# NumericalEarth/Breeze.jl

Measured on AMD Instinct MI355X. Metric: grid-cells advanced/sec (tendency+Poisson step), 512^3 anelastic, higher is better.
Workload: dtype f64

## Files before the change

breeze.jl_amd/csrc/bz_acoustic_kernels.h:

```cpp
#pragma once
#include "bz_compressible_internal.h"

__device__ __forceinline__ void ac_wall_faces(const DevGrid &g, const AcParams &P, int i, int j, double &up0, double &up1, double &vp0, double &vp1)
{
    if (g.bounded_x) {
        if (i == 0 && P.wall_w) up0 = 0.0;
        if (i == g.Nx - 1) up1 = 0.0;
    }
    if (g.bounded_y) {
        if (j == 0 && P.wall_s) vp0 = 0.0;
        if (j == g.Ny - 1) vp1 = 0.0;
    }
}
__device__ __forceinline__ bool ac_accumulate(const AcParams &P)
{
    return !(P.skip_avg_if_dry && __builtin_amdgcn_readfirstlane(*P.skip_avg_if_dry) == 1);
}

#ifndef AC_PENCIL
#define AC_PENCIL 1
#endif
__device__ __forceinline__ void ac_pencil_block(int &bx, int &j, int &k)
{
    bx = blockIdx.x; j = blockIdx.y; k = blockIdx.z;
    const unsigned gx = gridDim.x, gy = gridDim.y, gz = gridDim.z;
    if (AC_PENCIL && (gy & 63u) == 0) {
        const unsigned w = bx + gx * (j + gy * k), c = w & 7u;
        unsigned r = w >> 3;
        bx = (int)(r % gx); r /= gx;
        const unsigned jj = r & 7u; r >>= 3;
        k = (int)(r % gz); r /= gz;
        j = (int)(((r * 8 + c) * 8) + jj);
    }
    bx = __builtin_amdgcn_readfirstlane(bx); j = __builtin_amdgcn_readfirstlane(j); k = __builtin_amdgcn_readfirstlane(k);
}

template <bool ZERO, bool STORE0, bool PF, bool NOPERT, class ST>
__global__ __launch_bounds__(256) void k_ac_stage_init(DevGrid g, AcFieldsT<ST> F)
{
    int bx, j, k;
    ac_pencil_block(bx, j, k);
    const int i = bx * 256 + threadIdx.x;
    if (i >= g.Nx) return;
    const long long sz = g.Sxy;
    const long long n = g.idx(i, j, k);
    if (j >= g.Ny) {
        if (PF) F.Gp_rv[n] = F.G_rv[n] - (F.p[n] - F.p[n - g.Sx]) * g.rdy;
        return;
    }
    if (PF) {
        const WrapIdx W = wrap_of(g, i, j);
        const double p0 = F.p[n];
        F.Gp_ru[n] = F.G_ru[n] - (p0 - F.p[n + W.im]) * g.rdx;
        F.Gp_rv[n] = F.G_rv[n] - (p0 - F.p[n + W.jm]) * g.rdy;
    }
    if (STORE0) {
        ((double *)F.U0_rho_d)[n] = F.rho_d[n];
        ((double *)F.U0_rth)[n] = F.rth[n];
        ((double *)F.U0_ru)[n] = F.ru[n];
        ((double *)F.U0_rv)[n] = F.rv[n];
        ((double *)F.U0_rw)[n] = F.rw[n];
        ((double *)F.U0_rq)[n] = F.rq[n];
        if (!NOPERT) { F.rp[n] = 0.0; F.rthp_out[n] = 0.0; F.rup[n] = 0.0; F.rvp[n] = 0.0; F.rwp[n] = 0.0; }
    } else if (!NOPERT) {
    F.rp[n] = F.U0_rho_d[n] - F.rho_d[n];
    F.rthp_out[n] = F.U0_rth[n] - F.rth[n];
    F.rup[n] = F.U0_ru[n] - F.ru[n];
    F.rvp[n] = F.U0_rv[n] - F.rv[n];
    F.rwp[n] = F.U0_rw[n] - F.rw[n];
    }
    if (ZERO) {
    F.au[n] = 0.0;
    F.av[n] = 0.0;
    F.aw[n] = 0.0;
    }
    if (k == 0) {
        F.Gs[n] = 0.0;
    } else {
        const long long m = n - sz;
        const double dp = ((F.p[n] - g.p_r[k]) - (F.p[m] - g.p_r[k - 1])) * g.rdzf[k];
        const double rf = ((F.rho[n] - g.rho[k]) + (F.rho[m] - g.rho[k - 1])) / 2.0;
        F.Gs[n] = F.G_rw[n] - dp - g.g * rf;
    }
    if (k == g.Nz - 1) {
        if (STORE0) { ((double *)F.U0_rw)[n + sz] = F.rw[n + sz]; if (!NOPERT) F.rwp[n + sz] = 0.0; }
        else if (!NOPERT) F.rwp[n + sz] = F.U0_rw[n + sz] - F.rw[n + sz];
        F.Gs[n + sz] = 0.0;
    }
}

template <bool DAMP, bool STEP, class ST>
__global__ __launch_bounds__(256) void k_ac_horizontal(DevGrid g, AcFieldsT<ST> F, AcParams P)
{
    const int i = blockIdx.x * 256 + threadIdx.x, j = blockIdx.y, k = blockIdx.z;
    if (i >= g.Nx) return;
    const WrapIdx W = wrap_of(g, i, j);
    const long long n = g.idx(i, j, k), mx = n + W.im, my = n + W.jm;
    double up = F.rup[n], vp = F.rvp[n];
    const double rt = F.rthp[n], rtx = F.rthp[mx], rty = F.rthp[my];
    if (DAMP) {
        const double d0 = rt - F.rth_old[n];
        const double ddx = (d0 - (rtx - F.rth_old[mx])) * g.rdx;
        const double ddy = (d0 - (rty - F.rth_old[my])) * g.rdy;
        const double th = F.thL[n];
        up -= P.kdamp * ddx / ((th + F.thL[mx]) / 2.0);
        vp -= P.kdamp * ddy / ((th + F.thL[my]) / 2.0);
    }
    if (STEP) {
        const double p0 = F.p[n];
        double dpx = (p0 - F.p[mx]) * g.rdx;
        double dpy = (p0 - F.p[my]) * g.rdy;
        if (P.gate != 0.0) {
            const double c0 = F.Clin[n] * rt;
            dpx = dpx + P.gate * ((c0 - F.Clin[mx] * rtx) * g.rdx);
            dpy = dpy + P.gate * ((c0 - F.Clin[my] * rty) * g.rdy);
        }
        up += P.dtau * (F.G_ru[n] - dpx);
        vp += P.dtau * (F.G_rv[n] - dpy);
        if (g.bounded_x && i == 0 && P.wall_w) up = 0.0;
        if (g.bounded_y && j == 0 && P.wall_s) vp = 0.0;
        F.au[n] += up;
        F.av[n] += vp;
    }
    if (g.bounded_x && i == 0 && P.wall_w) up = 0.0;
    if (g.bounded_y && j == 0 && P.wall_s) vp = 0.0;
    F.rup[n] = up;
    F.rvp[n] = vp;
}

__device__ __forceinline__ double ibz(double fp, double fm, bool p_per, bool m_per)
{
    fp = p_per ? fm : fp;
    fm = m_per ? fp : fm;
    return (fp + fm) / 2.0;
}

template <bool DAMP>
__device__ __forceinline__ double ac_face_update(double up, double G, double rt_b, double rt_a, double rto_b, double rto_a,
                                                 double th_b, double th_a, double C_b, double C_a, double p_b, double p_a,
                                                 double rd, const AcParams &P)
{
    if (DAMP) {
        const double dd = ((rt_b - rto_b) - (rt_a - rto_a)) * rd;
        up -= P.kdamp * dd / ((th_b + th_a) / 2.0);
    }
    double dp = (p_b - p_a) * rd;
    if (P.gate != 0.0) dp = dp + P.gate * ((C_b * rt_b - C_a * rt_a) * rd);
    return up + P.dtau * (G - dp);
}

#ifndef ACX
#define ACX 64
#endif
#ifndef ACY
#define ACY 4
#endif
#ifndef ABX
#define ABX 256
#endif
#ifndef ABY
#define ABY 1
#endif
#ifndef AC_MINW
#define AC_MINW 1
#endif
template <bool FIRST, bool FUSED, bool DAMP, class ST>
__global__ __launch_bounds__(ACX * ACY, AC_MINW) void k_ac_column_forward(DevGrid g, AcFieldsT<ST> F, AcParams P)
{
    int bx = blockIdx.x, by = blockIdx.y;
    if (P.xcd) {
        const unsigned w = blockIdx.y * gridDim.x + blockIdx.x, c = w & 7u, r = w >> 3;
        bx = (int)(r % gridDim.x);
        by = (int)(c * (gridDim.y >> 3) + r / gridDim.x);
    }
    const int i = bx * ACX + threadIdx.x, j = by * ACY + threadIdx.y;
    if (i >= g.Nx || j >= g.Ny) return;
    const WrapIdx W = wrap_of(g, i, j);
    const long long sz = g.Sxy;
    const int Nz = g.Nz;
    long long n = g.idx(i, j, 0);
    const double dtn2 = P.dtn * P.dtn;

    double th_0 = F.thL[n], th_p = F.thL[n + sz];
    double C_m = 0.0, C_0 = F.Clin[n];
#ifndef AC_FX
#define AC_FX 1
#endif
    const bool FX = AC_FX && FUSED && (ACX == 64) && sizeof(ST) == 8;
    const int lane = threadIdx.x;
    double thy_m0 = 0.0, thy_p0 = 0.0, thy_m1 = 0.0, thy_p1 = 0.0;
    double cy_m0 = 0.0, cy_p0 = 0.0;
    if (FX) {
        thy_m0 = F.thL[n + W.jm]; thy_p0 = F.thL[n + W.jp];
        thy_m1 = F.thL[n + sz + W.jm]; thy_p1 = F.thL[n + sz + W.jp];
        cy_m0 = F.Clin[n + W.jm]; cy_p0 = F.Clin[n + W.jp];
    }
    double w_m = 0.0, w_0 = F.rwp[n], w_p = F.rwp[n + sz];
    double rs_m = 0.0, rths_m = 0.0, rp_m = 0.0, rthp_m = 0.0;
    double beta = 1.0, phi_m = 0.0, c_m = 0.0;
    double thf_0 = th_0, thf_m = th_0;

    for (int k = 0; k < Nz; ++k, n += sz) {
        const double rdc = g.rdzc[k];
        const double Ax = g.Ax[k], Ay = g.Ay[k], Vinv = g.Vinv_c[k];
        const double rp = F.rp[n], rthp = F.rthp[n];
        double thxm, thxp, thym, thyp;
        if (FX) {
            const double e_m = (lane == 0) ? F.thL[n + W.im] : 0.0, e_p = (lane == ACX - 1 || i == g.Nx - 1) ? F.thL[n + W.ip] : 0.0;
            thxm = __shfl_up(th_0, 1); thxp = __shfl_down(th_0, 1);
            if (lane == 0) thxm = e_m;
            if (lane == ACX - 1 || i == g.Nx - 1) thxp = e_p;
            thym = thy_m0; thyp = thy_p0;
        } else {
            thxm = F.thL[n + W.im]; thxp = F.thL[n + W.ip]; thym = F.thL[n + W.jm]; thyp = F.thL[n + W.jp];
        }
        double up0, up1, vp0, vp1;
        if (FUSED) {
            const long long nxm = n + W.im, nxp = n + W.ip, nym = n + W.jm, nyp = n + W.jp;
            const double rt_xm = F.rthp[nxm], rt_xp = F.rthp[nxp], rt_ym = F.rthp[nym], rt_yp = F.rthp[nyp];
            double o0 = 0.0, o_xm = 0.0, o_xp = 0.0, o_ym = 0.0, o_yp = 0.0;
            if (DAMP) { o0 = F.rth_old[n]; o_xm = F.rth_old[nxm]; o_xp = F.rth_old[nxp]; o_ym = F.rth_old[nym]; o_yp = F.rth_old[nyp]; }
            double c_xm = 0.0, c_xp = 0.0, c_ym = 0.0, c_yp = 0.0;
            if (FX) {
                const double e_m = (lane == 0) ? F.Clin[nxm] : 0.0, e_p = (lane == ACX - 1 || i == g.Nx - 1) ? F.Clin[nxp] : 0.0;
                c_xm = __shfl_up(C_0, 1); c_xp = __shfl_down(C_0, 1);
                if (lane == 0) c_xm = e_m;
                if (lane == ACX - 1 || i == g.Nx - 1) c_xp = e_p;
                c_ym = cy_m0; c_yp = cy_p0;
            } else if (P.gate != 0.0) { c_xm = F.Clin[nxm]; c_xp = F.Clin[nxp]; c_ym = F.Clin[nym]; c_yp = F.Clin[nyp]; }
            const double p0 = F.p[n], p_xm = F.p[nxm], p_xp = F.p[nxp], p_ym = F.p[nym], p_yp = F.p[nyp];
            up0 = ac_face_update<DAMP>(F.rup_in[n], F.G_ru[n], rthp, rt_xm, o0, o_xm, th_0, thxm, C_0, c_xm, p0, p_xm, g.rdx, P);
            up1 = ac_face_update<DAMP>(F.rup_in[nxp], F.G_ru[nxp], rt_xp, rthp, o_xp, o0, thxp, th_0, c_xp, C_0, p_xp, p0, g.rdx, P);
            vp0 = ac_face_update<DAMP>(F.rvp_in[n], F.G_rv[n], rthp, rt_ym, o0, o_ym, th_0, thym, C_0, c_ym, p0, p_ym, g.rdy, P);
            vp1 = ac_face_update<DAMP>(F.rvp_in[nyp], F.G_rv[nyp], rt_yp, rthp, o_yp, o0, thyp, th_0, c_yp, C_0, p_yp, p0, g.rdy, P);
            ac_wall_faces(g, P, i, j, up0, up1, vp0, vp1);
            F.rup[n] = up0;
            F.rvp[n] = vp0;
            if (FIRST) { F.au[n] = 0.0 + up0; F.av[n] = 0.0 + vp0; }
            else { F.au[n] += up0; F.av[n] += vp0; }
        } else {
            up0 = F.rup[n]; up1 = F.rup[n + W.ip]; vp0 = F.rvp[n]; vp1 = F.rvp[n + W.jp];
            ac_wall_faces(g, P, i, j, up0, up1, vp0, vp1);
            F.rth_old[n] = rthp;
        }
        const double thf_p = (k + 1 < Nz) ? (th_p + th_0) / 2.0 : th_0;

        const double dxM = Ax * up1 - Ax * up0;
        const double dxT = Ax * ((thxp + th_0) / 2.0) * up1 - Ax * ((th_0 + thxm) / 2.0) * up0;
        const double dyM = Ay * vp1 - Ay * vp0;
        const double dyT = Ay * ((thyp + th_0) / 2.0) * vp1 - Ay * ((th_0 + thym) / 2.0) * vp0;
        const double divM = Vinv * (dxM + dyM);
        const double divT = Vinv * (dxT + dyT);
        const double dzW = (w_p - w_0) * rdc;
        const double dzT = (thf_p * w_p - thf_0 * w_0) * rdc;
        const double rs = rp + P.dtau * (F.G_rho_d[n] - divM) - P.dto * dzW;
        const double rths = rthp + P.dtau * (P.f_theta * F.G_rth[n] - divT) - P.dto * dzT;
        F.rs[n] = rs;
        F.rths[n] = rths;

        double phi = 0.0;
        if (k > 0) {
            const double rdf = g.rdzf[k], rdm = g.rdzc[k - 1];
            const double dps = (C_0 * rths - C_m * rths_m) * rdf;
            const double dpo = (C_0 * rthp - C_m * rthp_m) * rdf;
            const double Gp = P.dto * dpo + P.dtn * dps;
            const double Gb = g.g * (P.dto * ((rp + rp_m) / 2.0) + P.dtn * ((rs + rs_m) / 2.0));
            const double d2 = ((w_p - w_0) * rdc - (w_0 - w_m) * rdm) * rdf;
            const double Gd = -P.d_old * d2;
            const double sp = F.sponge[k];
            const double f = w_0 + P.dtau * P.f_w * F.Gs[n] - Gp - Gb - Gd - fabs(P.dto) * sp * w_0;
            const double a = -dtn2 * C_m * thf_m * rdm * rdf + dtn2 * g.g * rdm / 2.0 + (-P.d_new * rdm * rdf);
            const double b = 1.0 + (dtn2 * thf_0 * (C_0 * rdc + C_m * rdm) * rdf + dtn2 * g.g * (rdc - rdm) / 2.0 +
                                    P.d_new * (rdc + rdm) * rdf + fabs(P.dtn) * sp);
            const double t = c_m / beta;
            beta = b - a * t;
            phi = (f - a * phi_m) / beta;
            if (FIRST) F.tfac[n] = t;
            c_m = -dtn2 * C_0 * thf_p * rdc * rdf + (-dtn2 * g.g * rdc / 2.0) + (-P.d_new * rdc * rdf);
        } else if (FIRST) {
            F.tfac[n] = 0.0;
        }
        F.phi[n] = phi;
        phi_m = phi;

        rs_m = rs; rths_m = rths; rp_m = rp; rthp_m = rthp;
        C_m = C_0;
        th_0 = th_p; thf_m = thf_0; thf_0 = thf_p;
        w_m = w_0; w_0 = w_p;
        if (k + 1 < Nz) {
            C_0 = F.Clin[n + sz];
            th_p = (k + 2 < Nz) ? F.thL[n + 2 * sz] : th_0;
            w_p = F.rwp[n + 2 * sz];
            if (FX) {
                cy_m0 = F.Clin[n + sz + W.jm]; cy_p0 = F.Clin[n + sz + W.jp];
                thy_m0 = thy_m1; thy_p0 = thy_p1;
                if (k + 2 < Nz) { thy_m1 = F.thL[n + 2 * sz + W.jm]; thy_p1 = F.thL[n + 2 * sz + W.jp]; }
            }
        }
    }
}

template <class T>
__device__ __forceinline__ T ac_ld(const T *base, unsigned e)
{
    return *(const T *)((const char *)base + (size_t)(e * (unsigned)sizeof(T)));
}
template <class T, class V>
__device__ __forceinline__ void ac_st(T *base, unsigned e, V v)
{
    *(T *)((char *)base + (size_t)(e * (unsigned)sizeof(T))) = (T)v;
}
#ifndef AC2_NT
#define AC2_NT 0
#endif
#ifndef AC2_BARRIER
#define AC2_BARRIER 0
#endif
template <class T>
__device__ __forceinline__ T ac_ld_nt(const T *base, unsigned e)
{
    if (AC2_NT & 1) return __builtin_nontemporal_load((const T *)((const char *)base + (size_t)(e * (unsigned)sizeof(T))));
    return ac_ld(base, e);
}
template <class T, class V>
__device__ __forceinline__ void ac_st_nt(T *base, unsigned e, V v)
{
    if (AC2_NT & 2) __builtin_nontemporal_store((T)v, (T *)((char *)base + (size_t)(e * (unsigned)sizeof(T))));
    else ac_st(base, e, v);
}

template <bool DAMP, bool PF>
__device__ __forceinline__ double ac_face_update2(double up, double G, double rt_b, double rt_a, double rto_b, double rto_a,
                                                  double th_b, double th_a, double C_b, double C_a, double p_b, double p_a,
                                                  double rd, const AcParams &P)
{
    if (DAMP) {
        const double dd = ((rt_b - rto_b) - (rt_a - rto_a)) * rd;
        up -= P.kdamp * dd / ((th_b + th_a) / 2.0);
    }
    if (PF) {
        if (P.gate != 0.0) G = G - P.gate * ((C_b * rt_b - C_a * rt_a) * rd);
        return up + P.dtau * G;
    }
    double dp = (p_b - p_a) * rd;
    if (P.gate != 0.0) dp = dp + P.gate * ((C_b * rt_b - C_a * rt_a) * rd);
    return up + P.dtau * (G - dp);
}

template <bool FIRST, bool DAMP, bool PF, int CFG, class ST, int INIT = 0>
__global__ __launch_bounds__((CFG & 1) ? 512 : 256, (CFG & 2) ? 3 : 2) void k_ac_forward2(DevGrid g, AcFieldsT<ST> F, AcParams P)
{
    static_assert(FIRST || INIT == 0, "initial perturbations belong to the first substep of a stage");
    int bx = blockIdx.x, by = blockIdx.y;
    if (P.xcd) {
        const unsigned w = blockIdx.y * gridDim.x + blockIdx.x, c = w & 7u, r = w >> 3;
        bx = (int)(r % gridDim.x);
        by = (int)(c * (gridDim.y >> 3) + r / gridDim.x);
    }
    const int i = bx * (int)blockDim.x + threadIdx.x, j = by * (int)blockDim.y + threadIdx.y;
    if (i >= g.Nx || j >= g.Ny) return;
    const WrapIdx W = wrap_of(g, i, j);
    const unsigned sz = (unsigned)g.Sxy;
    const unsigned dxp = (unsigned)(int)W.ip, dym = (unsigned)(int)W.jm, dyp = (unsigned)(int)W.jp;
    const int Nz = g.Nz;
    unsigned e = (unsigned)g.idx(i, j, 0);
    const double dtn2 = P.dtn * P.dtn;
    const int lane = threadIdx.x & 63;
    const bool edge_m = (lane == 0), edge_p = (lane == 63 || i == g.Nx - 1);
    const bool edge = edge_m || edge_p;
    const unsigned dedge = edge_m ? (unsigned)(int)W.im : dxp;
    const ColPtr::cptr sponge = (ColPtr::cptr)F.sponge;
    const double *Gu = PF ? F.Gp_ru : F.G_ru, *Gv = PF ? F.Gp_rv : F.G_rv;
    const bool acc = ac_accumulate(P);

    double th_0 = ac_ld(F.thL, e), th_p = ac_ld(F.thL, e + sz);
    double C_m = 0.0, C_0 = ac_ld(F.Clin, e);
    double thy_m0 = ac_ld(F.thL, e + dym), thy_p0 = ac_ld(F.thL, e + dyp);
    double thy_m1 = ac_ld(F.thL, e + sz + dym), thy_p1 = ac_ld(F.thL, e + sz + dyp);
    double cy_m0 = ac_ld(F.Clin, e + dym), cy_p0 = ac_ld(F.Clin, e + dyp);
    auto pert = [&](const double *U0, const double *U, unsigned ee) { return (double)(ST)(ac_ld(U0, ee) - ac_ld(U, ee)); };
    auto pert_w = [&](unsigned ee) { return ac_ld(F.U0_rw, ee) - ac_ld((const double *)F.rw, ee); };
    double w_m = 0.0, w_0, w_p;
    if (INIT == 2) { w_0 = 0.0; w_p = 0.0; }
    else if (INIT == 1) { w_0 = pert_w(e); w_p = pert_w(e + sz); }
    else { w_0 = ac_ld(F.rwp, e); w_p = ac_ld(F.rwp, e + sz); }
    double rs_m = 0.0, rths_m = 0.0, rp_m = 0.0, rthp_m = 0.0;
    double beta = 1.0, phi_m = 0.0, c_m = 0.0;
    double thf_0 = th_0, thf_m = th_0;

    struct AcLevel {
        double rp, rthp, rt_ym, rt_yp, o0, o_ym, o_yp, ru0, ru1, rv0, rv1, Gu0, Gu1, Gv0, Gv1, p0, p_xm, p_xp, p_ym, p_yp, au_o, av_o, Grho, Grth, Gs_k;
        double e_th, e_C, e_rt, e_o;
        double C_n, cy_mn, cy_pn, th_n, thy_mn, thy_pn, w_n;
    };
    auto level = [&](const unsigned e, const int k) {
        AcLevel L;
        const unsigned exp_ = e + dxp, eym = e + dym, eyp = e + dyp;
        if (INIT == 2) { L.rp = 0.0; L.rthp = 0.0; L.rt_ym = 0.0; L.rt_yp = 0.0; }
        else if (INIT == 1) {
            L.rp = pert(F.U0_rho_d, F.rho_d, e); L.rthp = pert(F.U0_rth, F.rth, e);
            L.rt_ym = pert(F.U0_rth, F.rth, eym); L.rt_yp = pert(F.U0_rth, F.rth, eyp);
        } else {
        L.rp = ac_ld_nt(F.rp, e); L.rthp = ac_ld(F.rthp, e);
        L.rt_ym = ac_ld(F.rthp, eym); L.rt_yp = ac_ld(F.rthp, eyp);
        }
        L.o0 = 0.0; L.o_ym = 0.0; L.o_yp = 0.0;
        if (DAMP) { L.o0 = ac_ld(F.rth_old, e); L.o_ym = ac_ld(F.rth_old, eym); L.o_yp = ac_ld(F.rth_old, eyp); }
        if (INIT == 2) { L.ru0 = 0.0; L.ru1 = 0.0; L.rv0 = 0.0; L.rv1 = 0.0; }
        else if (INIT == 1) {
            L.ru0 = pert(F.U0_ru, F.ru, e); L.ru1 = pert(F.U0_ru, F.ru, exp_); L.rv0 = pert(F.U0_rv, F.rv, e); L.rv1 = pert(F.U0_rv, F.rv, eyp);
        } else {
        L.ru0 = ac_ld(F.rup_in, e); L.ru1 = ac_ld(F.rup_in, exp_); L.rv0 = ac_ld(F.rvp_in, e); L.rv1 = ac_ld(F.rvp_in, eyp);
        }
        L.Gu0 = ac_ld(Gu, e); L.Gu1 = ac_ld(Gu, exp_); L.Gv0 = ac_ld(Gv, e); L.Gv1 = ac_ld(Gv, eyp);
        L.p0 = 0.0; L.p_xm = 0.0; L.p_xp = 0.0; L.p_ym = 0.0; L.p_yp = 0.0;
        if (!PF) {
            L.p0 = ac_ld(F.p, e); L.p_xm = ac_ld(F.p, e + (unsigned)(int)W.im); L.p_xp = ac_ld(F.p, exp_);
            L.p_ym = ac_ld(F.p, eym); L.p_yp = ac_ld(F.p, eyp);
        }
        L.au_o = 0.0; L.av_o = 0.0;
        if (!FIRST && acc && P.acc_mode != 1) { L.au_o = ac_ld_nt(F.au, e); L.av_o = ac_ld_nt(F.av, e); }
        L.Grho = ac_ld_nt(F.G_rho_d, e); L.Grth = ac_ld_nt(F.G_rth, e); L.Gs_k = ac_ld_nt(F.Gs, e);
        L.e_th = 0.0; L.e_C = 0.0; L.e_rt = 0.0; L.e_o = 0.0;
        if (edge) {
            const unsigned ee = e + dedge;
            L.e_th = ac_ld(F.thL, ee); L.e_C = ac_ld(F.Clin, ee);
            L.e_rt = INIT == 2 ? 0.0 : INIT == 1 ? pert(F.U0_rth, F.rth, ee) : ac_ld(F.rthp, ee);
            if (DAMP) L.e_o = ac_ld(F.rth_old, ee);
        }
        const unsigned e1 = (k + 1 < Nz) ? e + sz : e, e2 = (k + 2 < Nz) ? e1 + sz : e1;
        L.C_n = ac_ld(F.Clin, e1); L.cy_mn = ac_ld(F.Clin, e1 + dym); L.cy_pn = ac_ld(F.Clin, e1 + dyp);
        L.th_n = ac_ld(F.thL, e2); L.thy_mn = ac_ld(F.thL, e2 + dym); L.thy_pn = ac_ld(F.thL, e2 + dyp);
        L.w_n = INIT == 2 ? 0.0 : INIT == 1 ? pert_w(e1 + sz) : ac_ld_nt(F.rwp, e1 + sz);
        return L;
    };
    constexpr bool PIPE = (CFG & 8) != 0;
    auto work = [&](const AcLevel &L, const int k, const unsigned e) {
        const double rdc = g.rdzc[k];
        const double Ax = g.Ax[k], Ay = g.Ay[k], Vinv = g.Vinv_c[k];
        const double rp = L.rp, rthp = L.rthp, rt_ym = L.rt_ym, rt_yp = L.rt_yp, o0 = L.o0, o_ym = L.o_ym, o_yp = L.o_yp;
        const double ru0 = L.ru0, ru1 = L.ru1, rv0 = L.rv0, rv1 = L.rv1, Gu0 = L.Gu0, Gu1 = L.Gu1, Gv0 = L.Gv0, Gv1 = L.Gv1;
        const double p0 = L.p0, p_xm = L.p_xm, p_xp = L.p_xp, p_ym = L.p_ym, p_yp = L.p_yp, au_o = L.au_o, av_o = L.av_o;
        const double Grho = L.Grho, Grth = L.Grth, Gs_k = L.Gs_k, e_th = L.e_th, e_C = L.e_C, e_rt = L.e_rt, e_o = L.e_o;
        const double C_n = L.C_n, cy_mn = L.cy_mn, cy_pn = L.cy_pn, th_n = L.th_n, thy_mn = L.thy_mn, thy_pn = L.thy_pn, w_n = L.w_n;
        const double sp = sponge[k];

        constexpr bool DPP = (CFG & 16) != 0;
        double thxm = ac_lane_up<DPP>(th_0), thxp = ac_lane_down<DPP>(th_0);
        double c_xm = ac_lane_up<DPP>(C_0), c_xp = ac_lane_down<DPP>(C_0);
        double rt_xm = ac_lane_up<DPP>(rthp), rt_xp = ac_lane_down<DPP>(rthp);
        double o_xm = 0.0, o_xp = 0.0;
        if (DAMP) { o_xm = ac_lane_up<DPP>(o0); o_xp = ac_lane_down<DPP>(o0); }
        if (edge_m) { thxm = e_th; c_xm = e_C; rt_xm = e_rt; o_xm = e_o; }
        if (edge_p) { thxp = e_th; c_xp = e_C; rt_xp = e_rt; o_xp = e_o; }
        const double thym = thy_m0, thyp = thy_p0, c_ym = cy_m0, c_yp = cy_p0;

        const double up0 = ac_face_update2<DAMP, PF>(ru0, Gu0, rthp, rt_xm, o0, o_xm, th_0, thxm, C_0, c_xm, p0, p_xm, g.rdx, P);
        const double up1 = ac_face_update2<DAMP, PF>(ru1, Gu1, rt_xp, rthp, o_xp, o0, thxp, th_0, c_xp, C_0, p_xp, p0, g.rdx, P);
        const double vp0 = ac_face_update2<DAMP, PF>(rv0, Gv0, rthp, rt_ym, o0, o_ym, th_0, thym, C_0, c_ym, p0, p_ym, g.rdy, P);
        const double vp1 = ac_face_update2<DAMP, PF>(rv1, Gv1, rt_yp, rthp, o_yp, o0, thyp, th_0, c_yp, C_0, p_yp, p0, g.rdy, P);
        const double au_n = FIRST ? 0.0 + up0 : (P.acc_mode == 2) ? au_o + (ru0 + up0) : au_o + up0;
        const double av_n = FIRST ? 0.0 + vp0 : (P.acc_mode == 2) ? av_o + (rv0 + vp0) : av_o + vp0;
        const double thf_p = (k + 1 < Nz) ? (th_p + th_0) / 2.0 : th_0;

        const double dxM = Ax * up1 - Ax * up0;
        const double dxT = Ax * ((thxp + th_0) / 2.0) * up1 - Ax * ((th_0 + thxm) / 2.0) * up0;
        const double dyM = Ay * vp1 - Ay * vp0;
        const double dyT = Ay * ((thyp + th_0) / 2.0) * vp1 - Ay * ((th_0 + thym) / 2.0) * vp0;
        const double divM = Vinv * (dxM + dyM);
        const double divT = Vinv * (dxT + dyT);
        const double dzW = (w_p - w_0) * rdc;
        const double dzT = (thf_p * w_p - thf_0 * w_0) * rdc;
        const double rs = rp + P.dtau * (Grho - divM) - P.dto * dzW;
        const double rths = rthp + P.dtau * (P.f_theta * Grth - divT) - P.dto * dzT;

        double phi = 0.0, t = 0.0;
        if (k > 0) {
            const double rdf = g.rdzf[k], rdm = g.rdzc[k - 1];
            const double dps = (C_0 * rths - C_m * rths_m) * rdf;
            const double dpo = (C_0 * rthp - C_m * rthp_m) * rdf;
            const double Gp = P.dto * dpo + P.dtn * dps;
            const double Gb = g.g * (P.dto * ((rp + rp_m) / 2.0) + P.dtn * ((rs + rs_m) / 2.0));
            const double d2 = ((w_p - w_0) * rdc - (w_0 - w_m) * rdm) * rdf;
            const double Gd = -P.d_old * d2;
            const double f = w_0 + P.dtau * P.f_w * Gs_k - Gp - Gb - Gd - fabs(P.dto) * sp * w_0;
            const double a = -dtn2 * C_m * thf_m * rdm * rdf + dtn2 * g.g * rdm / 2.0 + (-P.d_new * rdm * rdf);
            const double b = 1.0 + (dtn2 * thf_0 * (C_0 * rdc + C_m * rdm) * rdf + dtn2 * g.g * (rdc - rdm) / 2.0 +
                                    P.d_new * (rdc + rdm) * rdf + fabs(P.dtn) * sp);
            t = c_m / beta;
            beta = b - a * t;
            phi = (f - a * phi_m) / beta;
            c_m = -dtn2 * C_0 * thf_p * rdc * rdf + (-dtn2 * g.g * rdc / 2.0) + (-P.d_new * rdc * rdf);
        }
        if (INIT) ac_st(F.rthp, e, rthp);
        if (INIT && !g.wrap_y) {
            if (j == 0) ac_st(F.rthp, e + dym, rt_ym);
            if (j == g.Ny - 1) ac_st(F.rthp, e + dyp, rt_yp);
        }
        ac_st_nt(F.rup, e, up0);
        ac_st_nt(F.rvp, e, vp0);
        if (acc && (FIRST || P.acc_mode != 1)) {
            ac_st_nt(F.au, e, au_n);
            ac_st_nt(F.av, e, av_n);
        }
        ac_st_nt(F.rs, e, rs);
        ac_st_nt(F.rths, e, rths);
        if (FIRST) ac_st_nt(F.tfac, e, t);
        ac_st_nt(F.phi, e, phi);
        phi_m = phi;
        if (AC2_BARRIER || (CFG & 4)) __builtin_amdgcn_s_barrier();

        rs_m = rs; rths_m = rths; rp_m = rp; rthp_m = rthp;
        C_m = C_0; C_0 = C_n;
        thf_m = thf_0; thf_0 = thf_p;
        th_0 = th_p; th_p = th_n;
        w_m = w_0; w_0 = w_p; w_p = w_n;
        cy_m0 = cy_mn; cy_p0 = cy_pn;
        thy_m0 = thy_m1; thy_p0 = thy_p1; thy_m1 = thy_mn; thy_p1 = thy_pn;
    };
    if (!PIPE) {
        for (int k = 0; k < Nz; ++k, e += sz) work(level(e, k), k, e);
    } else {
        AcLevel LA = level(e, 0), LB;
#pragma unroll 1
        for (int k = 0; k < Nz; k += 2, e += 2 * sz) {
            const int k1 = (k + 1 < Nz) ? k + 1 : k;
            LB = level(e + (unsigned)(k1 - k) * sz, k1);
            work(LA, k, e);
            if (k + 1 < Nz) {
                const int k2 = (k + 2 < Nz) ? k + 2 : k + 1;
                LA = level(e + (unsigned)(k2 - k) * sz, k2);
                work(LB, k + 1, e + sz);
            }
        }
    }
}

template <bool FIRST, class ST, int INIT = 0>
__global__ __launch_bounds__(ABX * ABY) void k_ac_column_backward(DevGrid g, AcFieldsT<ST> F, AcParams P)
{
    const int i = blockIdx.x * ABX + threadIdx.x, j = blockIdx.y * ABY + threadIdx.y;
    if (i >= g.Nx || j >= g.Ny) return;
    const long long sz = g.Sxy;
    const int Nz = g.Nz;
    const bool acc = ac_accumulate(P);
    long long n = g.idx(i, j, Nz - 1);
    double w_hi = F.rwp[n + sz];
    if (INIT) {
        w_hi = (INIT == 2) ? 0.0 : F.U0_rw[n + sz] - F.rw[n + sz];
        F.rwp[n + sz] = w_hi;
    }
    double th_0 = F.thL[n];
    double thf_hi = th_0;
    double t_hi = 0.0;
    for (int k = Nz - 1; k >= 0; --k, n -= sz) {
        const double th_m = (k > 0) ? F.thL[n - sz] : th_0;
        const double thf_lo = (k > 0) ? (th_0 + th_m) / 2.0 : th_0;
        double w_lo = F.phi[n];
        if (k < Nz - 1) w_lo -= t_hi * w_hi;
        const double rdc = g.rdzc[k];
        const double dzW = (w_hi - w_lo) * rdc;
        const double dzT = (thf_hi * w_hi - thf_lo * w_lo) * rdc;
        F.rp[n] = F.rs[n] - P.dtn * dzW;
        F.rthp_out[n] = F.rths[n] - P.dtn * dzT;
        const double w_old = (!FIRST && acc && P.acc_mode == 2) ? F.rwp[n] : 0.0;
        F.rwp[n] = w_lo;
        if (acc) {
            if (FIRST) F.aw[n] = 0.0 + w_lo;
            else if (P.acc_mode == 2) F.aw[n] += (w_old + w_lo);
            else if (P.acc_mode == 0) F.aw[n] += w_lo;
        }
        t_hi = F.tfac[n];
        w_hi = w_lo;
        thf_hi = thf_lo;
        th_0 = th_m;
    }
}

template <bool DAMP, class ST>
__global__ __launch_bounds__(256) void k_ac_finalize(DevGrid g, AcFieldsT<ST> F, AcParams P)
{
    const int i = blockIdx.x * 256 + threadIdx.x, j = blockIdx.y, k = blockIdx.z;
    if (i >= g.Nx) return;
    const WrapIdx W = wrap_of(g, i, j);
    const long long sz = g.Sxy;
    const long long n = g.idx(i, j, k), mx = n + W.im, my = n + W.jm;
    if (DAMP) {
        const double d0 = F.rthp[n] - F.rth_old[n];
        const double ddx = (d0 - (F.rthp[mx] - F.rth_old[mx])) * g.rdx;
        const double ddy = (d0 - (F.rthp[my] - F.rth_old[my])) * g.rdy;
        const double th = F.thL[n];
        double up = F.rup[n] - P.kdamp * ddx / ((th + F.thL[mx]) / 2.0);
        double vp = F.rvp[n] - P.kdamp * ddy / ((th + F.thL[my]) / 2.0);
        if (g.bounded_x && i == 0 && P.wall_w) up = 0.0;
        if (g.bounded_y && j == 0 && P.wall_s) vp = 0.0;
        F.rup[n] = up;
        F.rvp[n] = vp;
    }
    const double r0 = F.rho_d[n];
    double rx = (r0 + F.rho_d[mx]) / 2.0, ry = (r0 + F.rho_d[my]) / 2.0;
    rx = (rx == 0.0) ? 1.0 : rx;
    ry = (ry == 0.0) ? 1.0 : ry;
    const double ua = (F.ru[n] + F.au[n] * P.inv_N) / rx;
    const double va = (F.rv[n] + F.av[n] * P.inv_N) / ry;
    st_img(F.au, n, ua, W.ox, W.oy);
    st_img(F.av, n, va, W.ox, W.oy);
    double wa = 0.0;
    if (k > 0) {
        double rz = (r0 + F.rho_d[n - sz]) / 2.0;
        rz = (rz == 0.0) ? 1.0 : rz;
        wa = (F.rw[n] + F.aw[n] * P.inv_N) / rz;
    }
    st_img(F.aw, n, wa, W.ox, W.oy);
// ... 271 lines not shown
```

breeze.jl_amd/csrc/bz_internal.h:

```cpp
#pragma once
#include <hip/hip_runtime.h>
#include <hipfft/hipfft.h>

#include <cstdint>
#include <cstdio>
#include <string>
#include <vector>

#include "../../include/breeze_hip.h"

struct ColPtr {
    const double *p = nullptr;
    ColPtr() = default;
    __host__ __device__ ColPtr(const double *q) : p(q) {}
    __host__ __device__ operator const double *() const { return p; }
#ifdef __HIPCC__
    typedef const double __attribute__((address_space(4))) *cptr;
    __device__ __forceinline__ double operator[](int k) const { return ((cptr)p)[k]; }
    __device__ __forceinline__ double operator[](long long k) const { return ((cptr)p)[k]; }
#endif
};

struct DevGrid {
    int Nx, Ny, Nz;
    int Hx, Hy, Hz;
    int Sx, Sy;
    long long Sxy;
    double dx, dy, rdx, rdy, Az;
    ColPtr dzc, dzf, rdzf;
    ColPtr rdzc;
    ColPtr zc;
    ColPtr Ax, Ay;
    ColPtr Vinv_c, Vinv_f;
    ColPtr rho, rho_f;
    ColPtr rrho, rrho_f;
    ColPtr p_r, T_r;
    ColPtr pi_dry, lnpi;
    double kap_num;
    double g, Rd, Rv, cpd, cpv, pst;
    int formulation;
    int microphysics;
    int sa_maxiter;
    double sa_Ll, sa_cl, sa_dc, sa_L0, sa_Ttr, sa_ptr, sa_abstol;
    double *qv_field, *ql_field;
    double *rqcl_field, *rqr_field, *qcl_field, *qr_field;
    int wrap_y;
    int flat_y;
    int bounded_x;
    int bounded_y;

    __host__ __device__ inline long long idx(int i, int j, int k) const {
        return (long long)(i + Hx) + (long long)Sx * ((long long)(j + Hy)) + Sxy * (long long)(k + Hz);
    }
};

struct RKEpilogue {
    int mode = 0;
    double dt = 0.0, alpha = 0.0, oma = 0.0;
    const double *u0 = nullptr;
    double *u0_out = nullptr;
    const double *u0b = nullptr;
    double *u0b_out = nullptr;
};
#ifdef __HIPCC__
__device__ __forceinline__ void st_img(double *__restrict__ f, long long n, double v, long long ox, long long oy)
{
    f[n] = v;
    if (ox) f[n + ox] = v;
    if (oy) {
        f[n + oy] = v;
        if (ox) f[n + ox + oy] = v;
    }
}
__device__ __forceinline__ void st_img_only(double *__restrict__ f, long long n, double v, long long ox, long long oy)
{
    if (ox) f[n + ox] = v;
    if (oy) {
        f[n + oy] = v;
        if (ox) f[n + ox + oy] = v;
    }
}
__device__ __forceinline__ double bz_cdiv(double a, double b, double rb)
{
    const double q0 = a * rb;
    return fma(fma(-q0, b, a), rb, q0);
}
__device__ __forceinline__ double bz_rk_apply(int mode, double dt, double alpha, double oma, const double *u0,
                                              double *u0_out, double G, double uold, long long n)
{
    if (mode == 0) return G;
    double u0v;
    if (mode == 1) { u0_out[n] = uold; u0v = uold; }
    else u0v = u0[n];
    return oma * u0v + alpha * (uold + dt * G);
}
__device__ __forceinline__ double bz_rk_apply_pre(int mode, double dt, double alpha, double oma, double u0v, double *u0_out, double G,
                                                  double uold, long long n)
{
    if (mode == 1) { u0_out[n] = uold; u0v = uold; }
    else if (mode == 3) u0v = uold;
    return oma * u0v + alpha * (uold + dt * G);
}
#endif

#ifdef __HIPCC__
__device__ __forceinline__ double bz_sconst(double c)
{
    asm volatile("" : "+s"(c));
    return c;
}
__device__ __forceinline__ double bz_exp_small(double a)
{
    int s = 0;
    while (fabs(a) > 0.0625 && s < 64) { a *= 0.5; ++s; }
    double p = bz_sconst(1.0 / 362880.0);
    p = fma(p, a, bz_sconst(1.0 / 40320.0));
    p = fma(p, a, bz_sconst(1.0 / 5040.0));
    p = fma(p, a, bz_sconst(1.0 / 720.0));
    p = fma(p, a, bz_sconst(1.0 / 120.0));
    p = fma(p, a, bz_sconst(1.0 / 24.0));
    p = fma(p, a, bz_sconst(1.0 / 6.0));
    p = fma(p, a, 0.5);
    p = fma(p, a, 1.0);
    p = fma(p, a, 1.0);
    for (; s > 0; --s) p *= p;
    return p;
}
__device__ __forceinline__ double bz_exner_factor(const DevGrid &g, int k, double q, double cpm)
{
    return g.pi_dry[k] * bz_exp_small(((q * g.kap_num) / (cpm * g.cpd)) * g.lnpi[k]);
}
__device__ __forceinline__ double bz_buoyancy(const DevGrid &g, const double *__restrict__ T, const double *__restrict__ q,
                                              long long n, int k)
{
    double qv, ql = 0.0;
    if (g.microphysics == 1) { qv = g.qv_field[n]; ql = g.ql_field[n]; }
    else if (g.microphysics == 2) { qv = q[n]; ql = g.qcl_field[n] + g.qr_field[n]; }
    else qv = q[n];
    const double Rm = (1.0 - (qv + ql)) * g.Rd + qv * g.Rv;
    const double rhop = g.rho[k] * (g.Rd * g.T_r[k] / (Rm * T[n]) - 1.0);
    return -g.g * rhop;
}
__device__ __forceinline__ double bz_kessler_T(const DevGrid &g, double th, double qv, double ql, double pr)
{
    const double qd = 1.0 - (qv + ql);
    const double cpm = qd * g.cpd + qv * g.cpv + ql * g.sa_cl;
    return pow(pr / g.pst, (qd * g.Rd + qv * g.Rv) / cpm) * th + (g.sa_Ll * ql) / cpm;
}
__device__ __forceinline__ double bz_sa_psat(const DevGrid &g, double T)
{
    return g.sa_ptr * pow(T / g.sa_Ttr, g.sa_dc / g.Rv) * exp((1.0 / g.sa_Ttr - 1.0 / T) * g.sa_L0 / g.Rv);
}
__device__ __forceinline__ double bz_sa_T(const DevGrid &g, double th, double qv, double ql, double pr)
{
    const double qd = 1.0 - (qv + ql);
    const double cpm = qd * g.cpd + qv * g.cpv + ql * g.sa_cl;
    return pow(pr / g.pst, (qd * g.Rd + qv * g.Rv) / cpm) * th + (g.sa_Ll * ql) / cpm;
}
__device__ __forceinline__ void bz_sa_adjust(const DevGrid &g, double T, double qt, double pr, double &qv, double &ql)
{
    const double ps = bz_sa_psat(g, T);
    const double qs = (g.Rd / g.Rv) * (1.0 - qt) * ps / (pr - ps);
    ql = fmax(0.0, qt - qs);
    qv = qt - ql;
}
__device__ __forceinline__ double bz_sa_residual(const DevGrid &g, double T, double th, double qt, double pr)
{
    double qv, ql;
    bz_sa_adjust(g, T, qt, pr, qv, ql);
    return T - bz_sa_T(g, th, qv, ql, pr);
}
__device__ __forceinline__ double bz_sa_diagnose(const DevGrid &g, double th, double qt, double pr, double &qv, double &ql)
{
    qv = qt; ql = 0.0;
    const double T1 = bz_sa_T(g, th, qt, 0.0, pr);
    if (th == 0.0) return T1;
    const double rho1 = pr / (((1.0 - qt) * g.Rd + qt * g.Rv) * T1);
    if (qt <= bz_sa_psat(g, T1) / (rho1 * g.Rv * T1)) return T1;
    double qv1, ql1;
    bz_sa_adjust(g, T1, qt, pr, qv1, ql1);
    const double dT = (g.sa_Ll * ql1) / ((1.0 - (qv1 + ql1)) * g.cpd + qv1 * g.cpv + ql1 * g.sa_cl);
    double x1 = T1, x2 = T1 + fmax(0.01, dT / 2.0);
    double r1 = bz_sa_residual(g, x1, th, qt, pr), r2 = bz_sa_residual(g, x2, th, qt, pr);
    for (int it = 0; it < g.sa_maxiter && fabs(r2) > g.sa_abstol; ++it) {
        double s = (x2 - x1) / (r2 - r1);
        const bool valid = isfinite(s);
        s = valid ? s : 0.0;
        x1 = x2; r1 = r2;
        x2 -= r2 * s;
        r2 = valid ? bz_sa_residual(g, x2, th, qt, pr) : 0.0;
    }
    bz_sa_adjust(g, x2, qt, pr, qv, ql);
    return bz_sa_T(g, th, qv, ql, pr);
}
__device__ __forceinline__ double bz_ds_temperature(const DevGrid &g, double th, double qv, double ql, double rho, double abstol,
                                                    int maxiter)
{
    const double qd = 1.0 - (qv + ql);
    const double Rm = qd * g.Rd + qv * g.Rv;
    const double cpm = qd * g.cpd + qv * g.cpv + ql * g.sa_cl;
    const double kap = Rm / cpm, gam = cpm / (cpm - Rm);
    const double L = (g.sa_Ll * ql) / cpm;
    double T = pow(th, gam) * pow(rho * Rm / g.pst, gam - 1.0) + L;
    double dT = T;
    for (int it = 0; it < maxiter && fabs(dT) > abstol; ++it) {
        const double Phi = pow(rho * Rm * T / g.pst, kap) * th;
        dT = -(T - Phi - L) / (1.0 - kap * Phi / T);
        T += dT;
    }
    return T;
}
__device__ __forceinline__ double bz_ds_residual(const DevGrid &g, double T, double th0, double rho, double qt, double &qv, double &ql)
{
    const double qs = bz_sa_psat(g, T) / (rho * g.Rv * T);
    ql = fmax(0.0, qt - qs);
    qv = qt - ql;
    const double qd = 1.0 - (qv + ql);
    const double Rm = qd * g.Rd + qv * g.Rv;
    const double cpm = qd * g.cpd + qv * g.cpv + ql * g.sa_cl;
    const double L = (g.sa_Ll * ql) / cpm;
    const double p = rho * Rm * T;
    return (T - L) * pow(g.pst / p, Rm / cpm) - th0;
}
__device__ __forceinline__ double bz_ds_adjust(const DevGrid &g, double th, double qt, double rho, double nabstol, int nmaxiter,
                                               double &qv, double &ql)
{
    qv = qt; ql = 0.0;
    if (th == 0.0) return 0.0;
    const double T1 = bz_ds_temperature(g, th, qt, 0.0, rho, nabstol, nmaxiter);
    if (qt <= bz_sa_psat(g, T1) / (rho * g.Rv * T1)) return T1;
    double qv1, ql1;
    bz_ds_residual(g, T1, th, rho, qt, qv1, ql1);
    const double dT = (g.sa_Ll * ql1) / ((1.0 - (qv1 + ql1)) * g.cpd + qv1 * g.cpv + ql1 * g.sa_cl);
    double x1 = T1, x2 = T1 + fmax(0.01, dT / 2.0);
    double a, b;
    double r1 = bz_ds_residual(g, x1, th, rho, qt, a, b), r2 = bz_ds_residual(g, x2, th, rho, qt, a, b);
    for (int it = 0; it < g.sa_maxiter && fabs(r2) > g.sa_abstol; ++it) {
        double s = (x2 - x1) / (r2 - r1);
        const bool valid = isfinite(s);
        s = valid ? s : 0.0;
        x1 = x2; r1 = r2;
        x2 -= r2 * s;
        r2 = valid ? bz_ds_residual(g, x2, th, rho, qt, a, b) : 0.0;
    }
    bz_ds_residual(g, x2, th, rho, qt, qv, ql);
    return bz_ds_temperature(g, th, qv, ql, rho, nabstol, nmaxiter);
}
#endif

struct BzComm;
struct ProfileSlot {
    const char *name;
    double total_ms = 0.0;
    int64_t launches = 0;
    std::vector<std::pair<hipEvent_t, hipEvent_t>> pending;
};

struct bz_tuning {
    bool no_fused = false;
    bool no_fuse_rk = false;
    bool no_lean = false;
    bool no_xcd = false;
    bool no_closure_march = false;
    bool no_k6_stored = false;
    bool no_dry_shortcut = false;
    bool side_scalar = false;
    int side_cus = 0;
    int side_cu_layout = 0;
    bool no_fuse_forcing = false;
    bool no_fold_forcing = false;
    int ac_xcd = 1;
    int ac_forward2 = 1;
    int ac_rotate = 1;
    int ac_pair_avg = 1;
    int ac_init_fold = 1;
    int ac_pfold = 1;
    int ac_bx = 128;
    int ac_cfg = 29;
    bool no_fuse_level_sums = false;
    bool no_tridiag_coop = false;
    bool no_xfft = false;
    int poisson_kxmajor = 1;
    int poisson_kx_chunk_mb = 0;
    int poisson_kx_chunk_kb = 0;
    int poisson_kx_pad = 1;
    int poisson_chunk = 0;
    int xf_kchunk_f = 0, xf_kchunk_i = 0;
    int scalar_lds = 1;
    bool no_rho3d_exchange = false;
    bool no_generic_march = false;
    bool generic_onepass = false;
    bool no_ac_fuse = false;
    bool no_ac_end_fuse = false;
    bool comm_no_overlap = false;
    bool comm_self_messages = false;
    bool comm_no_side_scalar = false;
    int graph = -1;
    bool graph_debug = false;
};
void bzi_read_tuning(bz_tuning &t);
#define BZ_REJECT_BOUNDED_Y(ctx, enabling, what)                                                                             \
    do {                                                                                                                     \
        if ((ctx) && (ctx)->dg.bounded_y && (enabling)) {                                                                                \
            (ctx)->last_error = what ": not implemented on a Bounded y (topology (Periodic, Bounded, Bounded))";            \
            return BZ_ERR_UNSUPPORTED;                                                                                       \
        }                                                                                                                    \
    } while (0)
#define BZ_REJECT_KINEMATIC(ctx, who)                                                                                        \
    do {                                                                                                                     \
        if ((ctx) && (ctx)->kinematic) {                                                                                     \
            (ctx)->last_error = who ": the context has PrescribedDynamics (no momentum, no pressure solve); use bz_time_steps_kinematic"; \
            return BZ_ERR_UNSUPPORTED;                                                                                       \
        }                                                                                                                    \
    } while (0)
#define BZ_HALO_XFACE 8
#define BZ_HALO_YFACE 4
struct bz_ctx;
bool bzi_lean_forcings_ok(const bz_ctx *ctx);

struct bz_ctx {
    bz_tuning tune;
    bz_grid grid;
    bz_constants constants;
    DevGrid dg;
    hipStream_t stream = nullptr;
    bool walls_lean_ok = false;
    int num_cus = 256;
    std::string last_error;

    double *d_columns = nullptr;
    int NXH = 0;
    hipfftHandle plan_fwd = 0, plan_inv = 0;
    hipfftDoubleComplex *d_dctx = nullptr;
    bool plans_ok = false;
    hipfftHandle plan_fwd_c = 0, plan_inv_c = 0;
    int pchunk = 0;
    int kr0 = 0, krn = 0;
    bool xf = false;
    bool xf_slab = false;
    void *d_wtab = nullptr;
    hipfftHandle plan_y = 0;
    bool kxmajor = false;
    int kx_cw = 0, kx_nch = 0, kx_pad = 0;
    hipfftHandle plan_yc = 0, plan_yc_last = 0;
    int profile_mute = 0;
    hipfftHandle slab_plan_x_fwd = 0, slab_plan_x_inv = 0, slab_plan_y = 0;
    bool slab_plans_ok = false;
    int slab_inv_ld = 0;
    double *d_rhs = nullptr;
    hipfftDoubleComplex *d_hat = nullptr;
    double *d_ibeta = nullptr;
    double *d_tfac = nullptr;
    double *d_lower = nullptr;
    double *d_scalar = nullptr;
    double *d_havg = nullptr;
    double *d_moments = nullptr;
    struct AzPlan *az = nullptr;
    int y_nranks = 1, y_rank = 0, nkx = 0, kx0 = 0, Ny_global = 0;
    bool slab_mode = false;
    bool tiled_tendencies = true;
    bool fuse_rk = true;
    bool G_is_predictor = false;
    bool fused_ok = true;
    int q_host = 0;
    int *h_qstate = nullptr;
    hipEvent_t ev_q = nullptr;
    bool q_pending = false;
    int *d_qstate = nullptr;
    bool diagnostics_stale = false;
    bool lean_step_last = false;
    bool lean = true;
    bool lean_xcd = true;
    hipStream_t side_stream = nullptr;
    hipEvent_t ev_fork = nullptr, ev_join = nullptr;
    bool side_scalar = false;
    void *d_lev_rows = nullptr;
    double *d_pi_dry = nullptr;
    bool compressible = false;
    bool has_reference = false;
    bz_split_explicit se;
    int weno_R = 3;
    int scalar_R = 3;
    double *d_gflux = nullptr;
    double dz_min = 0.0;
    double *d_sponge = nullptr;
    double *d_Clin = nullptr;
    double *d_tfac_ac = nullptr;
    double *d_up2 = nullptr, *d_vp2 = nullptr;
    double *d_Gp_ru = nullptr, *d_Gp_rv = nullptr;
    double *d_thL2 = nullptr;
    double *d_balance = nullptr;
    bool thL_alt = false;
    bool substep_f32 = false;
    bool ac_whole_step = false;
    bool ac_rotate = false;
    bool ac_skip_avg = false;
    bool ac_fused = true;
    int ac_open[4] = {0, 0, 0, 0};
    double ac_open_relax = 0.5;
    bz_kessler_microphysics kessler_params;
    bz_kessler_model_fields kessler;
    double kessler_pst = 1e5;
    bool has_instant_precip = false;
    double *ip_precipitation_rate = nullptr;
    bool has_relaxation = false;
    double *d_relax = nullptr;
    int relax_mask = 0, relax_specific = 0;
    const double *field_forcing = nullptr;
    int field_forcing_specific = 0;
    bool has_forcings = false;
    double *d_forcing = nullptr;
    int forcing_static_mask = 0, forcing_subsidence_mask = 0;
    double *d_lsum_rows = nullptr;
    long long lsum_P = 0;
    bool lsum_fresh = false;
    bool lsum_step_last = false;
    bool fold_momentum_forcing = false;
    double forcing_f = 0.0, forcing_flux_theta = 0.0, forcing_flux_q = 0.0, forcing_drag = 0.0, forcing_drag_eps = 0.0, forcing_flux_energy = 0.0;
    bool has_bulk = false;
    bz_bulk_surface_fluxes bulk;
    bool bulk_const_on = false;
    bool sl_on = false;
    bz_surface_layer sl;
    double *d_sl = nullptr;
    bool sl_initialized = false;
    int n_tracers = 0;
    bz_tracer_fields tracers[BZ_MAX_TRACERS];
    bool has_closure = false;
    bz_smagorinsky_lilly closure;
    double *closure_nu = nullptr;
    double *d_closure_ipi = nullptr;
    bool has_diffusivity = false;
    bz_scalar_diffusivity diffusivity;
    double *diff_nu = nullptr, *diff_kappa = nullptr;
    double *d_diff_table = nullptr;
    double *d_diff_scratch = nullptr;
    int diff_scratch_fields = 0;
    double *up2_user = nullptr, *vp2_user = nullptr;
    alignas(8) unsigned char ac_stage_storage[160] = {0};
    int bounded_mask = 0;
    double bounded_lo = 0.0, bounded_hi = 1.0;
    bool kinematic = false;
    bool kin_correction = false;
    double *d_kin_div = nullptr;
    uint64_t velocity_epoch = 0;
    uint64_t kin_div_epoch = 0;
    const double *kin_div_u = nullptr, *kin_div_v = nullptr, *kin_div_w = nullptr;
    struct BzComm *comm = nullptr;
    bool profiling = false;
    std::vector<ProfileSlot> slots;
    int graph_mode = 0;
    bool graph_capturing = false;
    uint64_t config_epoch = 0;
    struct GraphSlot {
        uint64_t key = 0;
        int seen = 0;
        hipGraph_t graph = nullptr;
        hipGraphExec_t exec = nullptr;
        bool g_is_predictor = false, lean_step_last = false, lsum_step_last = false;
    } graph_slots[2];
    int graph_next = 0;
    hipStream_t graph_stream = nullptr, graph_user_stream = nullptr;
    long long graph_replays = 0, graph_captures = 0;
};

uint64_t bzi_graph_key(const bz_ctx *ctx, int kind, double dt, const void *a, size_t na, const void *b, size_t nb, const void *c, size_t nc,
                       const void *d, size_t nd);
int bzi_graph_begin(bz_ctx *ctx, uint64_t key, bool *capture);
int bzi_graph_end(bz_ctx *ctx, uint64_t key, int body_rc);
void bzi_graph_destroy(bz_ctx *ctx);
void bzi_graph_configure(bz_ctx *ctx);
int bzi_apply_stream(bz_ctx *ctx, hipStream_t stream);

#define BZ_HIP(expr)                                                                        \
    do {                                                                                    \
        hipError_t _e = (expr);                                                             \
        if (_e != hipSuccess) {                                                             \
            ctx->last_error = std::string(#expr) + ": " + hipGetErrorString(_e);            \
            return -(int)_e;                                                                \
        }                                                                                   \
    } while (0)

#define BZ_FFT(expr)                                                                        \
    do {                                                                                    \
        hipfftResult _r = (expr);                                                           \
        if (_r != HIPFFT_SUCCESS) {                                                         \
            ctx->last_error = std::string(#expr) + ": hipfft status " + std::to_string((int)_r); \
            return -1000 - (int)_r;                                                         \
        }                                                                                   \
    } while (0)

#define BZ_LAUNCH_CHECK()                                                                   \
    do {                                                                                    \
        hipError_t _e = hipGetLastError();                                                  \
        if (_e != hipSuccess) {                                                             \
            ctx->last_error = std::string("kernel launch: ") + hipGetErrorString(_e);       \
            return -(int)_e;                                                                \
        }                                                                                   \
    } while (0)

typedef unsigned long long bz_bits_t;
__device__ __forceinline__ bz_bits_t bz_real_bits(double d) { return (bz_bits_t)__double_as_longlong(d); }
__device__ __forceinline__ double bz_real_inf() { return __longlong_as_double(0x7ff0000000000000LL); }

struct ProfileScope {
    bz_ctx *ctx;
    int slot = -1;
    hipEvent_t e0 = nullptr, e1 = nullptr;
    ProfileScope(bz_ctx *c, const char *name);
    ~ProfileScope();
};

int bzi_fill_halo(bz_ctx *ctx, double *f, int kind);
int bzi_apply_forcings(bz_ctx *ctx, const bz_state *s, double *Gu, double *Gv, double *Gth, double *Gq, double scale, bool momentum_done = false);
int bzi_compute_forcings(bz_ctx *ctx, const bz_state *s);
double *bzi_level_sum_rows(bz_ctx *ctx, long long *P);
bool bzi_level_sums_ride(const bz_ctx *ctx);
int bzi_flux_bc(bz_ctx *ctx, const bz_state *s, double *Gu, double *Gv, double *Gth, double *Gq, double scale);
int bzi_surface_layer_stage(bz_ctx *ctx, const bz_state *s, int stage, double dt);
void bzi_forcing_teardown(bz_ctx *ctx);
void bzi_diagnostics_teardown(bz_ctx *ctx);
void bzi_azimuthal_teardown(bz_ctx *ctx);
void bzi_moments_teardown(bz_ctx *ctx);
int bzi_tracer_specific(bz_ctx *ctx);
int bzi_tracer_rk3(bz_ctx *ctx, double dt, double alpha, bool first);
int bzi_tracer_store_initial_state(bz_ctx *ctx);
int bzi_tracer_tendencies(bz_ctx *ctx, const bz_state *s, bool one_record = true);
int bzi_momentum_advection_gen1(bz_ctx *ctx, const bz_state *s, const bz_prognostic *G);
int bzi_momentum_advection_generic(bz_ctx *ctx, const bz_state *s, const bz_prognostic *G);
int bzi_generic_tendencies_fused_rk(bz_ctx *ctx, const bz_state *s, const bz_prognostic *U0, const bz_prognostic *G, double dt, double alpha,
                                    bool first);
int bzi_scalar_tendency_generic(bz_ctx *ctx, double *Gc, const double *u, const double *v, const double *w, const double *c);
int bzi_scalar_rho3d_generic(bz_ctx *ctx, double *Gc, double *Grho, const double *rho, const double *u, const double *v, const double *w,
                             const double *c, const double *ru, const double *rv, const double *rw);
void bzi_closure_teardown(bz_ctx *ctx);
int bzi_apply_closure(bz_ctx *ctx, const bz_state *s, double *Gu, double *Gv, double *Gw, double *Gth, double *Gq, double scale);
void bzi_diffusivity_teardown(bz_ctx *ctx);
int bzi_diffusivity_halos(bz_ctx *ctx);
int bzi_apply_diffusivity(bz_ctx *ctx, const bz_state *s, double *Gu, double *Gv, double *Gw, double *Gth, double *Gq, double scale);
int bzi_cmp_closure_fields(bz_ctx *ctx, const bz_compressible_state *s);
int bzi_cmp_closure_slow(bz_ctx *ctx, const bz_compressible_state *s, const bz_compressible_prognostic *G);
int bzi_cmp_diffusivity_slow(bz_ctx *ctx, const bz_compressible_state *s, const bz_compressible_prognostic *G);
int bzi_cmp_water_closure(bz_ctx *ctx, const bz_compressible_state *s, const bz_compressible_prognostic *G, const int *skip_if_dry);
int bzi_implicit_step(bz_ctx *ctx, double *ru, double *rv, double *rw, double *rth, double *rq, double dtau);
int bzi_kessler_rk3(bz_ctx *ctx, double dt, double alpha, bool first);
int bzi_kessler_columns(bz_ctx *ctx, double *theta, double *rho_theta, double *rho_q, const double *density, const double *pressure, double dt);
int bzi_kessler_update(bz_ctx *ctx, const bz_state *s, const bz_prognostic *G, double dt);
int bzi_fill_halos_multi(bz_ctx *ctx, double *const *fields, const int *kinds, int n);
int bzi_poisson_setup(bz_ctx *ctx, const double *h_rho_halo );
int bzi_bounded_tendencies(bz_ctx *ctx, const bz_state *s, const bz_prognostic *G);
int bzi_compute_tendencies_generic(bz_ctx *ctx, const bz_state *s, const bz_prognostic *G);
int bzi_momentum_tendencies_generic(bz_ctx *ctx, const bz_state *s, const bz_prognostic *G);
int bzi_apply_relaxation(bz_ctx *ctx, const bz_state *s, const bz_prognostic *G, const double *rho3d = nullptr);
int bzi_lean_setup(bz_ctx *ctx);
int bzi_dist_time_step(bz_ctx *ctx, const bz_state *s, const bz_prognostic *U0, const bz_prognostic *G, double dt, bool diagnose = true);
int bzi_pack_rows_geom(bz_ctx *ctx, double *const *fields, const int32_t *levels, int32_t n, int32_t row0, int32_t nrows, double *buffer,
                       int32_t unpack, int sx, long long sxy);
int bzi_comm_join_pending(bz_ctx *ctx);
int bzi_refresh_diagnostics(bz_ctx *ctx, const bz_state *s, const char *who);
int bzi_kinematic_update_state(bz_ctx *ctx, const bz_state *s, const bz_prognostic *G, int compute_tendencies);
void bzi_kinematic_teardown(bz_ctx *ctx);
enum bz_tier { BZ_TIER_LEAN, BZ_TIER_FUSED_RK, BZ_TIER_FUSED, BZ_TIER_OPERATORS };
bz_tier bzi_anelastic_tier(const bz_ctx *ctx);
inline constexpr double BZ_SSP_RK3_ALPHA[3] = {1.0, 1.0 / 4.0, 2.0 / 3.0};
int bzi_zero_wall_faces(bz_ctx *ctx, const bz_prognostic *G, const bz_prognostic *U0 = nullptr);
int bzi_fused_rk_physics(bz_ctx *ctx, const bz_state *s, const bz_prognostic *G, double dt, double alpha, bool first, bool fold);
void bzi_lean_step_done(bz_ctx *ctx, bool diagnosed);
int bzi_scan_moisture(bz_ctx *ctx, const bz_state *s);
int bzi_scan_moisture_field(bz_ctx *ctx, const double *rho_q);
const int *bzi_moisture_state(const bz_ctx *ctx);
void bzi_moisture_unknown(bz_ctx *ctx);
struct LeanStage;
void bzi_lean_stage(const bz_state *s, const bz_prognostic *U0, const bz_prognostic *G, int stage, LeanStage *L);
int bzi_dist_time_step_compressible(bz_ctx *ctx, const bz_compressible_state *s, const bz_compressible_prognostic *U0,
                                    const bz_compressible_prognostic *G, const bz_acoustic_substepper *sub, double dt);
int bzi_compressible_store_initial_state(bz_ctx *ctx, const bz_compressible_state *s, const bz_compressible_prognostic *U0);
void bzi_comm_teardown(bz_ctx *ctx);
int bzi_comm_allreduce_sum(bz_ctx *ctx, double *buf, int n);
void bzi_lean_teardown(bz_ctx *ctx);
void bzi_poisson_teardown(bz_ctx *ctx);
int bzi_poisson_solve(bz_ctx *ctx, const bz_state *s, double dt);
int bzi_poisson_spectral(bz_ctx *ctx);
int bzi_poisson_from_momentum(bz_ctx *ctx, const bz_state *s, double dt, const bz_prognostic *predictor);
int bzi_fft_chunk(bz_ctx *ctx, int k0, bool forward);
int bzi_xf_forward(bz_ctx *ctx, const bz_state *s, double dt, const bz_prognostic *predictor, const double *rhs = nullptr,
                   double *hat = nullptr, int blocks = 1, int klo = 0, int khi = 0);
int bzi_xf_inverse(bz_ctx *ctx, const double *hat = nullptr, double *phi = nullptr, int blocks = 1, int klo = 0, int khi = 0);
int bzi_xf_y(bz_ctx *ctx, bool forward);
int bzi_tridiag_launch(bz_ctx *ctx, double *hat, double scale, int Ny, int mean_column, int kx_lo = 0, int kx_hi = 0);
int bzi_xf_middle(bz_ctx *ctx);
int bzi_rk3_fused(bz_ctx *ctx, const bz_state *s, const bz_prognostic *U0, const bz_prognostic *G, double dt,
                  double alpha, bool first);
int bzi_poisson_source_fused(bz_ctx *ctx, const bz_state *s, double dt, double *rhs = nullptr,
                             const bz_prognostic *predictor = nullptr);
int bzi_project_diagnose(bz_ctx *ctx, const bz_state *s, double dt, const double *phi_c = nullptr,
                         const double *phi_below = nullptr, const bz_prognostic *predictor = nullptr, bool store_phi = true,
                         const double *rtheta_in = nullptr, const double *rq_in = nullptr, bool level_sums = false);
int bzi_project_lean(bz_ctx *ctx, const bz_state *s, double dt, const double *phi_c, const double *phi_below,
                     const bz_prognostic *predictor, double *sa, double *sb);
struct LeanStage {
    bz_state sin;
    bz_state sout;
    bz_prognostic u0;
    const double *pa, *pb;
    double *oa, *ob;
};
int bzi_tendencies_lean(bz_ctx *ctx, const bz_state *s, const bz_prognostic *U0, const bz_prognostic *G, const double *pa,
                        const double *pb, double *oa, double *ob, double dt, double alpha, bool first, int rows = 0, int which = 3);
static inline int bzi_lean_tendencies(bz_ctx *ctx, const LeanStage &L, const bz_prognostic *G, double dt, double alpha, bool first,
                                      int rows = 0, int which = 3)
{
    return bzi_tendencies_lean(ctx, &L.sin, &L.u0, G, L.pa, L.pb, L.oa, L.ob, dt, alpha, first, rows, which);
}
int bzi_scalar_pair_fork(bz_ctx *ctx, const LeanStage &L, const bz_prognostic *G, double dt, double alpha, bool first);
int bzi_scalar_pair_join(bz_ctx *ctx);
int bzi_tendencies_fused_rk(bz_ctx *ctx, const bz_state *s, const bz_prognostic *U0, const bz_prognostic *G, double dt,
                            double alpha, bool first);
int bzi_create(bz_ctx **out, const bz_grid *grid, const bz_constants *constants, const bz_reference_state *ref,
               int weno_order, int y_nranks, int y_rank, bool slab_mode, bool compressible = false);
void bzi_compressible_teardown(bz_ctx *ctx);
void bzi_balance_teardown(bz_ctx *ctx);
int bzi_refresh_reference_columns(bz_ctx *ctx, const double *density, const double *pressure);
bool bzi_k6_stored_ok(const bz_ctx *ctx);
int bzi_k6_stored(bz_ctx *ctx, int comp, const bz_state *s, const bz_prognostic *G, const bz_prognostic *U0, const RKEpilogue *Ein, int bm);
int bzi_scalar_pair_tendency(bz_ctx *ctx, const bz_state *s, const bz_prognostic *G, const bz_prognostic *U0 = nullptr,
                             const RKEpilogue *E = nullptr);
int bzi_u_tendency_lds(bz_ctx *ctx, const bz_state *s, const bz_prognostic *G, const bz_prognostic *U0 = nullptr,
                       const RKEpilogue *E = nullptr);
int bzi_v_tendency_lds(bz_ctx *ctx, const bz_state *s, const bz_prognostic *G, const bz_prognostic *U0 = nullptr,
                       const RKEpilogue *E = nullptr);
int bzi_w_tendency_lds(bz_ctx *ctx, const bz_state *s, const bz_prognostic *G, const bz_prognostic *U0 = nullptr,
                       const RKEpilogue *E = nullptr, int buoyancy_mode = 0);
```

breeze.jl_amd/csrc/bz_step.hip:

```cpp
#include <cstdlib>

#include "bz_internal.h"

extern "C" int bz_update_state(bz_ctx *ctx, const bz_state *s, const bz_prognostic *G, int compute_tendencies)
{
    if (!ctx || !s || (compute_tendencies && !G)) return BZ_ERR_INVALID;
    if (ctx->kinematic) return bzi_kinematic_update_state(ctx, s, G, compute_tendencies);
    int rc;
    if (ctx->comm && (rc = bzi_comm_join_pending(ctx))) return rc;
    ctx->diagnostics_stale = false;
    if (ctx->d_qstate) BZ_HIP(hipMemsetAsync(ctx->d_qstate, 0, sizeof(int), ctx->stream));
    bzi_moisture_unknown(ctx);
    double *sf[4] = {s->rho_theta, s->rho_q, ctx->dg.rqcl_field, ctx->dg.rqr_field};
    int sk[4] = {0, 0, 0, 0};
    if ((rc = bzi_fill_halos_multi(ctx, sf, sk, ctx->dg.microphysics == 2 ? 4 : 2))) return rc;
    if ((rc = bz_compute_velocities(ctx, s))) return rc;
    if ((rc = bz_compute_auxiliary_thermodynamic_variables(ctx, s))) return rc;
    if (compute_tendencies && (rc = bz_compute_tendencies(ctx, s, G))) return rc;
    return BZ_OK;
}

bz_tier bzi_anelastic_tier(const bz_ctx *ctx)
{
    const DevGrid &g = ctx->dg;
    const bool slab = ctx->slab_mode;
    const bool walls_lean = g.bounded_y && ctx->walls_lean_ok;
    const bool order5 = ctx->weno_R == 3 && ctx->scalar_R == 3;
    const bool theta_model = g.formulation == 0;
    const bool lean_switches = slab || (ctx->fuse_rk && ctx->lean);
    const bool lean_anelastic = slab || !ctx->compressible;
    const bool lean_forcings = !ctx->has_forcings || (!slab && bzi_lean_forcings_ok(ctx));
    const bool rk_orders = slab ? order5
                                : ctx->scalar_R == ctx->weno_R && (ctx->weno_R == 3 || ctx->n_tracers == 0);
    const bool rk_forcings = slab || !(ctx->has_forcings && ctx->tune.no_fuse_forcing);
    const bool fused_tier = !slab;
    if ((ctx->fused_ok || walls_lean) && lean_switches && order5 && lean_anelastic && theta_model && g.microphysics == 0 && lean_forcings &&
        !ctx->has_bulk && !ctx->has_closure && !ctx->has_diffusivity && !ctx->has_relaxation && ctx->n_tracers == 0 && !ctx->bounded_mask &&
        (long long)g.Sxy * (g.Nz + 2 * g.Hz + 1) < (1LL << 32))
        return BZ_TIER_LEAN;
    if ((ctx->fused_ok || (walls_lean && ctx->weno_R != 3)) && ctx->fuse_rk && rk_orders && theta_model && g.microphysics != 2 &&
        !ctx->bounded_mask && !ctx->has_relaxation && rk_forcings)
        return BZ_TIER_FUSED_RK;
    return ctx->fused_ok && fused_tier ? BZ_TIER_FUSED : BZ_TIER_OPERATORS;
}

int bzi_zero_wall_faces(bz_ctx *ctx, const bz_prognostic *G, const bz_prognostic *U0)
{
    const DevGrid &g = ctx->dg;
    for (const long long face : {g.Sxy * g.Hz, g.Sxy * (g.Hz + g.Nz)})
        BZ_HIP(hipMemsetAsync(G->rho_w + face, 0, g.Sxy * sizeof(double), ctx->stream));
    return U0 ? bzi_zero_wall_faces(ctx, U0, nullptr) : BZ_OK;
}

int bzi_scalar_pair_fork(bz_ctx *ctx, const LeanStage &L, const bz_prognostic *G, double dt, double alpha, bool first)
{
    BZ_HIP(hipEventRecord(ctx->ev_fork, ctx->stream));
    BZ_HIP(hipStreamWaitEvent(ctx->side_stream, ctx->ev_fork, 0));
    hipStream_t keep = ctx->stream;
    ctx->stream = ctx->side_stream;
    const int rc = bzi_lean_tendencies(ctx, L, G, dt, alpha, first, 0, 2);
    ctx->stream = keep;
    if (rc) return rc;
    BZ_HIP(hipEventRecord(ctx->ev_join, ctx->side_stream));
    return BZ_OK;
}

int bzi_scalar_pair_join(bz_ctx *ctx) { BZ_HIP(hipStreamWaitEvent(ctx->stream, ctx->ev_join, 0)); return BZ_OK; }

int bzi_fused_rk_physics(bz_ctx *ctx, const bz_state *s, const bz_prognostic *G, double dt, double alpha, bool first, bool fold)
{
    int rc;
    if (ctx->n_tracers) {
        if ((rc = bzi_tracer_tendencies(ctx, s))) return rc;
        if ((rc = bzi_tracer_rk3(ctx, dt, alpha, first))) return rc;
    }
    if (ctx->has_closure && (rc = bzi_apply_closure(ctx, s, G->rho_u, G->rho_v, G->rho_w, s->rho_theta, s->rho_q, alpha * dt))) return rc;
    if (ctx->has_diffusivity && (rc = bzi_apply_diffusivity(ctx, s, G->rho_u, G->rho_v, G->rho_w, s->rho_theta, s->rho_q, alpha * dt))) return rc;
    if (ctx->has_forcings && (rc = bzi_apply_forcings(ctx, s, G->rho_u, G->rho_v, s->rho_theta, s->rho_q, alpha * dt, fold))) return rc;
    if ((ctx->has_forcings || ctx->has_bulk) && (rc = bzi_flux_bc(ctx, s, G->rho_u, G->rho_v, s->rho_theta, s->rho_q, alpha * dt))) return rc;
    return BZ_OK;
}

void bzi_lean_step_done(bz_ctx *ctx, bool diagnosed)
{
    ctx->lean_step_last = true;
    ctx->G_is_predictor = true;
    ctx->diagnostics_stale = !diagnosed;
}

void bzi_lean_stage(const bz_state *s, const bz_prognostic *U0, const bz_prognostic *G, int stage, LeanStage *L)
{
    L->sin = *s; L->sout = *s;
    if (stage > 0) { L->sin.rho_u = U0->rho_u; L->sin.rho_v = U0->rho_v; L->sin.rho_w = U0->rho_w; }
    if (stage < 2) { L->sout.rho_u = U0->rho_u; L->sout.rho_v = U0->rho_v; L->sout.rho_w = U0->rho_w; }
    L->u0.rho_u = s->rho_u; L->u0.rho_v = s->rho_v; L->u0.rho_w = s->rho_w; L->u0.rho_theta = s->rho_theta; L->u0.rho_q = s->rho_q;
    L->pa = stage == 0 ? s->rho_theta : stage == 1 ? G->rho_theta : U0->rho_theta;
    L->pb = stage == 0 ? s->rho_q : stage == 1 ? G->rho_q : U0->rho_q;
    L->oa = stage == 0 ? G->rho_theta : stage == 1 ? U0->rho_theta : s->rho_theta;
    L->ob = stage == 0 ? G->rho_q : stage == 1 ? U0->rho_q : s->rho_q;
}

static int lean_project(bz_ctx *ctx, const bz_state *s, const LeanStage &L, const bz_prognostic *G, double adt, bool full)
{
    return full ? bzi_project_diagnose(ctx, s, adt, nullptr, nullptr, G, true, L.oa, L.ob) : bzi_project_lean(ctx, &L.sout, adt, nullptr, nullptr, G, L.oa, L.ob);
}

static int lean_solve_and_project(bz_ctx *ctx, const bz_state *s, const LeanStage &L, const bz_prognostic *G, double adt, bool full, bool forked)
{
    const DevGrid &g = ctx->dg;
    const int ch = ctx->pchunk;
    int rc = BZ_OK;
    if (ch) {
        {
            ProfileScope ps(ctx, "poisson_source_term+fft_forward");
            ctx->profile_mute++;
            for (int k0 = 0; k0 < g.Nz && !rc; k0 += ch) {
                ctx->kr0 = k0; ctx->krn = ch;
                rc = bzi_poisson_source_fused(ctx, s, adt, nullptr, G);
                if (!rc) rc = bzi_fft_chunk(ctx, k0, true);
            }
            ctx->krn = 0;
            ctx->profile_mute--;
        }
        if (rc) return rc;
        ProfileScope ps(ctx, "poisson_tridiagonal");
        if ((rc = bzi_tridiag_launch(ctx, (double *)ctx->d_hat, 1.0 / ((double)g.Nx * (double)g.Ny), g.Ny, 1))) return rc;
    } else if (ctx->xf) {
        {
            ProfileScope ps(ctx, "poisson_source_term+fft_x");
            if ((rc = bzi_xf_forward(ctx, s, adt, G))) return rc;
        }
        if ((rc = bzi_xf_middle(ctx))) return rc;
        ProfileScope ps(ctx, "poisson_fft_x_inverse");
        if ((rc = bzi_xf_inverse(ctx))) return rc;
    } else {
        if ((rc = bzi_poisson_source_fused(ctx, s, adt, nullptr, G))) return rc;
        if ((rc = bzi_poisson_spectral(ctx))) return rc;
    }
    if (forked && (rc = bzi_scalar_pair_join(ctx))) return rc;
    if (!ch) return lean_project(ctx, s, L, G, adt, full);
    ProfileScope ps(ctx, !full ? "poisson_fft_inverse+project_momentum" : "poisson_fft_inverse+project_and_diagnose");
    ctx->profile_mute++;
    for (int k0 = 0; k0 < g.Nz && !rc; k0 += ch) {
        if ((rc = bzi_fft_chunk(ctx, k0, false))) break;
        ctx->kr0 = k0; ctx->krn = ch;
        rc = lean_project(ctx, s, L, G, adt, full);
    }
    ctx->krn = 0;
    ctx->profile_mute--;
    return rc;
}

static int step_lean(bz_ctx *ctx, const bz_state *s, const bz_prognostic *U0, const bz_prognostic *G, double dt, bool diagnose)
{
    int rc;
    if ((rc = bzi_zero_wall_faces(ctx, G, U0))) return rc;
    const bool fork = ctx->side_scalar && !ctx->has_forcings;
    for (int stage = 0; stage < 3; ++stage) {
        const double alpha = BZ_SSP_RK3_ALPHA[stage];
        LeanStage L;
        bzi_lean_stage(s, U0, G, stage, &L);
        if ((rc = bzi_lean_tendencies(ctx, L, G, dt, alpha, stage == 0, 0, fork ? 1 : 3))) return rc;
        if (fork && (rc = bzi_scalar_pair_fork(ctx, L, G, dt, alpha, stage == 0))) return rc;
        if (ctx->has_forcings && (rc = bzi_flux_bc(ctx, &L.sin, G->rho_u, G->rho_v, L.oa, L.ob, alpha * dt))) return rc;
        if ((rc = lean_solve_and_project(ctx, s, L, G, alpha * dt, diagnose && stage == 2, fork))) return rc;
    }
    bzi_lean_step_done(ctx, diagnose);
    return BZ_OK;
}

static int step_fused_rk(bz_ctx *ctx, const bz_state *s, const bz_prognostic *U0, const bz_prognostic *G, double dt, bool lsum_in)
{
    int rc;
    if ((rc = bzi_zero_wall_faces(ctx, G))) return rc;
    const bool fold = ctx->has_forcings && ctx->weno_R == 3 && bzi_k6_stored_ok(ctx) && ctx->tiled_tendencies && !ctx->tune.no_fuse_forcing && !ctx->tune.no_fold_forcing;
    for (int stage = 0; stage < 3; ++stage) {
        const double alpha = BZ_SSP_RK3_ALPHA[stage];
        if (stage == 0) ctx->lsum_fresh = lsum_in;
        if (fold && (rc = bzi_compute_forcings(ctx, s))) return rc;
        ctx->fold_momentum_forcing = fold;
        rc = bzi_tendencies_fused_rk(ctx, s, U0, G, dt, alpha, stage == 0);
        ctx->fold_momentum_forcing = false;
        if (rc) return rc;
        if ((rc = bzi_fused_rk_physics(ctx, s, G, dt, alpha, stage == 0, fold))) return rc;
        if ((rc = bzi_implicit_step(ctx, G->rho_u, G->rho_v, G->rho_w, s->rho_theta, s->rho_q, alpha * dt))) return rc;
        if (ctx->dg.bounded_y && (rc = bzi_fill_halo(ctx, G->rho_v, BZ_HALO_YFACE))) return rc;
        if ((rc = bzi_poisson_from_momentum(ctx, s, alpha * dt, G))) return rc;
        const bool ride = bzi_level_sums_ride(ctx) && ctx->d_lsum_rows;
        if ((rc = bzi_project_diagnose(ctx, s, alpha * dt, nullptr, nullptr, G, stage == 2, nullptr, nullptr, ride))) return rc;
        ctx->lsum_fresh = ride;
        if ((rc = bzi_tracer_specific(ctx))) return rc;
        if ((rc = bzi_surface_layer_stage(ctx, s, stage, dt))) return rc;
    }
    ctx->lsum_step_last = ctx->lsum_fresh;
    ctx->G_is_predictor = true;
    return BZ_OK;
}

static int step_fused(bz_ctx *ctx, const bz_state *s, const bz_prognostic *U0, const bz_prognostic *G, double dt)
{
    int rc;
    if (ctx->G_is_predictor && (rc = bz_compute_tendencies(ctx, s, G))) return rc;
    for (int stage = 0; stage < 3; ++stage) {
        const double alpha = BZ_SSP_RK3_ALPHA[stage];
        if ((rc = bz_compute_flux_bc_tendencies(ctx, s, G))) return rc;
        if ((rc = bzi_rk3_fused(ctx, s, U0, G, dt, alpha, stage == 0))) return rc;
        if (ctx->dg.microphysics == 2 && (rc = bzi_kessler_rk3(ctx, dt, alpha, stage == 0))) return rc;
        if ((rc = bzi_tracer_rk3(ctx, dt, alpha, stage == 0))) return rc;
        if ((rc = bz_implicit_step(ctx, s, alpha * dt))) return rc;
        if ((rc = bzi_poisson_from_momentum(ctx, s, alpha * dt, nullptr))) return rc;
        if ((rc = bzi_project_diagnose(ctx, s, alpha * dt))) return rc;
        if ((rc = bzi_tracer_specific(ctx))) return rc;
        if ((rc = bzi_surface_layer_stage(ctx, s, stage, dt))) return rc;
        if ((rc = bz_compute_tendencies(ctx, s, G))) return rc;
    }
    if (ctx->dg.microphysics == 2 && (rc = bzi_kessler_update(ctx, s, G, dt))) return rc;
    return BZ_OK;
}

static int step_operators(bz_ctx *ctx, const bz_state *s, const bz_prognostic *U0, const bz_prognostic *G, double dt)
{
    int rc;
    if (ctx->G_is_predictor && (rc = bz_compute_tendencies(ctx, s, G))) return rc;
    if ((rc = bz_store_initial_state(ctx, s, U0))) return rc;
    for (int stage = 0; stage < 3; ++stage) {
        const double alpha = BZ_SSP_RK3_ALPHA[stage];
        if ((rc = bz_compute_flux_bc_tendencies(ctx, s, G))) return rc;
        if ((rc = bz_ssp_rk3_substep(ctx, s, U0, G, dt, alpha))) return rc;
        if ((rc = bz_implicit_step(ctx, s, alpha * dt))) return rc;
        if ((rc = bz_compute_pressure_correction(ctx, s, alpha * dt))) return rc;
        if ((rc = bz_make_pressure_correction(ctx, s, alpha * dt))) return rc;
        if ((rc = bz_update_state(ctx, s, G, 1))) return rc;
        if ((rc = bzi_surface_layer_stage(ctx, s, stage, dt))) return rc;
    }
    if (ctx->dg.microphysics == 2 && (rc = bzi_kessler_update(ctx, s, G, dt))) return rc;
    return BZ_OK;
}

static int anelastic_step_body(bz_ctx *ctx, bz_tier tier, const bz_state *s, const bz_prognostic *U0, const bz_prognostic *G, double dt, bool diagnose)
{
    ctx->lean_step_last = false;
    ctx->lsum_step_last = false;
    const bool lsum_in = ctx->lsum_fresh;
    ctx->lsum_fresh = false;
    if (tier == BZ_TIER_LEAN) return step_lean(ctx, s, U0, G, dt, diagnose);
    if (tier == BZ_TIER_FUSED_RK) return step_fused_rk(ctx, s, U0, G, dt, lsum_in);
    if (tier == BZ_TIER_FUSED) return step_fused(ctx, s, U0, G, dt);
    return step_operators(ctx, s, U0, G, dt);
}

static int one_anelastic_step(bz_ctx *ctx, const bz_state *s, const bz_prognostic *U0, const bz_prognostic *G, double dt, bool diagnose)
{
    if (ctx->slab_mode) {
        if (ctx->comm) return bzi_dist_time_step(ctx, s, U0, G, dt, diagnose);
        ctx->last_error = "bz_time_step_anelastic: a y-slab context needs a communicator (bz_comm_init_rccl / bz_comm_init_local) "
                          "or a host-side distributed driver";
        return BZ_ERR_UNSUPPORTED;
    }
    const bz_tier tier = bzi_anelastic_tier(ctx);
    if (ctx->diagnostics_stale && tier != BZ_TIER_LEAN) { const int rcs = bz_update_state(ctx, s, G, 0); if (rcs) return rcs; }
    const int kind = 1 + (diagnose ? 0 : 16) + 32 * ctx->q_host + (ctx->lsum_fresh ? 128 : 0);
    const uint64_t key = bzi_graph_key(ctx, kind, dt, s, sizeof(*s), U0, sizeof(*U0), G, sizeof(*G), nullptr, 0);
    bool capture = false;
    int rc;
    if (bzi_graph_begin(ctx, key, &capture) == 1) {
        if (ctx->lean_step_last) ctx->diagnostics_stale = !diagnose;
        ctx->lsum_fresh = ctx->lsum_step_last;
        return BZ_OK;
    }
    const bool lsum_in = ctx->lsum_fresh;
    if (capture) {
        rc = anelastic_step_body(ctx, tier, s, U0, G, dt, diagnose);
        if ((rc = bzi_graph_end(ctx, key, rc)) != -1) return rc;
        ctx->lsum_fresh = lsum_in;
    }
    return anelastic_step_body(ctx, tier, s, U0, G, dt, diagnose);
}

static void level_sums_open(bz_ctx *ctx)
{
    ctx->lsum_fresh = false;
    long long P;
    (void)bzi_level_sum_rows(ctx, &P);
}

static int surface_layer_first_step(bz_ctx *ctx, const bz_state *s)
{
    if (!ctx->sl_on || !ctx->sl.filtered || ctx->sl_initialized) return BZ_OK;
    return bz_surface_layer_initialize(ctx, s);
}

extern "C" int bz_time_step_anelastic(bz_ctx *ctx, const bz_state *s, const bz_prognostic *U0, const bz_prognostic *G, double dt)
{
    if (!ctx || !s || !U0 || !G) return BZ_ERR_INVALID;
    BZ_REJECT_KINEMATIC(ctx, "bz_time_step_anelastic");
    level_sums_open(ctx);
    int rc = bzi_scan_moisture(ctx, s);
    if (!rc) rc = surface_layer_first_step(ctx, s);
    if (!rc) rc = one_anelastic_step(ctx, s, U0, G, dt, true);
    ctx->lsum_fresh = false;
    return rc;
}

extern "C" int bz_time_steps_anelastic(bz_ctx *ctx, const bz_state *s, const bz_prognostic *U0, const bz_prognostic *G, double dt, int n,
                                       int diagnose_last)
{
    if (!ctx || !s || !U0 || !G || n < 0) return BZ_ERR_INVALID;
    BZ_REJECT_KINEMATIC(ctx, "bz_time_steps_anelastic");
    level_sums_open(ctx);
    if (n > 0) { const int rc = bzi_scan_moisture(ctx, s); if (rc) return rc; }
    if (n > 0) { const int rc = surface_layer_first_step(ctx, s); if (rc) return rc; }
    for (int it = 0; it < n; ++it) {
        const int rc = one_anelastic_step(ctx, s, U0, G, dt, it == n - 1 && diagnose_last);
        if (rc) { ctx->lsum_fresh = false; return rc; }
    }
    ctx->lsum_fresh = false;
    return BZ_OK;
}

int bzi_refresh_diagnostics(bz_ctx *ctx, const bz_state *s, const char *who)
{
    if (!ctx->diagnostics_stale) return BZ_OK;
    if (!s) {
        ctx->last_error = std::string(who) + ": the diagnostics are stale (bz_time_steps_anelastic ended without the last diagnosis); call bz_update_state first";
        return BZ_ERR_INVALID;
    }
    if (ctx->comm) return bz_comm_update_state_and_project(ctx, s, nullptr, 1.0, 0);
    return bz_update_state(ctx, s, nullptr, 0);
}

extern "C" int bz_diagnostics_stale(const bz_ctx *ctx) { return ctx ? (ctx->diagnostics_stale ? 1 : 0) : BZ_ERR_INVALID; }
```

breeze.jl_amd/csrc/bz_tendency5.hip:

```cpp
#include <cstdlib>

#include "bz_tendency5_kernels.h"

__global__ void k_pi_dry(DevGrid g, double *__restrict__ pi, int n)
{
    const int t = blockIdx.x * blockDim.x + threadIdx.x;
    if (t >= n) return;
    const int k = t - g.Hz;
    const double q = 0.0, qd = 1.0 - q;
    const double Rm = qd * g.Rd + q * g.Rv;
    const double cpm = qd * g.cpd + q * g.cpv;
    pi[t] = pow(g.p_r[k] / g.pst, Rm / cpm);
}

__global__ void k_lev_rows(DevGrid g, const double *__restrict__ pi, LevRow5 *__restrict__ rows, int n)
{
    const int t = blockIdx.x * blockDim.x + threadIdx.x;
    if (t >= n) return;
    const int k = t - g.Hz;
    LevRow5 r;
    r.rho = g.rho[k]; r.rrho = g.rrho[k]; r.rho_f = g.rho_f[k]; r.rrho_f = g.rrho_f[k];
    r.Ax = g.Ax[k]; r.Ay = g.Ay[k]; r.Vinv_c = g.Vinv_c[k]; r.pi = pi[t];
    r.Vinv_f = g.Vinv_f[k]; r.T_r = g.T_r[k];
    for (int q = 0; q < 6; ++q) r.pad[q] = 0.0;
    rows[t] = r;
}

int bzi_lean_setup(bz_ctx *ctx)
{
    const DevGrid &g = ctx->dg;
    const int n = g.Nz + 2 * g.Hz;
    BZ_HIP(hipMalloc(&ctx->d_pi_dry, n * sizeof(double)));
    hipLaunchKernelGGL(k_pi_dry, dim3((n + 63) / 64), dim3(64), 0, 0, g, ctx->d_pi_dry, n);
    ctx->dg.pi_dry = ColPtr(ctx->d_pi_dry + g.Hz);
    BZ_HIP(hipMalloc(&ctx->d_lev_rows, n * sizeof(LevRow5)));
    hipLaunchKernelGGL(k_lev_rows, dim3((n + 63) / 64), dim3(64), 0, 0, g, ctx->d_pi_dry, (LevRow5 *)ctx->d_lev_rows, n);
    BZ_HIP(hipGetLastError());
    BZ_HIP(hipDeviceSynchronize());
    if (ctx->tune.side_cus > 0 && ctx->tune.side_cus < ctx->num_cus) {
        uint32_t mask[32] = {0};
        const int total = ctx->num_cus, want = ctx->tune.side_cus;
        for (int b = 0; b < want; ++b) {
            const int bit = ctx->tune.side_cu_layout == 1 ? (int)((long long)b * total / want) : b;
            mask[bit >> 5] |= 1u << (bit & 31);
        }
        BZ_HIP(hipExtStreamCreateWithCUMask(&ctx->side_stream, (uint32_t)((total + 31) / 32), mask));
    } else
    BZ_HIP(hipStreamCreateWithFlags(&ctx->side_stream, hipStreamNonBlocking));
    BZ_HIP(hipEventCreateWithFlags(&ctx->ev_fork, hipEventDisableTiming));
    BZ_HIP(hipEventCreateWithFlags(&ctx->ev_join, hipEventDisableTiming));
    ctx->side_scalar = ctx->tune.side_scalar;
    ctx->lean = !ctx->tune.no_lean;
    ctx->lean_xcd = !ctx->tune.no_xcd;
    return BZ_OK;
}

void bzi_lean_teardown(bz_ctx *ctx)
{
    if (ctx->d_pi_dry) hipFree(ctx->d_pi_dry);
    ctx->d_pi_dry = nullptr;
    if (ctx->d_lev_rows) hipFree(ctx->d_lev_rows);
    ctx->d_lev_rows = nullptr;
    if (ctx->d_qstate) hipFree(ctx->d_qstate);
    ctx->d_qstate = nullptr;
    if (ctx->h_qstate) hipHostFree(ctx->h_qstate);
    ctx->h_qstate = nullptr;
    if (ctx->ev_q) hipEventDestroy(ctx->ev_q);
    ctx->ev_q = nullptr;
    if (ctx->side_stream) { hipStreamSynchronize(ctx->side_stream); hipStreamDestroy(ctx->side_stream); ctx->side_stream = nullptr; }
    if (ctx->ev_fork) hipEventDestroy(ctx->ev_fork);
    if (ctx->ev_join) hipEventDestroy(ctx->ev_join);
    ctx->ev_fork = ctx->ev_join = nullptr;
}

static int pick_chunk5(const DevGrid &g, int nlev, int rows_per_block, bool fine = false)
{
    long long tiles = (long long)((g.Nx + 63) / 64) * ((g.Ny + rows_per_block - 1) / rows_per_block);
    const int floor_levels = fine ? 64 : 128;
    long long want = ((fine ? 4096 : 1024) + tiles - 1) / tiles;
    long long maxchunks = nlev / floor_levels > 0 ? nlev / floor_levels : 1;
    if (want > maxchunks) want = maxchunks;
    if (want < 1) want = 1;
    if (tiles * want < 512) {
        long long fill = (512 + tiles - 1) / tiles;
        long long cap = nlev / 8 > 0 ? nlev / 8 : 1;
        if (tiles * cap < 256) cap = nlev / 2 > 0 ? nlev / 2 : 1;
        if (fill > cap) fill = cap;
        if (fill > want) want = fill;
    }
    return (int)((nlev + want - 1) / want);
}

template <int TY>
static int lean_launch(bz_ctx *ctx, const bz_state *s, const bz_prognostic *U0, const bz_prognostic *G, const double *pa,
                       const double *pb, double *oa, double *ob, double dt, double alpha, bool first, int rows, int which)
{
    const DevGrid &g = ctx->dg;
    RKEpilogue E;
    E.mode = first ? 3 : 2; E.dt = dt; E.alpha = alpha; E.oma = 1.0 - alpha;
    Lean5 L;
    L.ru = s->rho_u; L.rv = s->rho_v; L.rw = s->rho_w; L.pa = pa; L.pb = pb; L.oa = oa; L.ob = ob; L.out = nullptr;
    L.T = s->T;
    L.pi_dry = ColPtr(ctx->d_pi_dry + g.Hz);
    L.lev = (const LevRow5 *)ctx->d_lev_rows + g.Hz;
    L.qstate = bzi_moisture_state(ctx);
    const int qh = L.qstate ? ctx->q_host : 2;
    L.mforce = 0; L.cor_f = 0.0; L.Fu = ColPtr(nullptr); L.Fv = ColPtr(nullptr); L.Su = ColPtr(nullptr); L.Sv = ColPtr(nullptr);
    if (ctx->has_forcings && bzi_lean_forcings_ok(ctx)) {
        const int m = ctx->forcing_static_mask;
        L.cor_f = ctx->forcing_f;
        if (m & 1) L.Fu = ColPtr(ctx->d_forcing);
        if (m & 2) L.Fv = ColPtr(ctx->d_forcing + (size_t)g.Nz);
        L.mforce = (ctx->forcing_f != 0.0 ? 1 : 0) | ((m & 1) ? 2 : 0) | ((m & 2) ? 4 : 0);
    }
    const dim3 block(64, TY);
    const int tx = (g.Nx + 63) / 64, nty = (g.Ny + TY - 1) / TY;
    if (rows && nty < 3) return rows == 1 ? BZ_OK : lean_launch<TY>(ctx, s, U0, G, pa, pb, oa, ob, dt, alpha, first, 0, which);
    const int ty = rows == 1 ? nty - 2 : rows == 2 ? 2 : nty;
    L.by0 = rows == 1 ? 1 : 0;
    L.bys = rows == 2 ? nty - 1 : 1;
    auto shape = [&](int nlev, int &kc) {
        kc = pick_chunk5(g, nlev, TY, sizeof(double) == 8);
        dim3 grid(tx, ty, (nlev + kc - 1) / kc);
        L.xcd = (ctx->lean_xcd && ((long long)grid.x * grid.y * grid.z) % 8 == 0) ? 1 : 0;
        return grid;
    };
    int kc;
    if (which & 1) {
        ProfileScope ps(ctx, "x_momentum_tendency+rk3+velocity");
        E.u0 = U0->rho_u; E.u0_out = U0->rho_u;
        L.out = G->rho_u;
        const dim3 grid = shape(g.Nz, kc);
        if (g.bounded_y) {
            if (L.mforce) hipLaunchKernelGGL((k6_u<TY, true, true>), grid, block, 0, ctx->stream, g, L, kc, E);
            else hipLaunchKernelGGL((k6_u<TY, false, true>), grid, block, 0, ctx->stream, g, L, kc, E);
        } else if (L.mforce) hipLaunchKernelGGL((k6_u<TY, true>), grid, block, 0, ctx->stream, g, L, kc, E);
        else hipLaunchKernelGGL((k6_u<TY, false>), grid, block, 0, ctx->stream, g, L, kc, E);
    }
    if (which & 1) {
        ProfileScope ps(ctx, "y_momentum_tendency+rk3+velocity");
        E.u0 = U0->rho_v; E.u0_out = U0->rho_v;
        L.out = G->rho_v;
        if (sizeof(double) == 8 && TY == 8 && rows == 0 && !ctx->slab_mode && !g.bounded_y && g.Ny % 16 == 0 && g.Ny >= 64) {
            const int kc16 = pick_chunk5(g, g.Nz, 16);
            const dim3 grid16(tx, g.Ny / 16, (g.Nz + kc16 - 1) / kc16), block16(64, 16);
            L.xcd = (ctx->lean_xcd && ((long long)grid16.x * grid16.y * grid16.z) % 8 == 0) ? 1 : 0;
            if (L.mforce) hipLaunchKernelGGL((k6_v<16, true>), grid16, block16, 0, ctx->stream, g, L, kc16, E);
            else hipLaunchKernelGGL((k6_v<16, false>), grid16, block16, 0, ctx->stream, g, L, kc16, E);
        } else {
        const dim3 grid = shape(g.Nz, kc);
        if (g.bounded_y) {
            if (L.mforce) hipLaunchKernelGGL((k6_v<TY, true, true>), grid, block, 0, ctx->stream, g, L, kc, E);
            else hipLaunchKernelGGL((k6_v<TY, false, true>), grid, block, 0, ctx->stream, g, L, kc, E);
        } else if (L.mforce) hipLaunchKernelGGL((k6_v<TY, true>), grid, block, 0, ctx->stream, g, L, kc, E);
        else hipLaunchKernelGGL((k6_v<TY, false>), grid, block, 0, ctx->stream, g, L, kc, E);
        }
    }
    if (which & 1) {
        ProfileScope ps(ctx, "z_momentum_tendency+rk3+velocity");
        E.u0 = U0->rho_w; E.u0_out = U0->rho_w;
        L.out = G->rho_w;
        const dim3 grid = shape(g.Nz - 1, kc);
#define BZ_LAUNCH_DRY_GENERAL(KERNEL, WYV)                                                                                                  \
        do {                                                                                                                                \
            if (qh != 2) {                                                                                                                  \
                hipLaunchKernelGGL((KERNEL<TY, WYV, true, true>), grid, block, 0, ctx->stream, g, L, kc, E);                                \
                hipLaunchKernelGGL((KERNEL<TY, WYV, false, true>), grid, block, 0, ctx->stream, g, L, kc, E);                               \
            } else hipLaunchKernelGGL((KERNEL<TY, WYV, false, false>), grid, block, 0, ctx->stream, g, L, kc, E);                           \
        } while (0)
        if (g.bounded_y) BZ_LAUNCH_DRY_GENERAL(k6_w, true);
        else BZ_LAUNCH_DRY_GENERAL(k6_w, false);
    }
    if (which & 2) {
        ProfileScope ps(ctx, "scalar_tendencies+rk3+thermo");
        E.u0 = U0->rho_theta; E.u0_out = U0->rho_theta; E.u0b = U0->rho_q; E.u0b_out = U0->rho_q;
        L.out = nullptr;
        const dim3 grid = shape(g.Nz, kc);
        if (g.bounded_y) BZ_LAUNCH_DRY_GENERAL(k5_scalar_pair, true);
        else BZ_LAUNCH_DRY_GENERAL(k5_scalar_pair, false);
    }
    BZ_LAUNCH_CHECK();
    return BZ_OK;
}

bool bzi_k6_stored_ok(const bz_ctx *ctx)
{
    const DevGrid &g = ctx->dg;
    return !ctx->tune.no_k6_stored && !g.flat_y && !g.bounded_x && !g.bounded_y && g.Nz > 1 &&
           (long long)g.Sxy * (g.Nz + 2 * g.Hz + 1) < (1LL << 32);
}

int bzi_k6_stored(bz_ctx *ctx, int comp, const bz_state *s, const bz_prognostic *G, const bz_prognostic *U0, const RKEpilogue *Ein, int bm)
{
    constexpr int TY = 8;
    const DevGrid &g = ctx->dg;
    RKEpilogue E;
    if (Ein) E = *Ein;
    Lean5 L;
    L.ru = s->rho_u; L.rv = s->rho_v; L.rw = s->rho_w; L.pa = L.pb = nullptr; L.oa = L.ob = nullptr; L.T = nullptr;
    L.pi_dry = ColPtr(nullptr);
    L.lev = nullptr;
    L.qstate = nullptr;
    L.mforce = 0; L.cor_f = 0.0; L.Fu = ColPtr(nullptr); L.Fv = ColPtr(nullptr); L.Su = ColPtr(nullptr); L.Sv = ColPtr(nullptr);
    if (ctx->fold_momentum_forcing && Ein && comp < 2) {
        const int m = ctx->forcing_static_mask, sm = ctx->forcing_subsidence_mask;
        const double *sub = ctx->d_forcing + (size_t)5 * g.Nz + (g.Nz + 1) + (size_t)4 * g.Nz;
        L.cor_f = ctx->forcing_f;
        if (m & 1) L.Fu = ColPtr(ctx->d_forcing);
        if (m & 2) L.Fv = ColPtr(ctx->d_forcing + (size_t)g.Nz);
        if (sm) { L.Su = ColPtr(sub); L.Sv = ColPtr(sub + (size_t)g.Nz); }
        L.mforce = (ctx->forcing_f != 0.0 ? 1 : 0) | ((m & 1) ? 2 : 0) | ((m & 2) ? 4 : 0) | (sm ? 8 | 16 : 0);
    }
    L.bT = s->T; L.bq = s->q;
    L.by0 = 0; L.bys = 1;
    const dim3 block(64, TY);
    const int tx = (g.Nx + 63) / 64, nty = (g.Ny + TY - 1) / TY;
    const int nlev = comp == 2 ? g.Nz - 1 : g.Nz;
    const int kc = pick_chunk5(g, nlev, TY, sizeof(double) == 8);
    const dim3 grid(tx, nty, (nlev + kc - 1) / kc);
    L.xcd = (!ctx->tune.no_xcd && ((long long)grid.x * grid.y * grid.z) % 8 == 0) ? 1 : 0;
    if (comp == 0) {
        ProfileScope ps(ctx, Ein ? "x_momentum_tendency+rk3" : "x_momentum_tendency");
        if (Ein) { E.u0 = U0->rho_u; E.u0_out = U0->rho_u; }
        L.vel = s->u; L.out = G->rho_u;
        if (L.mforce) hipLaunchKernelGGL((k6_u<TY, true, false, true>), grid, block, 0, ctx->stream, g, L, kc, E);
        else hipLaunchKernelGGL((k6_u<TY, false, false, true>), grid, block, 0, ctx->stream, g, L, kc, E);
    } else if (comp == 1) {
        ProfileScope ps(ctx, Ein ? "y_momentum_tendency+rk3" : "y_momentum_tendency");
        if (Ein) { E.u0 = U0->rho_v; E.u0_out = U0->rho_v; }
        L.vel = s->v; L.out = G->rho_v;
        if (L.mforce) hipLaunchKernelGGL((k6_v<TY, true, false, true>), grid, block, 0, ctx->stream, g, L, kc, E);
        else hipLaunchKernelGGL((k6_v<TY, false, false, true>), grid, block, 0, ctx->stream, g, L, kc, E);
    } else {
        ProfileScope ps(ctx, Ein ? "z_momentum_tendency+rk3" : "z_momentum_tendency");
        if (Ein) { E.u0 = U0->rho_w; E.u0_out = U0->rho_w; }
        L.vel = s->w; L.out = G->rho_w;
        if (bm == 0) hipLaunchKernelGGL((k6_w<TY, false, false, false, 0>), grid, block, 0, ctx->stream, g, L, kc, E);
        else if (bm == 1) hipLaunchKernelGGL((k6_w<TY, false, false, false, 1>), grid, block, 0, ctx->stream, g, L, kc, E);
        else if (bm == 2) hipLaunchKernelGGL((k6_w<TY, false, false, false, 2>), grid, block, 0, ctx->stream, g, L, kc, E);
        else hipLaunchKernelGGL((k6_w<TY, false, false, false, 3>), grid, block, 0, ctx->stream, g, L, kc, E);
    }
    BZ_LAUNCH_CHECK();
    return BZ_OK;
}

int bzi_tendencies_lean(bz_ctx *ctx, const bz_state *s, const bz_prognostic *U0, const bz_prognostic *G, const double *pa,
                        const double *pb, double *oa, double *ob, double dt, double alpha, bool first, int rows, int which)
{
    return lean_launch<8>(ctx, s, U0, G, pa, pb, oa, ob, dt, alpha, first, rows, which);
}
```

breeze.jl_amd/csrc/bz_tendency5_kernels.h:

```cpp
#pragma once
#include "bz_internal.h"
#include "bz_weno.h"
#include "bz_tendency4_kernels.h"

#ifndef BZ_KO
#define BZ_KO 0
#endif
#ifndef BZ6_ROTATE_DUTY
#define BZ6_ROTATE_DUTY 0
#endif
#ifndef BZ6_UNROLL2
#define BZ6_UNROLL2 0
#endif
#ifndef BZ6_LDS_BARRIER
#define BZ6_LDS_BARRIER 0
#endif
__device__ __forceinline__ void bz6_barrier()
{
#if BZ6_LDS_BARRIER
    __builtin_amdgcn_fence(__ATOMIC_RELEASE, "workgroup", "local");
    __builtin_amdgcn_s_barrier();
    __builtin_amdgcn_fence(__ATOMIC_ACQUIRE, "workgroup", "local");
#else
    __syncthreads();
#endif
}
typedef long long ix_t;
typedef unsigned ix32_t;

struct LevRow5 {
    double rho, rrho;
    double rho_f, rrho_f;
    double Ax, Ay, Vinv_c;
    double pi;
    double Vinv_f, T_r;
    double pad[6];
};
struct Lev5 {
    const LevRow5 *p;
#ifdef __HIPCC__
    __device__ __forceinline__ double at(int k, int f) const { return ((ColPtr::cptr)(const double *)p)[(long long)k * 16 + f]; }
    __device__ __forceinline__ double rho(int k) const { return at(k, 0); }
    __device__ __forceinline__ double rrho(int k) const { return at(k, 1); }
    __device__ __forceinline__ double rho_f(int k) const { return at(k, 2); }
    __device__ __forceinline__ double rrho_f(int k) const { return at(k, 3); }
    __device__ __forceinline__ double Ax(int k) const { return at(k, 4); }
    __device__ __forceinline__ double Ay(int k) const { return at(k, 5); }
    __device__ __forceinline__ double Vinv_c(int k) const { return at(k, 6); }
    __device__ __forceinline__ double pi(int k) const { return at(k, 7); }
    __device__ __forceinline__ double Vinv_f(int k) const { return at(k, 8); }
    __device__ __forceinline__ double T_r(int k) const { return at(k, 9); }
#endif
};
static_assert(sizeof(LevRow5) == 16 * sizeof(double), "LevRow5 is sixteen reals");

#ifndef BZ_LEAN_WAVES
#define BZ_LEAN_WAVES (sizeof(double) == 8 ? 4 : 6)
#endif
#ifndef BZ5_ZERO_SHORTCUT
#define BZ5_ZERO_SHORTCUT 1
#endif
#ifndef BZ5_TOPS_AHEAD
#define BZ5_TOPS_AHEAD 1
#endif
#ifndef BZ6_W_WAVES
#define BZ6_W_WAVES 4
#endif
#ifndef BZ5_EB
#define BZ5_EB 64
#endif
#ifndef BZ5_RAW_LDS
#define BZ5_RAW_LDS 0
#endif
#ifndef BZ5_SCALAR_WAVES
#define BZ5_SCALAR_WAVES (sizeof(double) == 8 ? 4 : 6)
#endif

struct Lean5 {
    const double *ru, *rv, *rw;
    const double *pa, *pb;
    double *out;
    double *oa, *ob;
    double *T;
    ColPtr pi_dry;
    const LevRow5 *lev;
    int mforce;
    double cor_f;
    ColPtr Fu, Fv;
    ColPtr Su, Sv;
    const double *vel, *bT, *bq;
    const int *qstate;
    int xcd;
    int by0, bys;
};

__device__ __forceinline__ void bz_block5(const Lean5 &L, int &bx, int &by, int &bz)
{
    bx = blockIdx.x; by = blockIdx.y; bz = blockIdx.z;
    if (L.xcd) {
        const unsigned gx = gridDim.x, gy = gridDim.y;
        const unsigned W = gx * gy * gridDim.z;
        unsigned w = bx + gx * (by + gy * bz);
        w = (w & 7u) * (W >> 3) + (w >> 3);
        bx = (int)(w % gx);
        by = (int)((w / gx) % gy);
        bz = (int)(w / (gx * gy));
    }
    by = L.by0 + by * L.bys;
    bx = __builtin_amdgcn_readfirstlane(bx);
    by = __builtin_amdgcn_readfirstlane(by);
    bz = __builtin_amdgcn_readfirstlane(bz);
}

__device__ __forceinline__ void st_img5(double *__restrict__ f, long long n, double v, long long ox, long long oy)
{
    f[n] = v;
    if (ox) f[n + ox] = v;
    if (oy) {
        f[n + oy] = v;
        if (ox) f[n + ox + oy] = v;
    }
}


__device__ __forceinline__ double bz_temperature5(const DevGrid &g, double rth, double rq, int k, const ColPtr pi_dry)
{
    const double rho = g.rho[k], rrho = g.rrho[k];
    const double th = bz_cdiv(rth, rho, rrho), q = bz_cdiv(rq, rho, rrho);
    if (pi_dry.p && __all(q == 0.0)) return pi_dry[k] * th;
    const double qd = 1.0 - q;
    const double cpm = qd * g.cpd + q * g.cpv;
    return bz_exner_factor(g, k, q, cpm) * th;
}

__device__ __forceinline__ double bz_temperature5r(const DevGrid &g, double rth, double rq, int k, double rho, double rrho, double pi)
{
    const double th = bz_cdiv(rth, rho, rrho), q = bz_cdiv(rq, rho, rrho);
    if (__all(q == 0.0)) return pi * th;
    const double qd = 1.0 - q;
    const double cpm = qd * g.cpd + q * g.cpv;
    return bz_exner_factor(g, k, q, cpm) * th;
}

template <bool WY> __device__ __forceinline__ int by5_face(const DevGrid &g, int j) { return WY ? bz_buffer_face(j, g.Ny) : 3; }
template <bool WY> __device__ __forceinline__ int by5_center(const DevGrid &g, int j) { return WY ? bz_buffer_center(j, g.Ny) : 3; }
template <bool WY>
__device__ __forceinline__ double bz_up5y(double m3, double m2, double m1, double p0, double p1, double p2, bool left, int B)
{
    if constexpr (WY) return bz_upB(m3, m2, m1, p0, p1, p2, left, B);
    else return bz_up5(m3, m2, m1, p0, p1, p2, left);
}
template <bool WY>
__device__ __forceinline__ double bz_symm4y(double qm2, double qm1, double q0, double qp1, int B)
{
    if constexpr (WY) return (B == 3) ? bz_symm4(qm2, qm1, q0, qp1) : bz_symm2(qm1, q0);
    else return bz_symm4(qm2, qm1, q0, qp1);
}

template <int TY, bool WY, bool DRYQ>
__device__ __forceinline__ void k5_scalar_pair_body(const DevGrid &g, const Lean5 &F, int kchunk, const RKEpilogue &E, double *Tp, double *FYp, int *ZF, double *RAWp)
{
    constexpr bool Q = !DRYQ;
    constexpr int TR = TY + 6, TC = 72;
    constexpr int NHALO = TR * 70 - TY * 64;
    constexpr int NT = 64 * TY;
    constexpr int HPT = (NHALO + NT - 1) / NT;
    double(*T)[2][TR][TC] = (double(*)[2][TR][TC])Tp;
    double(*FY)[2][TY + 1][64] = (double(*)[2][TY + 1][64])FYp;
    double *__restrict__ RAW = RAWp;
    constexpr bool ZS = BZ5_ZERO_SHORTCUT && Q;

    int bx, by, bz;
    bz_block5(F, bx, by, bz);
    const int tx = threadIdx.x, ty = threadIdx.y, t = ty * 64 + tx;
    const int tyu = __builtin_amdgcn_readfirstlane(ty);
    const Lev5 LV{F.lev};
    const int i0 = bx * 64, j0 = by * TY;
    const int i = i0 + tx, j = j0 + ty;
    const int ic = min(i, g.Nx + 2), jc = min(j, g.Ny + 2);
    const int nact = min(64, g.Nx - i0);
    const int ie = i0 + nact, le = nact - 1;
    const int kbeg = bz * kchunk, kend = min(kbeg + kchunk, g.Nz);
    if (kbeg >= kend) return;
    const int Byj = by5_face<WY>(g, j0 + tyu), Byt = by5_face<WY>(g, j0 + TY);
    const unsigned sz = (unsigned)g.Sxy;
    const bool store = (i < g.Nx) && (j < g.Ny);
    const double *__restrict__ ru = F.ru, *__restrict__ rv = F.rv, *__restrict__ rw = F.rw;
    const double *__restrict__ pa = F.pa, *__restrict__ pb = F.pb;
    unsigned n = (unsigned)g.idx(ic, jc, kbeg);

    int hr[HPT], hc[HPT];
    unsigned hn[HPT];
    bool hok[HPT];
#pragma unroll
    for (int q = 0; q < HPT; ++q) {
        const int h = t + q * NT;
        hok[q] = h < NHALO;
        int r, c;
        if (h < 6 * 70) {
            const int rr = h / 70;
            c = h - rr * 70;
            r = (rr < 3) ? rr : TY + rr;
        } else {
            const int hh = h - 6 * 70;
            const int rr = hh / 6, cc = hh - rr * 6;
            r = 3 + rr;
            c = (cc < 3) ? cc : 64 + cc;
        }
        if (!hok[q]) { r = 0; c = 0; }
        hr[q] = r; hc[q] = c;
        const int gi = min(i0 - 3 + c, g.Nx + 2), gj = min(j0 - 3 + r, g.Ny + 2);
        hn[q] = (unsigned)g.idx(gi, gj, kbeg);
    }
    const unsigned ntop0 = (unsigned)g.idx(ic, min(j0 + TY, g.Ny), kbeg);

    double a[6], b[6];
    double araw[3] = {0.0, 0.0, 0.0};
#pragma unroll
    for (int s = 0; s < 6; ++s) {
        const double rh = g.rho[kbeg + s - 3], rr = g.rrho[kbeg + s - 3];
        const double raw = pa[n + s * sz - 3 * sz];
        a[s] = bz_cdiv(raw, rh, rr);
        if (DRYQ && s >= 3) araw[s - 3] = raw;
        if constexpr (Q) {
            const double rawb = pb[n + s * sz - 3 * sz];
            b[s] = bz_cdiv(rawb, rh, rr);
            if (BZ5_RAW_LDS && s >= 3) { RAW[((s - 3) * 2 + 0) * NT + t] = raw; RAW[((s - 3) * 2 + 1) * NT + t] = rawb; }
        } else b[s] = 0.0;
    }
    double fza, fzb = 0.0;
    {
        const double wt = bz_cdiv(rw[n], g.rho_f[kbeg], g.rrho_f[kbeg]);
        const bool left = wt > 0.0;
        const int B = bz_buffer_face(kbeg, g.Nz);
        const double cf = g.Az * wt, rf = g.rho_f[kbeg];
        fza = rf * (cf * bz_upB(a[0], a[1], a[2], a[3], a[4], a[5], left, B));
        if constexpr (Q) fzb = rf * (cf * bz_upB(b[0], b[1], b[2], b[3], b[4], b[5], left, B));
    }
    int zrun = 0;
    if constexpr (ZS) {
#pragma unroll
        for (int s = 0; s < 6; ++s) zrun = (b[s] == 0.0) ? zrun + 1 : 0;
        if (t < 3) ZF[t] = 1;
        __syncthreads();
    }
    T[0][0][ty + 3][tx + 3] = a[3];
    if constexpr (Q) T[0][1][ty + 3][tx + 3] = b[3];
    {
        const double rh = g.rho[kbeg], rr = g.rrho[kbeg];
        bool z0 = (b[3] == 0.0);
#pragma unroll
        for (int q = 0; q < HPT; ++q)
            if (hok[q]) {
                T[0][0][hr[q]][hc[q]] = bz_cdiv(pa[hn[q]], rh, rr);
                if constexpr (Q) {
                    const double hbv = bz_cdiv(pb[hn[q]], rh, rr);
                    T[0][1][hr[q]][hc[q]] = hbv;
                    z0 = z0 && (hbv == 0.0);
                }
            }
        if (ZS && !__all(z0) && tx == 0) ZF[0] = 0;
    }
    __syncthreads();

    double ea = 0.0, eb = 0.0;
    int buf = 0;
    double ru_n = ru[n], rv_n = rv[n], rw_n = rw[n + sz];
    double rvtop_n = (tyu == 0 || (Q && tyu == TY / 2)) ? rv[ntop0] : 0.0;
    double ta_nx = 0.0, tb_nx = 0.0;
    if constexpr (BZ5_TOPS_AHEAD) { ta_nx = pa[n + 3 * sz]; if constexpr (Q) tb_nx = pb[n + 3 * sz]; }
    for (int k = kbeg; k < kend; ++k, n += sz) {
        double ha[HPT], hb[HPT];
        const unsigned lev = (unsigned)(k + 1 - kbeg) * sz;
        double ta_raw, tb_raw = 0.0;
        if constexpr (BZ5_TOPS_AHEAD) {
            ta_raw = ta_nx; tb_raw = tb_nx;
            const unsigned up = (k + 4 <= g.Nz + g.Hz - 1) ? 4 * sz : 3 * sz;
            ta_nx = pa[n + up];
            if constexpr (Q) tb_nx = pb[n + up];
        } else { ta_raw = pa[n + 3 * sz]; if constexpr (Q) tb_raw = pb[n + 3 * sz]; }
        const int lv3 = (ZS || (Q && BZ5_RAW_LDS)) ? (k - kbeg) % 3 : 0;
        bool zxy = false;
        if constexpr (ZS) {
            if (t == 0) ZF[(lv3 + 2) % 3] = 1;
            zxy = __builtin_amdgcn_readfirstlane(ZF[lv3]) != 0;
        }
#pragma unroll
        for (int q = 0; q < HPT; ++q) {
            if (BZ_KO & 2) { ha[q] = ta_raw; hb[q] = tb_raw; }
            else { ha[q] = hok[q] ? pa[hn[q] + lev] : 0.0; hb[q] = (Q && hok[q]) ? pb[hn[q] + lev] : 0.0; }
        }
        const double u0a = (BZ_KO & 16) ? ta_raw : (E.mode == 2) ? E.u0[n] : 0.0, u0b = (BZ_KO & 16) ? tb_raw : (Q && E.mode == 2) ? E.u0b[n] : 0.0;
        const double ru_t = ru_n, rv_t = rv_n, rw_t = rw_n, rvtop = rvtop_n;
        const int turn = (k - kbeg) & (TY - 1);
        const bool duty_a = tyu == turn, duty_b = Q && tyu == ((turn + TY / 2) & (TY - 1));
        if (BZ_KO & 32) { ru_n = ta_raw * 1e-3; rv_n = tb_raw; rw_n = ta_raw * 1e-4; } else {
        ru_n = ru[n + sz]; rv_n = rv[n + sz]; rw_n = rw[n + 2 * sz]; }
        {
            const int turn_n = (turn + 1) & (TY - 1);
            const bool duty_n = tyu == turn_n || (Q && tyu == ((turn_n + TY / 2) & (TY - 1)));
            rvtop_n = duty_n ? rv[ntop0 + lev] : 0.0;
        }
        const double rho = LV.rho(k), rrho = LV.rrho(k), Ax_k = LV.Ax(k), Ay_k = LV.Ay(k), Vi_k = LV.Vinv_c(k);
        const double rho1 = LV.rho(k + 1), rrho1 = LV.rrho(k + 1), rhof1 = LV.rho_f(k + 1), rrhof1 = LV.rrho_f(k + 1);
        const double rho3 = LV.rho(k + 3), rrho3 = LV.rrho(k + 3);
        if (((k - kbeg) & (BZ5_EB - 1)) == 0) {
            const int kk = min(k + (tx & (BZ5_EB - 1)), kend - 1);
            const long long ne = g.idx(ie, jc, kk);
            const double rhk = g.rho[kk], rrk = g.rrho[kk];
            const double ue = bz_cdiv(ru[ne], rhk, rrk);
            const bool le_ = ue > 0.0;
            const double cf = g.Ax[kk] * ue;
            ea = rhk * (cf * bz_up5(bz_cdiv(pa[ne - 3], rhk, rrk), bz_cdiv(pa[ne - 2], rhk, rrk), bz_cdiv(pa[ne - 1], rhk, rrk),
                                    bz_cdiv(pa[ne], rhk, rrk), bz_cdiv(pa[ne + 1], rhk, rrk), bz_cdiv(pa[ne + 2], rhk, rrk), le_));
            if constexpr (Q)
            eb = rhk * (cf * bz_up5(bz_cdiv(pb[ne - 3], rhk, rrk), bz_cdiv(pb[ne - 2], rhk, rrk), bz_cdiv(pb[ne - 1], rhk, rrk),
                                    bz_cdiv(pb[ne], rhk, rrk), bz_cdiv(pb[ne + 1], rhk, rrk), bz_cdiv(pb[ne + 2], rhk, rrk), le_));
        }
        const int src = (k - kbeg) & (BZ5_EB - 1);
        const double ut = bz_cdiv(ru_t, rho, rrho), vt = bz_cdiv(rv_t, rho, rrho);
        const double wt = bz_cdiv(rw_t, rhof1, rrhof1);
        const double cfx = Ax_k * ut, cfy = Ay_k * vt, cfz = g.Az * wt, rf = rhof1;
        const bool lx = ut > 0.0, ly = vt > 0.0, lz = wt > 0.0;
        const int Bz = bz_buffer_face(k + 1, g.Nz);
        double cfy2 = 0.0;
        bool ly2 = false;
        if (duty_a || duty_b) {
            const double vtop = bz_cdiv(rvtop, rho, rrho);
            ly2 = vtop > 0.0;
            cfy2 = Ay_k * vtop;
        }
        const int c = tx + 3;
        double fxa, fya, fza_hi, fxb, fyb, fzb_hi;
        const double ta = bz_cdiv(ta_raw, rho3, rrho3);
        {
            const double(*Tk)[TC] = T[buf][0];
            const double *rr_ = Tk[ty + 3] + tx;
            fxa = rho * (cfx * bz_up5(rr_[0], rr_[1], rr_[2], a[3], rr_[4], rr_[5], lx));
            fya = rho * (cfy * bz_up5y<WY>(Tk[ty][c], Tk[ty + 1][c], Tk[ty + 2][c], a[3], Tk[ty + 4][c], Tk[ty + 5][c], ly, Byj));
            FY[buf][0][ty][tx] = fya;
            if (duty_a)
                FY[buf][0][TY][tx] = rho * (cfy2 * bz_up5y<WY>(Tk[TY][c], Tk[TY + 1][c], Tk[TY + 2][c], Tk[TY + 3][c], Tk[TY + 4][c], Tk[TY + 5][c], ly2, Byt));
            fza_hi = rf * (cfz * bz_upB(a[1], a[2], a[3], a[4], a[5], ta, lz, Bz));
        }
        double tb = 0.0;
        fxb = 0.0; fyb = 0.0; fzb_hi = 0.0;
        if constexpr (Q) {
        tb = bz_cdiv(tb_raw, rho3, rrho3);
        bool zz = false;
        if constexpr (ZS) {
            zrun = (tb == 0.0) ? min(zrun + 1, 6) : 0;
            zz = __all(zrun >= 6);
        }
        if (zxy) {
            fxb = 0.0; fyb = 0.0;
            FY[buf][1][ty][tx] = 0.0;
            if (duty_b) FY[buf][1][TY][tx] = 0.0;
        } else {
            const double(*Tk)[TC] = T[buf][1];
            const double *rr_ = Tk[ty + 3] + tx;
            if (BZ_KO & 128) { fxb = rho * (cfx * b[3]); fyb = rho * (cfy * b[3]); } else {
            fxb = rho * (cfx * bz_up5(rr_[0], rr_[1], rr_[2], b[3], rr_[4], rr_[5], lx));
            fyb = rho * (cfy * bz_up5y<WY>(Tk[ty][c], Tk[ty + 1][c], Tk[ty + 2][c], b[3], Tk[ty + 4][c], Tk[ty + 5][c], ly, Byj)); }
            FY[buf][1][ty][tx] = fyb;
            if (duty_b)
                FY[buf][1][TY][tx] = rho * (cfy2 * bz_up5y<WY>(Tk[TY][c], Tk[TY + 1][c], Tk[TY + 2][c], Tk[TY + 3][c], Tk[TY + 4][c], Tk[TY + 5][c], ly2, Byt));
        }
        if (zz) fzb_hi = 0.0;
        else fzb_hi = (BZ_KO & 128) ? rf * (cfz * b[3]) : rf * (cfz * bz_upB(b[1], b[2], b[3], b[4], b[5], tb, lz, Bz));
        }
        double pa_n, pb_n;
        if constexpr (DRYQ) { pa_n = araw[0]; pb_n = b[3]; araw[0] = araw[1]; araw[1] = araw[2]; araw[2] = ta_raw; }
        else if (BZ_KO & 4) { pa_n = a[3]; pb_n = b[3]; }
        else if constexpr (BZ5_RAW_LDS) {
            double *ra = RAW + (lv3 * 2 + 0) * NT + t, *rb = ra + NT;
            pa_n = *ra; pb_n = *rb;
            *ra = ta_raw; *rb = tb_raw;
        } else { pa_n = pa[n]; pb_n = pb[n]; }
        T[buf ^ 1][0][ty + 3][tx + 3] = a[4];
        if constexpr (Q) T[buf ^ 1][1][ty + 3][tx + 3] = b[4];
        {
            const double rh = rho1, rr = rrho1;
            bool z1 = (b[4] == 0.0);
#pragma unroll
            for (int q = 0; q < HPT; ++q)
                if (hok[q]) {
                    T[buf ^ 1][0][hr[q]][hc[q]] = bz_cdiv(ha[q], rh, rr);
                    if constexpr (Q) {
                        const double hbv = bz_cdiv(hb[q], rh, rr);
                        T[buf ^ 1][1][hr[q]][hc[q]] = hbv;
                        z1 = z1 && (hbv == 0.0);
                    }
                }
            if (ZS && !__all(z1) && tx == 0) ZF[(lv3 + 1) % 3] = 0;
        }
        if (!(BZ_KO & 64)) __syncthreads();
        {
            double na = __shfl_down(fxa, 1);
            const double xa = __shfl(ea, src);
            if (tx == le) na = xa;
            const double dya = FY[buf][0][ty + 1][tx] - fya;
            const double Vi = Vi_k;
            const double ga = -(Vi * ((na - fxa) + dya + (fza_hi - fza)));
            double gb = 0.0;
            if constexpr (Q) {
                double nb = __shfl_down(fxb, 1);
                const double xb = __shfl(eb, src);
                if (tx == le) nb = xb;
                const double dyb = FY[buf][1][ty + 1][tx] - fyb;
                gb = -(Vi * ((nb - fxb) + dyb + (fzb_hi - fzb)));
            }
            if (store) {
                const double rth = bz_rk_apply_pre(E.mode, E.dt, E.alpha, E.oma, u0a, E.u0_out, ga, pa_n, n);
                F.oa[n] = rth;
                if constexpr (Q) {
                    const double rq = bz_rk_apply_pre(E.mode, E.dt, E.alpha, E.oma, u0b, E.u0b_out, gb, pb_n, n);
                    F.ob[n] = rq;
                }
            }
        }
        fza = fza_hi; fzb = fzb_hi;
#pragma unroll
        for (int s = 0; s < 5; ++s) { a[s] = a[s + 1]; b[s] = b[s + 1]; }
        a[5] = ta; b[5] = tb;
        buf ^= 1;
    }
}


template <bool DRYQ, bool GUARD>
__device__ __forceinline__ bool bz_lean_skip(const Lean5 &F)
{
    if constexpr (!GUARD) return false;
    const bool dry = F.qstate != nullptr && __builtin_amdgcn_readfirstlane(*F.qstate) == 1;
    return dry != DRYQ;
}
template <int TY, bool WY = false, bool DRYQ = false, bool GUARD = true>
__global__ __launch_bounds__(64 * TY) __attribute__((amdgpu_waves_per_eu(BZ5_SCALAR_WAVES, BZ5_SCALAR_WAVES))) void k5_scalar_pair(DevGrid g, Lean5 F, int kchunk, RKEpilogue E)
{
    constexpr int TR = TY + 6, TC = 72;
    __shared__ double T[2 * 2 * TR * TC];
    __shared__ double FY[2 * 2 * (TY + 1) * 64];
    __shared__ int ZF[3];
    __shared__ double RAW[(!DRYQ && BZ5_RAW_LDS) ? 3 * 2 * 64 * TY : 1];
    if (bz_lean_skip<DRYQ, GUARD>(F)) return;
    k5_scalar_pair_body<TY, WY, DRYQ>(g, F, kchunk, E, T, FY, ZF, RAW);
}

template <int KIND>
__device__ __forceinline__ double flux_x_lean(const DevGrid &g, const Tend3Fields &F, const double *__restrict__ m, int i, int j, int k, int By = 3)
{
    const long long n = g.idx(i, j, k);
    const double a = (KIND == T3_V && By != 3) ? bz_symm2(g.Ax[k] * F.ru[n - g.Sx], g.Ax[k] * F.ru[n]) : adv_x<KIND>(g, F, n, k);
    const double rh = (KIND == T3_W) ? g.rho_f[k] : g.rho[k], rr = (KIND == T3_W) ? g.rrho_f[k] : g.rrho[k];
    if constexpr (KIND == T3_U)
        return a * bz_up5(bz_cdiv(m[n - 2], rh, rr), bz_cdiv(m[n - 1], rh, rr), bz_cdiv(m[n], rh, rr), bz_cdiv(m[n + 1], rh, rr),
                          bz_cdiv(m[n + 2], rh, rr), bz_cdiv(m[n + 3], rh, rr), a > 0.0);
    else
        return a * bz_up5(bz_cdiv(m[n - 3], rh, rr), bz_cdiv(m[n - 2], rh, rr), bz_cdiv(m[n - 1], rh, rr), bz_cdiv(m[n], rh, rr),
                          bz_cdiv(m[n + 1], rh, rr), bz_cdiv(m[n + 2], rh, rr), a > 0.0);
}


template <int TY, bool MF = false, bool WY = false, bool ST = false>
__global__ __launch_bounds__(64 * TY, BZ_LEAN_WAVES) void k6_u(DevGrid g, Lean5 L, int kchunk, RKEpilogue E)
{
    static_assert(!(ST && WY), "stored-velocity instantiations: periodic / slab rows");
    constexpr int TR = TY + 6, TC = 72, NT = 64 * TY;
    constexpr int NH1 = TR * 70 - TY * 64;
    constexpr int NH2 = 3 * (TY + 1) + 64 + 3 * TY;
    static_assert(NH1 <= NT && NH2 <= NT, "one frame cell of each kind per thread");
    __shared__ double U[2][TR][TC];
    __shared__ double RU[2][TY][TC];
    __shared__ double RV[2][TY + 1][TC];
    __shared__ double RW[2][TY][TC];
    __shared__ double FY[2][TY + 1][64];
    int bx, by, bz;
    bz_block5(L, bx, by, bz);
    const int tx = threadIdx.x, ty = threadIdx.y, t = ty * 64 + tx, tc = tx + 3;
    const int i0 = bx * 64, j0 = by * TY;
    const int i = i0 + tx, j = j0 + ty;
    const int ic = min(i, g.Nx + 2), jc = min(j, g.Ny + 2);
    const int ie = i0 - 1, le = 0;
    const int kbeg = bz * kchunk, kend = min(kbeg + kchunk, g.Nz);
    if (kbeg >= kend) return;
    const ix_t sz = (ix_t)g.Sxy;
    const bool store = (i < g.Nx) && (j < g.Ny);
    const double *__restrict__ ru = L.ru, *__restrict__ rv = L.rv, *__restrict__ rw = L.rw;
    const double *__restrict__ vel = ST ? L.vel : L.ru;
    Tend3Fields F;
    F.ru = L.ru; F.rv = L.rv; F.rw = L.rw; F.u = F.v = F.w = F.T = F.q = nullptr; F.c = ST ? L.vel : nullptr; F.G = L.out;
    ix_t n = (ix_t)g.idx(ic, jc, kbeg);
    const bool h1ok = !(BZ_KO & 32768) && t < NH1;
    int h1r = 0, h1c = 0;
    {
        const int h = h1ok ? t : 0;
        if (h < 6 * 70) { const int rr = h / 70; h1c = h - rr * 70; h1r = (rr < 3) ? rr : TY + rr; }
        else { const int hh = h - 6 * 70, rr = hh / 6, cc = hh - rr * 6; h1r = 3 + rr; h1c = (cc < 3) ? cc : 64 + cc; }
    }
    const ix_t h1n = (ix_t)g.idx(min(i0 - 3 + h1c, g.Nx + 2), min(j0 - 3 + h1r, g.Ny + 2), kbeg);
    const bool h1raw = h1ok && h1r >= 3 && h1r < TY + 3 && (h1c == 2 || h1c == 67 || h1c == 68);
    const bool h2ok = !(BZ_KO & 32768) && t < NH2;
    int h2sel = 0, h2r = 0, h2c = 0;
    {
        const int id = h2ok ? t : 0;
        if (id < 3 * (TY + 1)) { h2r = id / 3; const int cc = id - 3 * h2r; h2c = (cc < 2) ? 1 + cc : 67; }
        else if (id < 3 * (TY + 1) + 64) { h2r = TY; h2c = 3 + (id - 3 * (TY + 1)); }
        else { h2sel = 1; const int m = id - 3 * (TY + 1) - 64; h2r = m / 3; const int cc = m - 3 * h2r; h2c = (cc < 2) ? 1 + cc : 67; }
    }
    const double *__restrict__ h2src = h2sel ? rw : rv;
    const ix_t h2n = (ix_t)g.idx(min(i0 - 3 + h2c, g.Nx + 2), min(j0 + h2r, g.Ny + 2), kbeg) + (h2sel ? sz : (ix_t)0);

    double r[6];
#pragma unroll
    for (int s = 0; s < 6; ++s) r[s] = ST ? vel[n + s * sz - 3 * sz] : bz_cdiv(ru[n + s * sz - 3 * sz], g.rho[kbeg + s - 3], g.rrho[kbeg + s - 3]);
    double fz_lo = vflux<T3_U>(g, F, n, kbeg, r[0], r[1], r[2], r[3], r[4], r[5]);
    double q0 = ru[n], q1 = ru[n + sz], q2 = ru[n + 2 * sz];
    U[0][ty + 3][tc] = r[3];
    RU[0][ty][tc] = q0;
    RV[0][ty][tc] = rv[n];
    RW[0][ty][tc] = rw[n + sz];
    if (h1ok) {
        const double raw = (ST && !h1raw) ? 0.0 : ru[h1n];
        U[0][h1r][h1c] = ST ? vel[h1n] : bz_cdiv(raw, g.rho[kbeg], g.rrho[kbeg]);
        if (h1raw) RU[0][h1r - 3][h1c] = raw;
    }
    if (h2ok) { if (h2sel) RW[0][h2r][h2c] = h2src[h2n]; else RV[0][h2r][h2c] = h2src[h2n]; }
    double tcur_raw = ru[n + 3 * sz];
    double tcur_v = ST ? vel[n + 3 * sz] : 0.0;
    double u0cur = (E.mode == 2) ? E.u0[n] : 0.0;
    __syncthreads();

    double edge = 0.0;
    int buf = 0;
#if BZ6_UNROLL2
#pragma unroll 2
#endif
    for (int k = kbeg; k < kend; ++k, n += sz) {
        const ix_t lev1 = (ix_t)(k + 1 - kbeg) * sz;
        const double p_top = ST ? ru[n + sz] : ru[n + ((k + 4 <= g.Nz + g.Hz - 1) ? 4 * sz : 3 * sz)];
        const double p_topv = ST ? vel[n + ((k + 4 <= g.Nz + g.Hz - 1) ? 4 * sz : 3 * sz)] : 0.0;
        const double p_h1 = (BZ_KO & 256) ? p_top : h1ok ? (ST ? vel : ru)[h1n + lev1] : 0.0;
        const double p_h1raw = (ST && h1raw) ? ru[h1n + lev1] : 0.0;
        const double p_h2 = (BZ_KO & 512) ? p_top : h2ok ? h2src[h2n + lev1] : 0.0;
        const double p_rv = (BZ_KO & 1024) ? p_top * 0.5 : rv[n + sz], p_rw = (BZ_KO & 1024) ? p_top * 0.25 : rw[n + 2 * sz];
        const double p_u0 = (BZ_KO & 2048) ? p_top : (E.mode == 2) ? E.u0[n + sz] : 0.0;
        if (((k - kbeg) & (BZ5_EB - 1)) == 0) {
            const int kk = min(k + (tx & (BZ5_EB - 1)), kend - 1);
            edge = ST ? flux_x_at<T3_U>(g, F, ie, jc, kk) : flux_x_lean<T3_U>(g, F, ru, ie, jc, kk);
        }
        const int src = (k - kbeg) & (BZ5_EB - 1);
        const double Ax = g.Ax[k], Ay = g.Ay[k], Az = g.Az;
        const double c0 = r[3];
        const double(*Uk)[TC] = U[buf];
        const double *rur = RU[buf][ty] + tc, *ur = Uk[ty + 3] + tc;
        const double ax = bz_symm4(Ax * rur[-1], Ax * q0, Ax * rur[1], Ax * rur[2]);
        const double fx = ax * bz_up5(ur[-2], ur[-1], c0, ur[1], ur[2], ur[3], ax > 0.0);
        const double *rvr = RV[buf][ty] + tc;
        const double ay = bz_symm4(Ay * rvr[-2], Ay * rvr[-1], Ay * rvr[0], Ay * rvr[1]);
        const double fy = ay * bz_up5y<WY>(Uk[ty][tc], Uk[ty + 1][tc], Uk[ty + 2][tc], c0, Uk[ty + 4][tc], Uk[ty + 5][tc], ay > 0.0, by5_face<WY>(g, __builtin_amdgcn_readfirstlane(j)));
        FY[buf][ty][tx] = fy;
        if (ty == (BZ6_ROTATE_DUTY ? ((k - kbeg) & (TY - 1)) : 0) && !(BZ_KO & 4096)) {
            const double *rvt = RV[buf][TY] + tc;
            const double at = bz_symm4(Ay * rvt[-2], Ay * rvt[-1], Ay * rvt[0], Ay * rvt[1]);
            FY[buf][TY][tx] = at * bz_up5y<WY>(Uk[TY][tc], Uk[TY + 1][tc], Uk[TY + 2][tc], Uk[TY + 3][tc], Uk[TY + 4][tc], Uk[TY + 5][tc], at > 0.0,
                                               by5_face<WY>(g, j0 + TY));
        }
        const double tnew = ST ? tcur_v : bz_cdiv(tcur_raw, g.rho[k + 3], g.rrho[k + 3]);
        const double *rwr = RW[buf][ty] + tc;
        const double wt = bz_symm4(Az * rwr[-2], Az * rwr[-1], Az * rwr[0], Az * rwr[1]);
        const double fz_hi = wt * bz_upB(r[1], r[2], r[3], r[4], r[5], tnew, wt > 0.0, bz_buffer_face(k + 1, g.Nz));
        U[buf ^ 1][ty + 3][tc] = r[4];
        RU[buf ^ 1][ty][tc] = ST ? p_top : q1;
        RV[buf ^ 1][ty][tc] = p_rv;
        RW[buf ^ 1][ty][tc] = p_rw;
        if (h1ok) {
            U[buf ^ 1][h1r][h1c] = ST ? p_h1 : bz_cdiv(p_h1, g.rho[k + 1], g.rrho[k + 1]);
            if (h1raw) RU[buf ^ 1][h1r - 3][h1c] = ST ? p_h1raw : p_h1;
        }
        if (h2ok) { if (h2sel) RW[buf ^ 1][h2r][h2c] = p_h2; else RV[buf ^ 1][h2r][h2c] = p_h2; }
        if (!(BZ_KO & 16384) && (!(BZ_KO & 8192) || ((k - kbeg) & 1))) bz6_barrier();
        {
            double nb = __shfl_up(fx, 1);
            const double e = __shfl(edge, src);
            if (tx == le) nb = e;
            const double dx = fx - nb;
            const double dy = (BZ_KO & 16384) ? 0.5 * fy : FY[buf][ty + 1][tx] - fy;
            double Gu = -(g.Vinv_c[k] * (dx + dy + (fz_hi - fz_lo)));
            if constexpr (MF) {
                if (L.mforce & 1) {
                    const double *rv0 = RV[buf][ty] + tc, *rv1 = RV[buf][ty + 1] + tc;
                    const double a = (rv0[-1] + rv1[-1]) / 2, b = (rv0[0] + rv1[0]) / 2;
                    Gu -= -L.cor_f * ((a + b) / 2);
                }
                if (L.mforce & (2 | 8)) {
                    const double rho = g.rho[k];
                    double tot = (L.mforce & 8) ? rho * L.Su[k] : 0.0;
                    if (L.mforce & 2) tot = (L.mforce & 8) ? tot + rho * L.Fu[k] : rho * L.Fu[k];
                    Gu += tot;
                }
            }
            if (store) L.out[n] = (ST && E.mode == 0) ? Gu : bz_rk_apply_pre(E.mode, E.dt, E.alpha, E.oma, u0cur, E.u0_out, Gu, q0, n);
        }
        fz_lo = fz_hi;
#pragma unroll
        for (int s = 0; s < 5; ++s) r[s] = r[s + 1];
        r[5] = tnew;
        if (ST) q0 = p_top;
        else { q0 = q1; q1 = q2; q2 = tcur_raw; tcur_raw = p_top; }
        u0cur = p_u0;
        if (ST) tcur_v = p_topv;
        buf ^= 1;
    }
}


template <int TY, bool MF = false, bool WY = false, bool ST = false>
__global__ __launch_bounds__(64 * TY, ((MF && WY) ? 4 : BZ_LEAN_WAVES)) void k6_v(DevGrid g, Lean5 L, int kchunk, RKEpilogue E)
{
    static_assert(!(ST && WY), "stored-velocity instantiations: periodic / slab rows");
    constexpr int RV = TY + 6, RM = TY + 4;
    constexpr int TC = 72;
    __shared__ double Tv[2][RV][TC];
    __shared__ double Tm[2][3][RM][64];
    __shared__ double FY[2][TY + 1][64];
    constexpr int NT = 64 * TY, NFR = 16 * 64, HPT = (NFR + NT - 1) / NT;
    int bx, by, bz;
    bz_block5(L, bx, by, bz);
    const int tx = threadIdx.x, ty = threadIdx.y, t = ty * 64 + tx, tc = tx + 3;
    const int i0 = bx * 64, j0 = by * TY;
    const int i = i0 + tx, j = j0 + ty;
    const int ic = min(i, g.Nx + 2), jc = min(j, g.Ny + 2);
    const int nact = min(64, g.Nx - i0);
    const int ie = i0 + nact, le = nact - 1;
    const int kbeg = bz * kchunk, kend = min(kbeg + kchunk, g.Nz);
    if (kbeg >= kend) return;
    const ix_t sz = (ix_t)g.Sxy;
    const bool store = (i < g.Nx) && (j < g.Ny) && !(WY && j == 0);
    const int ju = __builtin_amdgcn_readfirstlane(j);
    const int Bf = by5_face<WY>(g, ju), Bc = by5_center<WY>(g, ju), Bc0 = by5_center<WY>(g, j0 - 1);
    const double *__restrict__ ru = L.ru, *__restrict__ rv = L.rv, *__restrict__ rw = L.rw;
    const double *__restrict__ vel = ST ? L.vel : L.rv;
    Tend3Fields F;
    F.ru = L.ru; F.rv = L.rv; F.rw = L.rw; F.u = F.v = F.w = F.T = F.q = nullptr; F.c = ST ? L.vel : nullptr; F.G = L.out;
    const double Az = g.Az;
    ix_t n = (ix_t)g.idx(ic, jc, kbeg);

    bool hok[HPT];
    int hsel[HPT], hrow[HPT];
    ix_t hn[HPT];
    const double *hsrc[HPT];
#pragma unroll
    for (int q = 0; q < HPT; ++q) {
        const int h = t + q * NT;
        hok[q] = h < NFR;
        const int id = __builtin_amdgcn_readfirstlane(hok[q] ? (h >> 6) : 0);
        int sel, row, grow;
        if (id < 6) { sel = 0; row = (id < 3) ? id : TY + id; grow = j0 - 3 + row; }
        else if (id < 9) { sel = 1; const int m = id - 6; row = (m < 2) ? m : TY + 2; grow = j0 - 2 + row; }
        else if (id < 13) { sel = 2; const int m = id - 9; row = (m < 2) ? m : TY + m; grow = j0 - 2 + row; }
        else { sel = 3; const int m = id - 13; row = (m < 2) ? m : TY + 2; grow = j0 - 2 + row; }
        hsel[q] = sel; hrow[q] = row;
        hsrc[q] = (sel == 1) ? ru : (sel == 3) ? rw : (ST && sel == 0) ? vel : rv;
        hn[q] = (ix_t)g.idx(min(i0 + tx, g.Nx + 2), min(grow, g.Ny + 2), kbeg) + (sel == 3 ? sz : (ix_t)0);
    }
    auto frame_load = [&](int q, ix_t lev) -> double { return hsrc[q][hn[q] + lev]; };
    auto frame_store = [&](int b, int q, double raw, int klev) {
        if (hsel[q] == 0) Tv[b][hrow[q]][tc] = ST ? raw : bz_cdiv(raw, g.rho[klev], g.rrho[klev]);
        else Tm[b][hsel[q] - 1][hrow[q]][tx] = ((hsel[q] == 1) ? g.Ax[klev] : (hsel[q] == 2) ? g.Ay[klev] : Az) * raw;
    };

    const bool sok = t < 5 * TY;
    const int srow = sok ? t / 5 : 0, scc = sok ? t % 5 : 0, scol = (scc < 3) ? scc : 64 + scc;
    const ix_t sn = (ix_t)g.idx(min(i0 - 3 + scol, g.Nx + 2), min(j0 + srow, g.Ny + 2), kbeg);

    double r[6];
#pragma unroll
    for (int s = 0; s < 6; ++s) r[s] = ST ? vel[n + s * sz - 3 * sz] : bz_cdiv(rv[n + s * sz - 3 * sz], g.rho[kbeg + s - 3], g.rrho[kbeg + s - 3]);
    double fz_lo;
    if (WY && Bf != 3) {
        const double wt0 = bz_symm2(Az * rw[n - (ix_t)g.Sx], Az * rw[n]);
        fz_lo = wt0 * bz_upB(r[0], r[1], r[2], r[3], r[4], r[5], wt0 > 0.0, bz_buffer_face(kbeg, g.Nz));
    } else fz_lo = vflux<T3_V>(g, F, n, kbeg, r[0], r[1], r[2], r[3], r[4], r[5]);
    double q0 = rv[n], q1 = rv[n + sz], q2 = rv[n + 2 * sz];
    Tv[0][ty + 3][tc] = r[3];
    if (sok) Tv[0][srow + 3][scol] = ST ? vel[sn] : bz_cdiv(rv[sn], g.rho[kbeg], g.rrho[kbeg]);
    Tm[0][0][ty + 2][tx] = g.Ax[kbeg] * ru[n];
    Tm[0][1][ty + 2][tx] = g.Ay[kbeg] * q0;
    Tm[0][2][ty + 2][tx] = Az * rw[n + sz];
#pragma unroll
    for (int q = 0; q < HPT; ++q)
        if (hok[q]) frame_store(0, q, frame_load(q, 0), kbeg);
    __syncthreads();

    double tcur_raw = rv[n + 3 * sz];
    double tcur_v = ST ? vel[n + 3 * sz] : 0.0;
    double u0cur = (E.mode == 2) ? E.u0[n] : 0.0;
    double edge = 0.0;
    int buf = 0;
    for (int k = kbeg; k < kend; ++k, n += sz) {
        const ix_t lev = (ix_t)(k + 1 - kbeg) * sz;
        double hnext[HPT];
#pragma unroll
        for (int q = 0; q < HPT; ++q) hnext[q] = hok[q] ? frame_load(q, lev) : 0.0;
        const double p_side = sok ? (ST ? vel : rv)[sn + lev] : 0.0;
        const double p_top = ST ? rv[n + sz] : rv[n + ((k + 4 <= g.Nz + g.Hz - 1) ? 4 * sz : 3 * sz)];
        const double p_topv = ST ? vel[n + ((k + 4 <= g.Nz + g.Hz - 1) ? 4 * sz : 3 * sz)] : 0.0;
        const double p_u0 = (E.mode == 2) ? E.u0[n + sz] : 0.0;
        const double tnew_raw = tcur_raw, u0v = u0cur;
        const double ru_n = g.Ax[k + 1] * ru[n + sz], rw_n = Az * rw[n + 2 * sz];
        double cor_u = 0.0, cg1 = 0.0, cg3 = 0.0;
        if constexpr (MF) { if ((L.mforce & 1) && tx == 63) { const ix_t sy = (ix_t)g.Sx; cg1 = ru[n - sy + 1]; cg3 = ru[n + 1]; } }
        if (((k - kbeg) & (BZ5_EB - 1)) == 0) {
            const int kk = min(k + (tx & (BZ5_EB - 1)), kend - 1);
            edge = ST ? flux_x_at<T3_V>(g, F, ie, jc, kk) : flux_x_lean<T3_V>(g, F, rv, ie, jc, kk, Bf);
        }
        const int src = (k - kbeg) & (BZ5_EB - 1);
        const double rho = g.rho[k];
        const double c0 = r[3];
        const double(*V)[TC] = Tv[buf];
        const double *vrow = V[ty + 3] + tc;
        const double(*MU)[64] = Tm[buf][0];
        const double(*MV)[64] = Tm[buf][1];
        const double(*MW)[64] = Tm[buf][2];
        const double ut = bz_symm4y<WY>(MU[ty][tx], MU[ty + 1][tx], MU[ty + 2][tx], MU[ty + 3][tx], Bf);
        const double fx = ut * bz_up5(vrow[-3], vrow[-2], vrow[-1], c0, vrow[1], vrow[2], ut > 0.0);
        const double vt = (!WY || Bc == 3) ? bz_symm4(MV[ty + 1][tx], MV[ty + 2][tx], MV[ty + 3][tx], MV[ty + 4][tx]) : bz_symm2(MV[ty + 2][tx], MV[ty + 3][tx]);
        const double fy = vt * bz_up5y<WY>(V[ty + 1][tc], V[ty + 2][tc], c0, V[ty + 4][tc], V[ty + 5][tc], V[ty + 6][tc], vt > 0.0, Bc);
        FY[buf][ty + 1][tx] = fy;
        if (ty == 0 && !(BZ_KO & 4096)) {
            const double vb = (!WY || Bc0 == 3) ? bz_symm4(MV[0][tx], MV[1][tx], MV[2][tx], MV[3][tx]) : bz_symm2(MV[1][tx], MV[2][tx]);
            FY[buf][0][tx] = vb * bz_up5y<WY>(V[0][tc], V[1][tc], V[2][tc], V[3][tc], V[4][tc], V[5][tc], vb > 0.0, Bc0);
        }
        const double tnew = ST ? tcur_v : bz_cdiv(tnew_raw, g.rho[k + 3], g.rrho[k + 3]);
        const double wt = bz_symm4y<WY>(MW[ty][tx], MW[ty + 1][tx], MW[ty + 2][tx], MW[ty + 3][tx], Bf);
        const double fz_hi = wt * bz_upB(r[1], r[2], r[3], r[4], r[5], tnew, wt > 0.0, bz_buffer_face(k + 1, g.Nz));
        if constexpr (MF) {
            if (L.mforce & 1) {
                const double Axk = g.Ax[k];
                const double l1 = MU[ty + 1][tx + 1], l3 = MU[ty + 2][tx + 1];
                const double c1 = (tx == 63) ? Axk * cg1 : l1, c3 = (tx == 63) ? Axk * cg3 : l3;
                cor_u = (((MU[ty + 1][tx] + c1) / 2 + (MU[ty + 2][tx] + c3) / 2) / 2) / Axk;
            }
        }
        Tv[buf ^ 1][ty + 3][tc] = r[4];
        if (sok) Tv[buf ^ 1][srow + 3][scol] = ST ? p_side : bz_cdiv(p_side, g.rho[k + 1], g.rrho[k + 1]);
        Tm[buf ^ 1][0][ty + 2][tx] = ru_n;
        Tm[buf ^ 1][1][ty + 2][tx] = g.Ay[k + 1] * (ST ? p_top : q1);
        Tm[buf ^ 1][2][ty + 2][tx] = rw_n;
#pragma unroll
        for (int q = 0; q < HPT; ++q)
            if (hok[q]) frame_store(buf ^ 1, q, hnext[q], k + 1);
        bz6_barrier();
        {
            double nb = __shfl_down(fx, 1);
            const double e = __shfl(edge, src);
            if (tx == le) nb = e;
            const double dx = nb - fx;
            const double dy = fy - FY[buf][ty][tx];
            double Gv = -(g.Vinv_c[k] * (dx + dy + (fz_hi - fz_lo)));
            if constexpr (MF) {
                if (L.mforce & 1) Gv -= L.cor_f * cor_u;
                if (L.mforce & (4 | 16)) {
                    double tot = (L.mforce & 16) ? rho * L.Sv[k] : 0.0;
                    if (L.mforce & 4) tot = (L.mforce & 16) ? tot + rho * L.Fv[k] : rho * L.Fv[k];
                    Gv += tot;
                }
            }
            if (store) L.out[n] = (ST && E.mode == 0) ? Gv : bz_rk_apply_pre(E.mode, E.dt, E.alpha, E.oma, u0v, E.u0_out, Gv, q0, n);
            if constexpr (WY) {
                if (i < g.Nx && j == 0) L.out[n] = 0.0;
                if (i < g.Nx && j == g.Ny - 1) L.out[n + (ix_t)g.Sx] = 0.0;
            }
        }
        fz_lo = fz_hi;
        if (ST) q0 = p_top;
        else { q0 = q1; q1 = q2; q2 = tnew_raw; tcur_raw = p_top; }
        u0cur = p_u0;
        if (ST) tcur_v = p_topv;
#pragma unroll
        for (int s = 0; s < 5; ++s) r[s] = r[s + 1];
        r[5] = tnew;
        buf ^= 1;
    }
}

__device__ __forceinline__ double buoyancy5(const DevGrid &g, double rth, double rq, int k, double rho, double rrho, double pi, double T_ref)
{
    const double th = bz_cdiv(rth, rho, rrho), q = bz_cdiv(rq, rho, rrho);
    double T;
    if (__all(q == 0.0)) T = pi * th;
    else {
        const double qd = 1.0 - q;
        const double cpm = qd * g.cpd + q * g.cpv;
        T = bz_exner_factor(g, k, q, cpm) * th;
    }
    const double Rm = (1.0 - q) * g.Rd + q * g.Rv;
    const double rhop = rho * (g.Rd * T_ref / (Rm * T) - 1.0);
    return -g.g * rhop;
}


template <int TY, bool WY = false, bool DRYQ = false, bool GUARD = true, int BM = 4>
__global__ __launch_bounds__(64 * TY, BZ6_W_WAVES) void k6_w(DevGrid g, Lean5 L, int kchunk, RKEpilogue E)
{
    constexpr bool ST = BM != 4;
    static_assert(!(ST && (WY || DRYQ || GUARD)), "stored-velocity instantiations: periodic / slab rows, no moisture-scan dispatch");
    if (bz_lean_skip<DRYQ, GUARD>(L)) return;
    constexpr int TR = TY + 6, TC = 72, NT = 64 * TY, NH = TR * 70 - TY * 64;
    static_assert(NH <= NT, "one frame cell per thread");
    __shared__ double T[2][TR][TC];
    __shared__ double FY[2][TY + 1][64];
    int bx, by, bz;
    bz_block5(L, bx, by, bz);
    const int tx = threadIdx.x, ty = threadIdx.y, t = ty * 64 + tx, tc = tx + 3;
    const int i0 = bx * 64, j0 = by * TY;
    const int i = i0 + tx, j = j0 + ty;
    const int ic = min(i, g.Nx + 2), jc = min(j, g.Ny + 2);
    const int nact = min(64, g.Nx - i0);
    const int ie = i0 + nact, le = nact - 1;
    const int kbeg = 1 + bz * kchunk, kend = min(kbeg + kchunk, g.Nz);
    if (kbeg >= kend) return;
    const ix32_t sz = (ix32_t)g.Sxy;
    const bool store = (i < g.Nx) && (j < g.Ny);
    const double *__restrict__ ru = L.ru, *__restrict__ rv = L.rv, *__restrict__ rw = L.rw;
    const double *__restrict__ pa = L.pa, *__restrict__ pb = L.pb;
    const double *__restrict__ vel = ST ? L.vel : L.rw;
    const double *__restrict__ bT = L.bT, *__restrict__ bq = L.bq;
    const Lev5 LV{L.lev};
    constexpr bool dryq = DRYQ;
    Tend3Fields F;
    F.ru = L.ru; F.rv = L.rv; F.rw = L.rw; F.u = F.v = F.w = F.T = F.q = nullptr; F.c = ST ? L.vel : nullptr; F.G = L.out;
    const double Az = g.Az;
    ix32_t n = (ix32_t)g.idx(ic, jc, kbeg);
    const bool hok = t < NH;
    int hr = 0, hc = 0;
    {
        const int h = hok ? t : 0;
        if (h < 6 * 70) { const int rr = h / 70; hc = h - rr * 70; hr = (rr < 3) ? rr : TY + rr; }
        else { const int hh = h - 6 * 70, rr = hh / 6, cc = hh - rr * 6; hr = 3 + rr; hc = (cc < 3) ? cc : 64 + cc; }
    }
    const ix32_t hn = (ix32_t)g.idx(min(i0 - 3 + hc, g.Nx + 2), min(j0 - 3 + hr, g.Ny + 2), kbeg);
    const ix32_t ntop0 = (ix32_t)g.idx(ic, min(j0 + TY, g.Ny), kbeg);
    const bool top = (ty == 0);

    double wr[6], qu[4], qv[4], qt[4], qw[4];
    double raw0 = 0.0, raw1 = 0.0, raw2 = 0.0;
#pragma unroll
    for (int s = 0; s < 6; ++s) {
        const double x = rw[n + s * sz - 3 * sz];
        wr[s] = ST ? vel[n + s * sz - 3 * sz] : bz_cdiv(x, LV.rho_f(kbeg + s - 3), LV.rrho_f(kbeg + s - 3));
        if (s >= 1 && s <= 4) qw[s - 1] = Az * x;
        if (s == 3) raw0 = x;
        if (s == 4) raw1 = x;
        if (s == 5) raw2 = x;
    }
#pragma unroll
    for (int s = 0; s < 4; ++s) {
        const int kk = kbeg - 2 + s;
        const double Axk = ST ? g.Ax[kk] : LV.Ax(kk), Ayk = ST ? g.Ay[kk] : LV.Ay(kk);
        qu[s] = Axk * ru[n + s * sz - 2 * sz];
        qv[s] = Ayk * rv[n + s * sz - 2 * sz];
        qt[s] = top ? Ayk * rv[ntop0 + s * sz - 2 * sz] : 0.0;
    }
    double fz_lo, b_lo, r_lo = 0.0;
    {
        const int B = bz_buffer_center(kbeg - 1, g.Nz);
        const double wt = (B == 3) ? bz_symm4(qw[0], qw[1], qw[2], qw[3]) : bz_symm2(qw[1], qw[2]);
        fz_lo = wt * bz_upB(wr[0], wr[1], wr[2], wr[3], wr[4], wr[5], wt > 0.0, B);
        if constexpr (BM == 4) b_lo = buoyancy5(g, pa[n - sz], dryq ? 0.0 : pb[n - sz], kbeg - 1, LV.rho(kbeg - 1), LV.rrho(kbeg - 1), LV.pi(kbeg - 1), LV.T_r(kbeg - 1));
        else if constexpr (BM == 0) b_lo = buoyancy3(g, bT[n - sz], bq[n - sz], kbeg - 1);
        else if constexpr (BM == 3) b_lo = bz_buoyancy(g, bT, bq, (long long)(n - sz), kbeg - 1);
        else if constexpr (BM == 2) { b_lo = bT[n - sz] - g.p_r[kbeg - 1]; r_lo = bq[n - sz] - g.rho[kbeg - 1]; }
        else b_lo = 0.0;
    }
    T[0][ty + 3][tc] = wr[3];
    if (hok) T[0][hr][hc] = ST ? vel[hn] : bz_cdiv(rw[hn], LV.rho_f(kbeg), LV.rrho_f(kbeg));
    double tcur_raw = rw[n + 3 * sz];
    double tcur_v = ST ? vel[n + 3 * sz] : 0.0;
    double u0cur = (E.mode == 2) ? E.u0[n] : 0.0;
    __syncthreads();

    double edge = 0.0;
    int buf = 0;
    for (int k = kbeg; k < kend; ++k, n += sz) {
        const ix32_t lev = (ix32_t)(k - kbeg) * sz;
        const double p_h = hok ? (ST ? vel : rw)[hn + lev + sz] : 0.0;
        const double p_top = rw[n + ((k + 4 <= g.Nz + g.Hz) ? 4 * sz : 3 * sz)];
        const double p_topv = ST ? vel[n + ((k + 4 <= g.Nz + g.Hz) ? 4 * sz : 3 * sz)] : 0.0;
        const double Tcur = (BM == 1) ? 0.0 : (ST ? bT : pa)[n], rqcur = (BM == 1) ? 0.0 : ST ? bq[n] : dryq ? 0.0 : pb[n];
        const double p_u0 = (E.mode == 2) ? E.u0[n + sz] : 0.0;
        const double Axn = ST ? g.Ax[k + 2] : LV.Ax(k + 2), Ayn = ST ? g.Ay[k + 2] : LV.Ay(k + 2);
        const double qun = Axn * ru[n + 2 * sz], qvn = Ayn * rv[n + 2 * sz];
        const double qtn = top ? Ayn * rv[ntop0 + lev + 2 * sz] : 0.0;
        if (((k - kbeg) & (BZ5_EB - 1)) == 0) {
            const int kk = min(k + (tx & (BZ5_EB - 1)), kend - 1);
            edge = ST ? flux_x_at<T3_W>(g, F, ie, jc, kk) : flux_x_lean<T3_W>(g, F, rw, ie, jc, kk);
        }
        const int src = (k - kbeg) & (BZ5_EB - 1);
        const int Bf = bz_buffer_face(k, g.Nz);
        const double w0 = wr[3];
        const double qwnew = Az * (ST ? rw[n + 2 * sz] : raw2);
        const double uold = ST ? rw[n] : raw0;
        const double(*Tk)[TC] = T[buf];
        const double *wrow = Tk[ty + 3] + tc;
        const double ut = (Bf == 3) ? bz_symm4(qu[0], qu[1], qu[2], qu[3]) : bz_symm2(qu[1], qu[2]);
        const double fx = ut * bz_up5(wrow[-3], wrow[-2], wrow[-1], w0, wrow[1], wrow[2], ut > 0.0);
        const double vt = (Bf == 3) ? bz_symm4(qv[0], qv[1], qv[2], qv[3]) : bz_symm2(qv[1], qv[2]);
        const double fy = vt * bz_up5y<WY>(Tk[ty][tc], Tk[ty + 1][tc], Tk[ty + 2][tc], w0, Tk[ty + 4][tc], Tk[ty + 5][tc], vt > 0.0, by5_face<WY>(g, __builtin_amdgcn_readfirstlane(j)));
        FY[buf][ty][tx] = fy;
        if (top && !(BZ_KO & 4096)) {
            const double v2 = (Bf == 3) ? bz_symm4(qt[0], qt[1], qt[2], qt[3]) : bz_symm2(qt[1], qt[2]);
            FY[buf][TY][tx] = v2 * bz_up5y<WY>(Tk[TY][tc], Tk[TY + 1][tc], Tk[TY + 2][tc], Tk[TY + 3][tc], Tk[TY + 4][tc], Tk[TY + 5][tc], v2 > 0.0,
                                               by5_face<WY>(g, j0 + TY));
        }
        const double wnew = ST ? tcur_v : bz_cdiv(tcur_raw, LV.rho_f(k + 3), LV.rrho_f(k + 3));
        double fz_hi;
        {
            const int B = bz_buffer_center(k, g.Nz);
            const double wt = (B == 3) ? bz_symm4(qw[1], qw[2], qw[3], qwnew) : bz_symm2(qw[2], qw[3]);
            fz_hi = wt * bz_upB(wr[1], wr[2], wr[3], wr[4], wr[5], wnew, wt > 0.0, B);
        }
        double b_hi = 0.0, r_hi = 0.0;
        if constexpr (BM == 4) b_hi = buoyancy5(g, Tcur, rqcur, k, LV.rho(k), LV.rrho(k), LV.pi(k), LV.T_r(k));
        else if constexpr (BM == 0) b_hi = buoyancy3(g, Tcur, rqcur, k);
        else if constexpr (BM == 3) b_hi = bz_buoyancy(g, bT, bq, (long long)n, k);
        else if constexpr (BM == 2) { b_hi = Tcur - g.p_r[k]; r_hi = rqcur - g.rho[k]; }
        T[buf ^ 1][ty + 3][tc] = wr[4];
        if (hok) T[buf ^ 1][hr][hc] = ST ? p_h : bz_cdiv(p_h, LV.rho_f(k + 1), LV.rrho_f(k + 1));
        bz6_barrier();
        {
            double nb = __shfl_down(fx, 1);
            const double e = __shfl(edge, src);
            if (tx == le) nb = e;
            const double dx = nb - fx;
            const double dy = FY[buf][ty + 1][tx] - fy;
            const double adv = -((ST ? g.Vinv_f[k] : LV.Vinv_f(k)) * (dx + dy + (fz_hi - fz_lo)));
            double Gval;
            if constexpr (BM == 2) Gval = adv - (b_hi - b_lo) * g.rdzf[k] - g.g * ((r_hi + r_lo) / 2.0);
            else if constexpr (BM == 1) Gval = adv;
            else Gval = adv + 0.5 * (b_lo + b_hi);
            if (store)
                L.out[n] = (ST && E.mode == 0) ? Gval : bz_rk_apply_pre(E.mode, E.dt, E.alpha, E.oma, u0cur, E.u0_out, Gval, uold, n);
        }
        fz_lo = fz_hi;
        b_lo = b_hi;
        r_lo = r_hi;
#pragma unroll
        for (int s = 0; s < 3; ++s) { qu[s] = qu[s + 1]; qv[s] = qv[s + 1]; qt[s] = qt[s + 1]; qw[s] = qw[s + 1]; }
        qu[3] = qun; qv[3] = qvn; qt[3] = qtn; qw[3] = qwnew;
        raw0 = raw1; raw1 = raw2; raw2 = tcur_raw;
        tcur_raw = p_top; u0cur = p_u0;
        if (ST) tcur_v = p_topv;
#pragma unroll
        for (int s = 0; s < 5; ++s) wr[s] = wr[s + 1];
        wr[5] = wnew;
        buf ^= 1;
    }
}
```

Before: 4.200 billion.

## Use uniform per-level bases with 32-bit lane byte offsets in lean tendency kernels

```diff
diff --git a/breeze.jl_amd/csrc/bz_acoustic_kernels.h b/breeze.jl_amd/csrc/bz_acoustic_kernels.h
--- a/breeze.jl_amd/csrc/bz_acoustic_kernels.h
+++ b/breeze.jl_amd/csrc/bz_acoustic_kernels.h
@@ -303,12 +303,12 @@
 template <class T>
 __device__ __forceinline__ T ac_ld(const T *base, unsigned e)
 {
-    return *(const T *)((const char *)base + (size_t)(e * (unsigned)sizeof(T)));
+    return lean_ld(base, e);
 }
 template <class T, class V>
 __device__ __forceinline__ void ac_st(T *base, unsigned e, V v)
 {
-    *(T *)((char *)base + (size_t)(e * (unsigned)sizeof(T))) = (T)v;
+    lean_st(base, e, v);
 }
 #ifndef AC2_NT
 #define AC2_NT 0
diff --git a/breeze.jl_amd/csrc/bz_internal.h b/breeze.jl_amd/csrc/bz_internal.h
--- a/breeze.jl_amd/csrc/bz_internal.h
+++ b/breeze.jl_amd/csrc/bz_internal.h
@@ -98,6 +98,56 @@
                                                   double uold, long long n)
 {
     if (mode == 1) { u0_out[n] = uold; u0v = uold; }
+    else if (mode == 3) u0v = uold;
+    return oma * u0v + alpha * (uold + dt * G);
+}
+template <class T>
+__device__ __forceinline__ T lean_ldb(const T *uniform_base, unsigned byte_offset)
+{
+    typedef const char __attribute__((address_space(1))) *gbytes;
+    typedef const T __attribute__((address_space(1))) *gptr;
+    return *(gptr)((gbytes)uniform_base + (size_t)byte_offset);
+}
+template <class T, class V>
+__device__ __forceinline__ void lean_stb(T *uniform_base, unsigned byte_offset, V v)
+{
+    typedef char __attribute__((address_space(1))) *gbytes;
+    typedef T __attribute__((address_space(1))) *gptr;
+    *(gptr)((gbytes)uniform_base + (size_t)byte_offset) = (T)v;
+}
+template <class T>
+__device__ __forceinline__ T lean_ld(const T *uniform_base, unsigned e)
+{
+    return lean_ldb(uniform_base, e * (unsigned)sizeof(T));
+}
+template <class T, class V>
+__device__ __forceinline__ void lean_st(T *uniform_base, unsigned e, V v)
+{
+    lean_stb(uniform_base, e * (unsigned)sizeof(T), v);
+}
+__device__ __forceinline__ void lean_pin(unsigned &lane_offset) { asm("" : "+v"(lane_offset)); }
+template <class P>
+__device__ __forceinline__ P *lean_ub(P *uniform_base) { asm("" : "+s"(uniform_base)); return uniform_base; }
+__device__ __forceinline__ double lean_in_vgpr(double x) { asm("" : "+v"(x)); return x; }
+template <bool PIN = true, class T>
+__device__ __forceinline__ T lean_ldp(const T *uniform_base, unsigned &byte_offset)
+{
+    if constexpr (!PIN) return lean_ldb(uniform_base, byte_offset);
+    lean_pin(byte_offset);
+    return lean_ldb(lean_ub(uniform_base), byte_offset);
+}
+template <bool PIN = true, class T, class V>
+__device__ __forceinline__ void lean_stp(T *uniform_base, unsigned &byte_offset, V v)
+{
+    if constexpr (!PIN) { lean_stb(uniform_base, byte_offset, v); return; }
+    lean_pin(byte_offset);
+    lean_stb(lean_ub(uniform_base), byte_offset, v);
+}
+template <bool PIN = true>
+__device__ __forceinline__ double bz_rk_apply_lev(int mode, double dt, double alpha, double oma, double u0v, double *u0_lev, double G,
+                                                  double uold, unsigned &byte_offset)
+{
+    if (mode == 1) { lean_stp<PIN>(u0_lev, byte_offset, uold); u0v = uold; }
     else if (mode == 3) u0v = uold;
     return oma * u0v + alpha * (uold + dt * G);
 }
@@ -621,6 +671,7 @@
 void bzi_compressible_teardown(bz_ctx *ctx);
 void bzi_balance_teardown(bz_ctx *ctx);
 int bzi_refresh_reference_columns(bz_ctx *ctx, const double *density, const double *pressure);
+bool bzi_lean_plane_ok(const DevGrid &g);
 bool bzi_k6_stored_ok(const bz_ctx *ctx);
 int bzi_k6_stored(bz_ctx *ctx, int comp, const bz_state *s, const bz_prognostic *G, const bz_prognostic *U0, const RKEpilogue *Ein, int bm);
 int bzi_scalar_pair_tendency(bz_ctx *ctx, const bz_state *s, const bz_prognostic *G, const bz_prognostic *U0 = nullptr,
diff --git a/breeze.jl_amd/csrc/bz_step.hip b/breeze.jl_amd/csrc/bz_step.hip
--- a/breeze.jl_amd/csrc/bz_step.hip
+++ b/breeze.jl_amd/csrc/bz_step.hip
@@ -36,7 +36,7 @@
     const bool fused_tier = !slab;
     if ((ctx->fused_ok || walls_lean) && lean_switches && order5 && lean_anelastic && theta_model && g.microphysics == 0 && lean_forcings &&
         !ctx->has_bulk && !ctx->has_closure && !ctx->has_diffusivity && !ctx->has_relaxation && ctx->n_tracers == 0 && !ctx->bounded_mask &&
-        (long long)g.Sxy * (g.Nz + 2 * g.Hz + 1) < (1LL << 32))
+        (long long)g.Sxy * (g.Nz + 2 * g.Hz + 1) < (1LL << 32) && bzi_lean_plane_ok(g))
         return BZ_TIER_LEAN;
     if ((ctx->fused_ok || (walls_lean && ctx->weno_R != 3)) && ctx->fuse_rk && rk_orders && theta_model && g.microphysics != 2 &&
         !ctx->bounded_mask && !ctx->has_relaxation && rk_forcings)
diff --git a/breeze.jl_amd/csrc/bz_tendency5.hip b/breeze.jl_amd/csrc/bz_tendency5.hip
--- a/breeze.jl_amd/csrc/bz_tendency5.hip
+++ b/breeze.jl_amd/csrc/bz_tendency5.hip
@@ -24,6 +24,11 @@
     r.Vinv_f = g.Vinv_f[k]; r.T_r = g.T_r[k];
     for (int q = 0; q < 6; ++q) r.pad[q] = 0.0;
     rows[t] = r;
+}
+
+bool bzi_lean_plane_ok(const DevGrid &g)
+{
+    return (unsigned long long)(g.Sxy + g.Sx + 1) * sizeof(double) < (1ULL << 32);
 }
 
 int bzi_lean_setup(bz_ctx *ctx)
@@ -96,6 +101,7 @@
                        const double *pb, double *oa, double *ob, double dt, double alpha, bool first, int rows, int which)
 {
     const DevGrid &g = ctx->dg;
+    if (!bzi_lean_plane_ok(g)) { ctx->last_error = "lean tendency kernels: an x-y plane of the padded arrays exceeds 32-bit byte offsets"; return BZ_ERR_UNSUPPORTED; }
     RKEpilogue E;
     E.mode = first ? 3 : 2; E.dt = dt; E.alpha = alpha; E.oma = 1.0 - alpha;
     Lean5 L;
@@ -187,13 +193,14 @@
 {
     const DevGrid &g = ctx->dg;
     return !ctx->tune.no_k6_stored && !g.flat_y && !g.bounded_x && !g.bounded_y && g.Nz > 1 &&
-           (long long)g.Sxy * (g.Nz + 2 * g.Hz + 1) < (1LL << 32);
+           (long long)g.Sxy * (g.Nz + 2 * g.Hz + 1) < (1LL << 32) && bzi_lean_plane_ok(g);
 }
 
 int bzi_k6_stored(bz_ctx *ctx, int comp, const bz_state *s, const bz_prognostic *G, const bz_prognostic *U0, const RKEpilogue *Ein, int bm)
 {
     constexpr int TY = 8;
     const DevGrid &g = ctx->dg;
+    if (!bzi_lean_plane_ok(g)) { ctx->last_error = "lean tendency kernels: an x-y plane of the padded arrays exceeds 32-bit byte offsets"; return BZ_ERR_UNSUPPORTED; }
     RKEpilogue E;
     if (Ein) E = *Ein;
     Lean5 L;
diff --git a/breeze.jl_amd/csrc/bz_tendency5_kernels.h b/breeze.jl_amd/csrc/bz_tendency5_kernels.h
--- a/breeze.jl_amd/csrc/bz_tendency5_kernels.h
+++ b/breeze.jl_amd/csrc/bz_tendency5_kernels.h
@@ -25,7 +25,7 @@
     __syncthreads();
 #endif
 }
-typedef long long ix_t;
+__device__ __forceinline__ unsigned bz_pidx5(const DevGrid &g, int i, int j) { return (unsigned)(i + g.Hx) + (unsigned)g.Sx * (unsigned)(j + g.Hy); }
 typedef unsigned ix32_t;
 
 struct LevRow5 {
@@ -484,13 +484,17 @@
     const int ie = i0 - 1, le = 0;
     const int kbeg = bz * kchunk, kend = min(kbeg + kchunk, g.Nz);
     if (kbeg >= kend) return;
-    const ix_t sz = (ix_t)g.Sxy;
+    const long long sz = g.Sxy;
     const bool store = (i < g.Nx) && (j < g.Ny);
     const double *__restrict__ ru = L.ru, *__restrict__ rv = L.rv, *__restrict__ rw = L.rw;
     const double *__restrict__ vel = ST ? L.vel : L.ru;
+    const Lev5 LV{L.lev};
+    auto c_rho = [&](int kk) { return ST ? g.rho[kk] : LV.rho(kk); };
+    auto c_rrho = [&](int kk) { return ST ? g.rrho[kk] : LV.rrho(kk); };
     Tend3Fields F;
     F.ru = L.ru; F.rv = L.rv; F.rw = L.rw; F.u = F.v = F.w = F.T = F.q = nullptr; F.c = ST ? L.vel : nullptr; F.G = L.out;
-    ix_t n = (ix_t)g.idx(ic, jc, kbeg);
+    unsigned o = bz_pidx5(g, ic, jc) * (unsigned)sizeof(double);
+    long long kb = sz * (long long)(kbeg + g.Hz);
     const bool h1ok = !(BZ_KO & 32768) && t < NH1;
     int h1r = 0, h1c = 0;
     {
@@ -498,59 +502,60 @@
         if (h < 6 * 70) { const int rr = h / 70; h1c = h - rr * 70; h1r = (rr < 3) ? rr : TY + rr; }
         else { const int hh = h - 6 * 70, rr = hh / 6, cc = hh - rr * 6; h1r = 3 + rr; h1c = (cc < 3) ? cc : 64 + cc; }
     }
-    const ix_t h1n = (ix_t)g.idx(min(i0 - 3 + h1c, g.Nx + 2), min(j0 - 3 + h1r, g.Ny + 2), kbeg);
+    unsigned h1o = bz_pidx5(g, min(i0 - 3 + h1c, g.Nx + 2), min(j0 - 3 + h1r, g.Ny + 2)) * (unsigned)sizeof(double);
     const bool h1raw = h1ok && h1r >= 3 && h1r < TY + 3 && (h1c == 2 || h1c == 67 || h1c == 68);
-    const bool h2ok = !(BZ_KO & 32768) && t < NH2;
-    int h2sel = 0, h2r = 0, h2c = 0;
-    {
-        const int id = h2ok ? t : 0;
-        if (id < 3 * (TY + 1)) { h2r = id / 3; const int cc = id - 3 * h2r; h2c = (cc < 2) ? 1 + cc : 67; }
-        else if (id < 3 * (TY + 1) + 64) { h2r = TY; h2c = 3 + (id - 3 * (TY + 1)); }
-        else { h2sel = 1; const int m = id - 3 * (TY + 1) - 64; h2r = m / 3; const int cc = m - 3 * h2r; h2c = (cc < 2) ? 1 + cc : 67; }
-    }
-    const double *__restrict__ h2src = h2sel ? rw : rv;
-    const ix_t h2n = (ix_t)g.idx(min(i0 - 3 + h2c, g.Nx + 2), min(j0 + h2r, g.Ny + 2), kbeg) + (h2sel ? sz : (ix_t)0);
+    static_assert(TY >= 3 && 3 * (TY + 1) <= 64, "frame cells of the second kind: one wavefront per kind");
+    const int wv = __builtin_amdgcn_readfirstlane(ty);
+    const int h2sel = (wv == 2) ? 1 : 0;
+    const bool h2ok = !(BZ_KO & 32768) && (wv == 0 || (wv == 1 && tx < 3 * (TY + 1)) || (wv == 2 && tx < 3 * TY));
+    int h2r = TY, h2c = 3 + tx;
+    if (wv != 0) { const int id = h2ok ? tx : 0; h2r = id / 3; const int cc = id - 3 * h2r; h2c = (cc < 2) ? 1 + cc : 67; }
+    const double *__restrict__ h2src = h2sel ? rw + sz : rv;
+    unsigned h2o = bz_pidx5(g, min(i0 - 3 + h2c, g.Nx + 2), min(j0 + h2r, g.Ny + 2)) * (unsigned)sizeof(double);
 
     double r[6];
 #pragma unroll
-    for (int s = 0; s < 6; ++s) r[s] = ST ? vel[n + s * sz - 3 * sz] : bz_cdiv(ru[n + s * sz - 3 * sz], g.rho[kbeg + s - 3], g.rrho[kbeg + s - 3]);
-    double fz_lo = vflux<T3_U>(g, F, n, kbeg, r[0], r[1], r[2], r[3], r[4], r[5]);
-    double q0 = ru[n], q1 = ru[n + sz], q2 = ru[n + 2 * sz];
+    for (int s = 0; s < 6; ++s) r[s] = ST ? lean_ldp(vel + kb + (s - 3) * sz, o) : bz_cdiv(lean_ldp(ru + kb + (s - 3) * sz, o), g.rho[kbeg + s - 3], g.rrho[kbeg + s - 3]);
+    double fz_lo = vflux<T3_U>(g, F, kb + (long long)(o / (unsigned)sizeof(double)), kbeg, r[0], r[1], r[2], r[3], r[4], r[5]);
+    double q0 = lean_ldp(ru + kb, o), q1 = lean_ldp(ru + kb + sz, o), q2 = lean_ldp(ru + kb + 2 * sz, o);
     U[0][ty + 3][tc] = r[3];
     RU[0][ty][tc] = q0;
-    RV[0][ty][tc] = rv[n];
-    RW[0][ty][tc] = rw[n + sz];
+    RV[0][ty][tc] = lean_ldp(rv + kb, o);
+    RW[0][ty][tc] = lean_ldp(rw + kb + sz, o);
     if (h1ok) {
-        const double raw = (ST && !h1raw) ? 0.0 : ru[h1n];
-        U[0][h1r][h1c] = ST ? vel[h1n] : bz_cdiv(raw, g.rho[kbeg], g.rrho[kbeg]);
+        const double raw = (ST && !h1raw) ? 0.0 : lean_ldp(ru + kb, h1o);
+        U[0][h1r][h1c] = ST ? lean_ldp(vel + kb, h1o) : bz_cdiv(raw, g.rho[kbeg], g.rrho[kbeg]);
         if (h1raw) RU[0][h1r - 3][h1c] = raw;
     }
-    if (h2ok) { if (h2sel) RW[0][h2r][h2c] = h2src[h2n]; else RV[0][h2r][h2c] = h2src[h2n]; }
-    double tcur_raw = ru[n + 3 * sz];
-    double tcur_v = ST ? vel[n + 3 * sz] : 0.0;
-    double u0cur = (E.mode == 2) ? E.u0[n] : 0.0;
+    if (h2ok) { if (h2sel) RW[0][h2r][h2c] = lean_ldp(h2src + kb, h2o); else RV[0][h2r][h2c] = lean_ldp(h2src + kb, h2o); }
+    double tcur_raw = lean_ldp(ru + kb + 3 * sz, o);
+    double tcur_v = ST ? lean_ldp(vel + kb + 3 * sz, o) : 0.0;
+    double u0cur = (E.mode == 2) ? lean_ldp(E.u0 + kb, o) : 0.0;
     __syncthreads();
 
     double edge = 0.0;
     int buf = 0;
+    const double Az = lean_in_vgpr(g.Az), rk_dt = lean_in_vgpr(E.dt), rk_alpha = lean_in_vgpr(E.alpha), rk_oma = lean_in_vgpr(E.oma);
+    const double *ru_k = ru + kb, *vel_k = vel + kb, *rv_1 = rv + kb + sz, *rw_2 = rw + kb + 2 * sz, *h2_1 = h2src + kb + sz, *u0_1 = E.u0 + kb + sz;
+    double *out_k = L.out + kb, *u0o_k = E.u0_out + kb;
 #if BZ6_UNROLL2
 #pragma unroll 2
 #endif
-    for (int k = kbeg; k < kend; ++k, n += sz) {
-        const ix_t lev1 = (ix_t)(k + 1 - kbeg) * sz;
-        const double p_top = ST ? ru[n + sz] : ru[n + ((k + 4 <= g.Nz + g.Hz - 1) ? 4 * sz : 3 * sz)];
-        const double p_topv = ST ? vel[n + ((k + 4 <= g.Nz + g.Hz - 1) ? 4 * sz : 3 * sz)] : 0.0;
-        const double p_h1 = (BZ_KO & 256) ? p_top : h1ok ? (ST ? vel : ru)[h1n + lev1] : 0.0;
-        const double p_h1raw = (ST && h1raw) ? ru[h1n + lev1] : 0.0;
-        const double p_h2 = (BZ_KO & 512) ? p_top : h2ok ? h2src[h2n + lev1] : 0.0;
-        const double p_rv = (BZ_KO & 1024) ? p_top * 0.5 : rv[n + sz], p_rw = (BZ_KO & 1024) ? p_top * 0.25 : rw[n + 2 * sz];
-        const double p_u0 = (BZ_KO & 2048) ? p_top : (E.mode == 2) ? E.u0[n + sz] : 0.0;
+    for (int k = kbeg; k < kend; ++k) {
+        const long long up = (k + 4 <= g.Nz + g.Hz - 1) ? 4 * sz : 3 * sz;
+        const double p_top = ST ? lean_ldp(ru_k + sz, o) : lean_ldp(ru_k + up, o);
+        const double p_topv = ST ? lean_ldp(vel_k + up, o) : 0.0;
+        const double p_h1 = (BZ_KO & 256) ? p_top : h1ok ? lean_ldp((ST ? vel_k : ru_k) + sz, h1o) : 0.0;
+        const double p_h1raw = (ST && h1raw) ? lean_ldp(ru_k + sz, h1o) : 0.0;
+        const double p_h2 = (BZ_KO & 512) ? p_top : h2ok ? lean_ldp(h2_1, h2o) : 0.0;
+        const double p_rv = (BZ_KO & 1024) ? p_top * 0.5 : lean_ldp(rv_1, o), p_rw = (BZ_KO & 1024) ? p_top * 0.25 : lean_ldp(rw_2, o);
+        const double p_u0 = (BZ_KO & 2048) ? p_top : (E.mode == 2) ? lean_ldp(u0_1, o) : 0.0;
         if (((k - kbeg) & (BZ5_EB - 1)) == 0) {
             const int kk = min(k + (tx & (BZ5_EB - 1)), kend - 1);
             edge = ST ? flux_x_at<T3_U>(g, F, ie, jc, kk) : flux_x_lean<T3_U>(g, F, ru, ie, jc, kk);
         }
         const int src = (k - kbeg) & (BZ5_EB - 1);
-        const double Ax = g.Ax[k], Ay = g.Ay[k], Az = g.Az;
+        const double Ax = ST ? g.Ax[k] : LV.Ax(k), Ay = ST ? g.Ay[k] : LV.Ay(k);
         const double c0 = r[3];
         const double(*Uk)[TC] = U[buf];
         const double *rur = RU[buf][ty] + tc, *ur = Uk[ty + 3] + tc;
@@ -566,7 +571,7 @@
             FY[buf][TY][tx] = at * bz_up5y<WY>(Uk[TY][tc], Uk[TY + 1][tc], Uk[TY + 2][tc], Uk[TY + 3][tc], Uk[TY + 4][tc], Uk[TY + 5][tc], at > 0.0,
                                                by5_face<WY>(g, j0 + TY));
         }
-        const double tnew = ST ? tcur_v : bz_cdiv(tcur_raw, g.rho[k + 3], g.rrho[k + 3]);
+        const double tnew = ST ? tcur_v : bz_cdiv(tcur_raw, c_rho(k + 3), c_rrho(k + 3));
         const double *rwr = RW[buf][ty] + tc;
         const double wt = bz_symm4(Az * rwr[-2], Az * rwr[-1], Az * rwr[0], Az * rwr[1]);
         const double fz_hi = wt * bz_upB(r[1], r[2], r[3], r[4], r[5], tnew, wt > 0.0, bz_buffer_face(k + 1, g.Nz));
@@ -575,7 +580,7 @@
         RV[buf ^ 1][ty][tc] = p_rv;
         RW[buf ^ 1][ty][tc] = p_rw;
         if (h1ok) {
-            U[buf ^ 1][h1r][h1c] = ST ? p_h1 : bz_cdiv(p_h1, g.rho[k + 1], g.rrho[k + 1]);
+            U[buf ^ 1][h1r][h1c] = ST ? p_h1 : bz_cdiv(p_h1, c_rho(k + 1), c_rrho(k + 1));
             if (h1raw) RU[buf ^ 1][h1r - 3][h1c] = ST ? p_h1raw : p_h1;
         }
         if (h2ok) { if (h2sel) RW[buf ^ 1][h2r][h2c] = p_h2; else RV[buf ^ 1][h2r][h2c] = p_h2; }
@@ -586,7 +591,7 @@
             if (tx == le) nb = e;
             const double dx = fx - nb;
             const double dy = (BZ_KO & 16384) ? 0.5 * fy : FY[buf][ty + 1][tx] - fy;
-            double Gu = -(g.Vinv_c[k] * (dx + dy + (fz_hi - fz_lo)));
+            double Gu = -((ST ? g.Vinv_c[k] : LV.Vinv_c(k)) * (dx + dy + (fz_hi - fz_lo)));
             if constexpr (MF) {
                 if (L.mforce & 1) {
                     const double *rv0 = RV[buf][ty] + tc, *rv1 = RV[buf][ty + 1] + tc;
@@ -594,13 +599,13 @@
                     Gu -= -L.cor_f * ((a + b) / 2);
                 }
                 if (L.mforce & (2 | 8)) {
-                    const double rho = g.rho[k];
+                    const double rho = c_rho(k);
                     double tot = (L.mforce & 8) ? rho * L.Su[k] : 0.0;
                     if (L.mforce & 2) tot = (L.mforce & 8) ? tot + rho * L.Fu[k] : rho * L.Fu[k];
                     Gu += tot;
                 }
             }
-            if (store) L.out[n] = (ST && E.mode == 0) ? Gu : bz_rk_apply_pre(E.mode, E.dt, E.alpha, E.oma, u0cur, E.u0_out, Gu, q0, n);
+            if (store) lean_stp(out_k, o, (ST && E.mode == 0) ? Gu : bz_rk_apply_lev(E.mode, rk_dt, rk_alpha, rk_oma, u0cur, u0o_k, Gu, q0, o));
         }
         fz_lo = fz_hi;
 #pragma unroll
@@ -611,6 +616,7 @@
         u0cur = p_u0;
         if (ST) tcur_v = p_topv;
         buf ^= 1;
+        ru_k += sz; vel_k += sz; rv_1 += sz; rw_2 += sz; h2_1 += sz; u0_1 += sz; out_k += sz; u0o_k += sz;
     }
 }
 
@@ -635,20 +641,27 @@
     const int ie = i0 + nact, le = nact - 1;
     const int kbeg = bz * kchunk, kend = min(kbeg + kchunk, g.Nz);
     if (kbeg >= kend) return;
-    const ix_t sz = (ix_t)g.Sxy;
+    const long long sz = g.Sxy;
     const bool store = (i < g.Nx) && (j < g.Ny) && !(WY && j == 0);
     const int ju = __builtin_amdgcn_readfirstlane(j);
     const int Bf = by5_face<WY>(g, ju), Bc = by5_center<WY>(g, ju), Bc0 = by5_center<WY>(g, j0 - 1);
     const double *__restrict__ ru = L.ru, *__restrict__ rv = L.rv, *__restrict__ rw = L.rw;
     const double *__restrict__ vel = ST ? L.vel : L.rv;
+    const Lev5 LV{L.lev};
+    auto c_rho = [&](int kk) { return ST ? g.rho[kk] : LV.rho(kk); };
+    auto c_rrho = [&](int kk) { return ST ? g.rrho[kk] : LV.rrho(kk); };
+    auto c_Ax = [&](int kk) { return ST ? g.Ax[kk] : LV.Ax(kk); };
+    auto c_Ay = [&](int kk) { return ST ? g.Ay[kk] : LV.Ay(kk); };
     Tend3Fields F;
     F.ru = L.ru; F.rv = L.rv; F.rw = L.rw; F.u = F.v = F.w = F.T = F.q = nullptr; F.c = ST ? L.vel : nullptr; F.G = L.out;
-    const double Az = g.Az;
-    ix_t n = (ix_t)g.idx(ic, jc, kbeg);
+    const double Az = lean_in_vgpr(g.Az);
+    const double rk_dt = lean_in_vgpr(E.dt), rk_alpha = lean_in_vgpr(E.alpha), rk_oma = lean_in_vgpr(E.oma);
+    unsigned o = bz_pidx5(g, ic, jc) * (unsigned)sizeof(double);
+    const long long kb = sz * (long long)(kbeg + g.Hz);
 
     bool hok[HPT];
     int hsel[HPT], hrow[HPT];
-    ix_t hn[HPT];
+    unsigned ho[HPT];
     const double *hsrc[HPT];
 #pragma unroll
     for (int q = 0; q < HPT; ++q) {
@@ -661,62 +674,65 @@
         else if (id < 13) { sel = 2; const int m = id - 9; row = (m < 2) ? m : TY + m; grow = j0 - 2 + row; }
         else { sel = 3; const int m = id - 13; row = (m < 2) ? m : TY + 2; grow = j0 - 2 + row; }
         hsel[q] = sel; hrow[q] = row;
-        hsrc[q] = (sel == 1) ? ru : (sel == 3) ? rw : (ST && sel == 0) ? vel : rv;
-        hn[q] = (ix_t)g.idx(min(i0 + tx, g.Nx + 2), min(grow, g.Ny + 2), kbeg) + (sel == 3 ? sz : (ix_t)0);
-    }
-    auto frame_load = [&](int q, ix_t lev) -> double { return hsrc[q][hn[q] + lev]; };
-    auto frame_store = [&](int b, int q, double raw, int klev) {
-        if (hsel[q] == 0) Tv[b][hrow[q]][tc] = ST ? raw : bz_cdiv(raw, g.rho[klev], g.rrho[klev]);
-        else Tm[b][hsel[q] - 1][hrow[q]][tx] = ((hsel[q] == 1) ? g.Ax[klev] : (hsel[q] == 2) ? g.Ay[klev] : Az) * raw;
+        hsrc[q] = ((sel == 1) ? ru : (sel == 3) ? rw + sz : (ST && sel == 0) ? vel : rv) + kb;
+        ho[q] = bz_pidx5(g, min(i0 + tx, g.Nx + 2), min(grow, g.Ny + 2)) * (unsigned)sizeof(double);
+    }
+    auto frame_load = [&](int q) -> double { return lean_ldp(hsrc[q], ho[q]); };
+    auto frame_store = [&](int b, int q, double raw, int klev, bool packed) {
+        if (hsel[q] == 0) Tv[b][hrow[q]][tc] = ST ? raw : packed ? bz_cdiv(raw, c_rho(klev), c_rrho(klev)) : bz_cdiv(raw, g.rho[klev], g.rrho[klev]);
+        else Tm[b][hsel[q] - 1][hrow[q]][tx] = ((hsel[q] == 1) ? (packed ? c_Ax(klev) : g.Ax[klev]) : (hsel[q] == 2) ? (packed ? c_Ay(klev) : g.Ay[klev]) : Az) * raw;
     };
 
     const bool sok = t < 5 * TY;
     const int srow = sok ? t / 5 : 0, scc = sok ? t % 5 : 0, scol = (scc < 3) ? scc : 64 + scc;
-    const ix_t sn = (ix_t)g.idx(min(i0 - 3 + scol, g.Nx + 2), min(j0 + srow, g.Ny + 2), kbeg);
+    unsigned so = bz_pidx5(g, min(i0 - 3 + scol, g.Nx + 2), min(j0 + srow, g.Ny + 2)) * (unsigned)sizeof(double);
 
     double r[6];
 #pragma unroll
-    for (int s = 0; s < 6; ++s) r[s] = ST ? vel[n + s * sz - 3 * sz] : bz_cdiv(rv[n + s * sz - 3 * sz], g.rho[kbeg + s - 3], g.rrho[kbeg + s - 3]);
+    for (int s = 0; s < 6; ++s) r[s] = ST ? lean_ldp(vel + kb + (s - 3) * sz, o) : bz_cdiv(lean_ldp(rv + kb + (s - 3) * sz, o), g.rho[kbeg + s - 3], g.rrho[kbeg + s - 3]);
     double fz_lo;
     if (WY && Bf != 3) {
-        const double wt0 = bz_symm2(Az * rw[n - (ix_t)g.Sx], Az * rw[n]);
+        unsigned om = o - (unsigned)g.Sx * (unsigned)sizeof(double);
+        const double wt0 = bz_symm2(Az * lean_ldp(rw + kb, om), Az * lean_ldp(rw + kb, o));
         fz_lo = wt0 * bz_upB(r[0], r[1], r[2], r[3], r[4], r[5], wt0 > 0.0, bz_buffer_face(kbeg, g.Nz));
-    } else fz_lo = vflux<T3_V>(g, F, n, kbeg, r[0], r[1], r[2], r[3], r[4], r[5]);
-    double q0 = rv[n], q1 = rv[n + sz], q2 = rv[n + 2 * sz];
+    } else fz_lo = vflux<T3_V>(g, F, kb + (long long)(o / (unsigned)sizeof(double)), kbeg, r[0], r[1], r[2], r[3], r[4], r[5]);
+    double q0 = lean_ldp(rv + kb, o), q1 = lean_ldp(rv + kb + sz, o), q2 = lean_ldp(rv + kb + 2 * sz, o);
     Tv[0][ty + 3][tc] = r[3];
-    if (sok) Tv[0][srow + 3][scol] = ST ? vel[sn] : bz_cdiv(rv[sn], g.rho[kbeg], g.rrho[kbeg]);
-    Tm[0][0][ty + 2][tx] = g.Ax[kbeg] * ru[n];
+    if (sok) Tv[0][srow + 3][scol] = ST ? lean_ldp(vel + kb, so) : bz_cdiv(lean_ldp(rv + kb, so), g.rho[kbeg], g.rrho[kbeg]);
+    Tm[0][0][ty + 2][tx] = g.Ax[kbeg] * lean_ldp(ru + kb, o);
     Tm[0][1][ty + 2][tx] = g.Ay[kbeg] * q0;
-    Tm[0][2][ty + 2][tx] = Az * rw[n + sz];
+    Tm[0][2][ty + 2][tx] = Az * lean_ldp(rw + kb + sz, o);
 #pragma unroll
     for (int q = 0; q < HPT; ++q)
-        if (hok[q]) frame_store(0, q, frame_load(q, 0), kbeg);
+        if (hok[q]) frame_store(0, q, frame_load(q), kbeg, false);
     __syncthreads();
 
-    double tcur_raw = rv[n + 3 * sz];
-    double tcur_v = ST ? vel[n + 3 * sz] : 0.0;
-    double u0cur = (E.mode == 2) ? E.u0[n] : 0.0;
+    double tcur_raw = lean_ldp(rv + kb + 3 * sz, o);
+    double tcur_v = ST ? lean_ldp(vel + kb + 3 * sz, o) : 0.0;
+    double u0cur = (E.mode == 2) ? lean_ldp(E.u0 + kb, o) : 0.0;
     double edge = 0.0;
     int buf = 0;
-    for (int k = kbeg; k < kend; ++k, n += sz) {
-        const ix_t lev = (ix_t)(k + 1 - kbeg) * sz;
+    const double *rv_k = rv + kb, *vel_k = vel + kb, *ru_1 = ru + kb + sz, *rw_2 = rw + kb + 2 * sz, *u0_1 = E.u0 + kb + sz;
+    double *out_k = L.out + kb, *u0o_k = E.u0_out + kb;
+    for (int k = kbeg; k < kend; ++k) {
+        const long long up = (k + 4 <= g.Nz + g.Hz - 1) ? 4 * sz : 3 * sz;
         double hnext[HPT];
 #pragma unroll
-        for (int q = 0; q < HPT; ++q) hnext[q] = hok[q] ? frame_load(q, lev) : 0.0;
-        const double p_side = sok ? (ST ? vel : rv)[sn + lev] : 0.0;
-        const double p_top = ST ? rv[n + sz] : rv[n + ((k + 4 <= g.Nz + g.Hz - 1) ? 4 * sz : 3 * sz)];
-        const double p_topv = ST ? vel[n + ((k + 4 <= g.Nz + g.Hz - 1) ? 4 * sz : 3 * sz)] : 0.0;
-        const double p_u0 = (E.mode == 2) ? E.u0[n + sz] : 0.0;
+        for (int q = 0; q < HPT; ++q) { hsrc[q] += sz; hnext[q] = hok[q] ? frame_load(q) : 0.0; }
+        const double p_side = sok ? lean_ldp((ST ? vel_k : rv_k) + sz, so) : 0.0;
+        const double p_top = ST ? lean_ldp(rv_k + sz, o) : lean_ldp(rv_k + up, o);
+        const double p_topv = ST ? lean_ldp(vel_k + up, o) : 0.0;
+        const double p_u0 = (E.mode == 2) ? lean_ldp(u0_1, o) : 0.0;
         const double tnew_raw = tcur_raw, u0v = u0cur;
-        const double ru_n = g.Ax[k + 1] * ru[n + sz], rw_n = Az * rw[n + 2 * sz];
+        const double ru_n = c_Ax(k + 1) * lean_ldp(ru_1, o), rw_n = Az * lean_ldp(rw_2, o);
         double cor_u = 0.0, cg1 = 0.0, cg3 = 0.0;
-        if constexpr (MF) { if ((L.mforce & 1) && tx == 63) { const ix_t sy = (ix_t)g.Sx; cg1 = ru[n - sy + 1]; cg3 = ru[n + 1]; } }
+        if constexpr (MF) { if ((L.mforce & 1) && tx == 63) { unsigned o3 = o + (unsigned)sizeof(double), o1 = o3 - (unsigned)g.Sx * (unsigned)sizeof(double); cg1 = lean_ldp(ru_1 - sz, o1); cg3 = lean_ldp(ru_1 - sz, o3); } }
         if (((k - kbeg) & (BZ5_EB - 1)) == 0) {
             const int kk = min(k + (tx & (BZ5_EB - 1)), kend - 1);
             edge = ST ? flux_x_at<T3_V>(g, F, ie, jc, kk) : flux_x_lean<T3_V>(g, F, rv, ie, jc, kk, Bf);
         }
         const int src = (k - kbeg) & (BZ5_EB - 1);
-        const double rho = g.rho[k];
+        const double rho = c_rho(k);
         const double c0 = r[3];
         const double(*V)[TC] = Tv[buf];
         const double *vrow = V[ty + 3] + tc;
@@ -732,25 +748,25 @@
             const double vb = (!WY || Bc0 == 3) ? bz_symm4(MV[0][tx], MV[1][tx], MV[2][tx], MV[3][tx]) : bz_symm2(MV[1][tx], MV[2][tx]);
             FY[buf][0][tx] = vb * bz_up5y<WY>(V[0][tc], V[1][tc], V[2][tc], V[3][tc], V[4][tc], V[5][tc], vb > 0.0, Bc0);
         }
-        const double tnew = ST ? tcur_v : bz_cdiv(tnew_raw, g.rho[k + 3], g.rrho[k + 3]);
+        const double tnew = ST ? tcur_v : bz_cdiv(tnew_raw, c_rho(k + 3), c_rrho(k + 3));
         const double wt = bz_symm4y<WY>(MW[ty][tx], MW[ty + 1][tx], MW[ty + 2][tx], MW[ty + 3][tx], Bf);
         const double fz_hi = wt * bz_upB(r[1], r[2], r[3], r[4], r[5], tnew, wt > 0.0, bz_buffer_face(k + 1, g.Nz));
         if constexpr (MF) {
             if (L.mforce & 1) {
-                const double Axk = g.Ax[k];
+                const double Axk = c_Ax(k);
                 const double l1 = MU[ty + 1][tx + 1], l3 = MU[ty + 2][tx + 1];
                 const double c1 = (tx == 63) ? Axk * cg1 : l1, c3 = (tx == 63) ? Axk * cg3 : l3;
                 cor_u = (((MU[ty + 1][tx] + c1) / 2 + (MU[ty + 2][tx] + c3) / 2) / 2) / Axk;
             }
         }
         Tv[buf ^ 1][ty + 3][tc] = r[4];
-        if (sok) Tv[buf ^ 1][srow + 3][scol] = ST ? p_side : bz_cdiv(p_side, g.rho[k + 1], g.rrho[k + 1]);
+        if (sok) Tv[buf ^ 1][srow + 3][scol] = ST ? p_side : bz_cdiv(p_side, c_rho(k + 1), c_rrho(k + 1));
         Tm[buf ^ 1][0][ty + 2][tx] = ru_n;
-        Tm[buf ^ 1][1][ty + 2][tx] = g.Ay[k + 1] * (ST ? p_top : q1);
+        Tm[buf ^ 1][1][ty + 2][tx] = c_Ay(k + 1) * (ST ? p_top : q1);
         Tm[buf ^ 1][2][ty + 2][tx] = rw_n;
 #pragma unroll
         for (int q = 0; q < HPT; ++q)
-            if (hok[q]) frame_store(buf ^ 1, q, hnext[q], k + 1);
+            if (hok[q]) frame_store(buf ^ 1, q, hnext[q], k + 1, true);
         bz6_barrier();
         {
             double nb = __shfl_down(fx, 1);
@@ -758,7 +774,7 @@
             if (tx == le) nb = e;
             const double dx = nb - fx;
             const double dy = fy - FY[buf][ty][tx];
-            double Gv = -(g.Vinv_c[k] * (dx + dy + (fz_hi - fz_lo)));
+            double Gv = -((ST ? g.Vinv_c[k] : LV.Vinv_c(k)) * (dx + dy + (fz_hi - fz_lo)));
             if constexpr (MF) {
                 if (L.mforce & 1) Gv -= L.cor_f * cor_u;
                 if (L.mforce & (4 | 16)) {
@@ -767,10 +783,10 @@
                     Gv += tot;
                 }
             }
-            if (store) L.out[n] = (ST && E.mode == 0) ? Gv : bz_rk_apply_pre(E.mode, E.dt, E.alpha, E.oma, u0v, E.u0_out, Gv, q0, n);
+            if (store) lean_stp(out_k, o, (ST && E.mode == 0) ? Gv : bz_rk_apply_lev(E.mode, rk_dt, rk_alpha, rk_oma, u0v, u0o_k, Gv, q0, o));
             if constexpr (WY) {
-                if (i < g.Nx && j == 0) L.out[n] = 0.0;
-                if (i < g.Nx && j == g.Ny - 1) L.out[n + (ix_t)g.Sx] = 0.0;
+                if (i < g.Nx && j == 0) lean_stp(out_k, o, 0.0);
+                if (i < g.Nx && j == g.Ny - 1) { unsigned oa = o + (unsigned)g.Sx * (unsigned)sizeof(double); lean_stp(out_k, oa, 0.0); }
             }
         }
         fz_lo = fz_hi;
@@ -782,6 +798,7 @@
         for (int s = 0; s < 5; ++s) r[s] = r[s + 1];
         r[5] = tnew;
         buf ^= 1;
+        rv_k += sz; vel_k += sz; ru_1 += sz; rw_2 += sz; u0_1 += sz; out_k += sz; u0o_k += sz;
     }
 }
 
@@ -801,10 +818,19 @@
 }
 
 
+__device__ __forceinline__ double buoyancy5_dry(const DevGrid &g, double rth, double rho, double rrho, double pi, double T_ref)
+{
+    const double T = pi * bz_cdiv(rth, rho, rrho);
+    const double rhop = rho * (g.Rd * T_ref / (g.Rd * T) - 1.0);
+    return -g.g * rhop;
+}
+
+
 template <int TY, bool WY = false, bool DRYQ = false, bool GUARD = true, int BM = 4>
 __global__ __launch_bounds__(64 * TY, BZ6_W_WAVES) void k6_w(DevGrid g, Lean5 L, int kchunk, RKEpilogue E)
 {
     constexpr bool ST = BM != 4;
+    constexpr bool UB = (BM == 4 && DRYQ);
     static_assert(!(ST && (WY || DRYQ || GUARD)), "stored-velocity instantiations: periodic / slab rows, no moisture-scan dispatch");
     if (bz_lean_skip<DRYQ, GUARD>(L)) return;
     constexpr int TR = TY + 6, TC = 72, NT = 64 * TY, NH = TR * 70 - TY * 64;
@@ -842,13 +868,21 @@
     }
     const ix32_t hn = (ix32_t)g.idx(min(i0 - 3 + hc, g.Nx + 2), min(j0 - 3 + hr, g.Ny + 2), kbeg);
     const ix32_t ntop0 = (ix32_t)g.idx(ic, min(j0 + TY, g.Ny), kbeg);
-    const bool top = (ty == 0);
+    unsigned o = bz_pidx5(g, ic, jc) * (unsigned)sizeof(double), ho = bz_pidx5(g, min(i0 - 3 + hc, g.Nx + 2), min(j0 - 3 + hr, g.Ny + 2)) * (unsigned)sizeof(double);
+    unsigned otop = bz_pidx5(g, ic, min(j0 + TY, g.Ny)) * (unsigned)sizeof(double);
+    const long long szl = g.Sxy;
+    const long long kcur = szl * (long long)(kbeg + g.Hz);
+    const bool top = UB ? (__builtin_amdgcn_readfirstlane(ty) == 0) : (ty == 0);
+    ix32_t lev = 0;
+    auto own = [&](const double *a, long long d) { if constexpr (UB) return lean_ldp(a + kcur + d * szl, o); else return a[n + (ix32_t)d * sz]; };
+    auto frm = [&](const double *a, long long d) { if constexpr (UB) return lean_ldp(a + kcur + d * szl, ho); else return a[hn + lev + (ix32_t)d * sz]; };
+    auto abv = [&](const double *a, long long d) { if constexpr (UB) return lean_ldp(a + kcur + d * szl, otop); else return a[ntop0 + lev + (ix32_t)d * sz]; };
 
     double wr[6], qu[4], qv[4], qt[4], qw[4];
     double raw0 = 0.0, raw1 = 0.0, raw2 = 0.0;
 #pragma unroll
     for (int s = 0; s < 6; ++s) {
-        const double x = rw[n + s * sz - 3 * sz];
+        const double x = UB ? own(rw, s - 3) : rw[n + s * sz - 3 * sz];
         wr[s] = ST ? vel[n + s * sz - 3 * sz] : bz_cdiv(x, LV.rho_f(kbeg + s - 3), LV.rrho_f(kbeg + s - 3));
         if (s >= 1 && s <= 4) qw[s - 1] = Az * x;
         if (s == 3) raw0 = x;
@@ -859,40 +893,45 @@
     for (int s = 0; s < 4; ++s) {
         const int kk = kbeg - 2 + s;
         const double Axk = ST ? g.Ax[kk] : LV.Ax(kk), Ayk = ST ? g.Ay[kk] : LV.Ay(kk);
-        qu[s] = Axk * ru[n + s * sz - 2 * sz];
-        qv[s] = Ayk * rv[n + s * sz - 2 * sz];
-        qt[s] = top ? Ayk * rv[ntop0 + s * sz - 2 * sz] : 0.0;
+        qu[s] = Axk * (UB ? own(ru, s - 2) : ru[n + s * sz - 2 * sz]);
+        qv[s] = Ayk * (UB ? own(rv, s - 2) : rv[n + s * sz - 2 * sz]);
+        qt[s] = top ? Ayk * (UB ? abv(rv, s - 2) : rv[ntop0 + s * sz - 2 * sz]) : 0.0;
     }
     double fz_lo, b_lo, r_lo = 0.0;
     {
         const int B = bz_buffer_center(kbeg - 1, g.Nz);
         const double wt = (B == 3) ? bz_symm4(qw[0], qw[1], qw[2], qw[3]) : bz_symm2(qw[1], qw[2]);
         fz_lo = wt * bz_upB(wr[0], wr[1], wr[2], wr[3], wr[4], wr[5], wt > 0.0, B);
-        if constexpr (BM == 4) b_lo = buoyancy5(g, pa[n - sz], dryq ? 0.0 : pb[n - sz], kbeg - 1, LV.rho(kbeg - 1), LV.rrho(kbeg - 1), LV.pi(kbeg - 1), LV.T_r(kbeg - 1));
+        if constexpr (BM == 4 && dryq) b_lo = buoyancy5_dry(g, UB ? own(pa, -1) : pa[n - sz], LV.rho(kbeg - 1), LV.rrho(kbeg - 1), LV.pi(kbeg - 1), LV.T_r(kbeg - 1));
+        else if constexpr (BM == 4) b_lo = buoyancy5(g, pa[n - sz], dryq ? 0.0 : pb[n - sz], kbeg - 1, LV.rho(kbeg - 1), LV.rrho(kbeg - 1), LV.pi(kbeg - 1), LV.T_r(kbeg - 1));
         else if constexpr (BM == 0) b_lo = buoyancy3(g, bT[n - sz], bq[n - sz], kbeg - 1);
         else if constexpr (BM == 3) b_lo = bz_buoyancy(g, bT, bq, (long long)(n - sz), kbeg - 1);
         else if constexpr (BM == 2) { b_lo = bT[n - sz] - g.p_r[kbeg - 1]; r_lo = bq[n - sz] - g.rho[kbeg - 1]; }
         else b_lo = 0.0;
     }
     T[0][ty + 3][tc] = wr[3];
-    if (hok) T[0][hr][hc] = ST ? vel[hn] : bz_cdiv(rw[hn], LV.rho_f(kbeg), LV.rrho_f(kbeg));
-    double tcur_raw = rw[n + 3 * sz];
+    if (hok) T[0][hr][hc] = ST ? vel[hn] : bz_cdiv(frm(rw, 0), LV.rho_f(kbeg), LV.rrho_f(kbeg));
+    double tcur_raw = own(rw, 3);
     double tcur_v = ST ? vel[n + 3 * sz] : 0.0;
-    double u0cur = (E.mode == 2) ? E.u0[n] : 0.0;
+    double u0cur = (E.mode == 2) ? own(E.u0, 0) : 0.0;
     __syncthreads();
 
     double edge = 0.0;
     int buf = 0;
+    const double *rw_k = rw + kcur, *ru_2 = ru + kcur + 2 * szl, *rv_2 = rv + kcur + 2 * szl, *th_k = pa + kcur, *u0_1 = E.u0 + kcur + szl;
+    double *out_k = L.out + kcur, *u0o_k = E.u0_out + kcur;
+    auto ld = [&](const double *level_base, unsigned &off, const double *a, ix32_t idx) { if constexpr (UB) return lean_ldp(level_base, off); else return a[idx]; };
     for (int k = kbeg; k < kend; ++k, n += sz) {
-        const ix32_t lev = (ix32_t)(k - kbeg) * sz;
-        const double p_h = hok ? (ST ? vel : rw)[hn + lev + sz] : 0.0;
-        const double p_top = rw[n + ((k + 4 <= g.Nz + g.Hz) ? 4 * sz : 3 * sz)];
+        lev = (ix32_t)(k - kbeg) * sz;
+        const double p_h = hok ? ld(rw_k + szl, ho, ST ? vel : rw, hn + lev + sz) : 0.0;
+        const double p_top = ld(rw_k + ((k + 4 <= g.Nz + g.Hz) ? 4 * szl : 3 * szl), o, rw, n + ((k + 4 <= g.Nz + g.Hz) ? 4 * sz : 3 * sz));
         const double p_topv = ST ? vel[n + ((k + 4 <= g.Nz + g.Hz) ? 4 * sz : 3 * sz)] : 0.0;
-        const double Tcur = (BM == 1) ? 0.0 : (ST ? bT : pa)[n], rqcur = (BM == 1) ? 0.0 : ST ? bq[n] : dryq ? 0.0 : pb[n];
-        const double p_u0 = (E.mode == 2) ? E.u0[n + sz] : 0.0;
+        const double Tcur = (BM == 1) ? 0.0 : ld(th_k, o, ST ? bT : pa, n), rqcur = (BM == 1) ? 0.0 : ST ? bq[n] : dryq ? 0.0 : pb[n];
+        const double p_u0 = (E.mode == 2) ? ld(u0_1, o, E.u0, n + sz) : 0.0;
         const double Axn = ST ? g.Ax[k + 2] : LV.Ax(k + 2), Ayn = ST ? g.Ay[k + 2] : LV.Ay(k + 2);
-        const double qun = Axn * ru[n + 2 * sz], qvn = Ayn * rv[n + 2 * sz];
-        const double qtn = top ? Ayn * rv[ntop0 + lev + 2 * sz] : 0.0;
+        const double qun = Axn * ld(ru_2, o, ru, n + 2 * sz), qvn = Ayn * ld(rv_2, o, rv, n + 2 * sz);
+        double qtn = 0.0;
+        if (top) qtn = Ayn * ld(rv_2, otop, rv, ntop0 + lev + 2 * sz);
         if (((k - kbeg) & (BZ5_EB - 1)) == 0) {
             const int kk = min(k + (tx & (BZ5_EB - 1)), kend - 1);
             edge = ST ? flux_x_at<T3_W>(g, F, ie, jc, kk) : flux_x_lean<T3_W>(g, F, rw, ie, jc, kk);
@@ -922,7 +961,8 @@
             fz_hi = wt * bz_upB(wr[1], wr[2], wr[3], wr[4], wr[5], wnew, wt > 0.0, B);
         }
         double b_hi = 0.0, r_hi = 0.0;
-        if constexpr (BM == 4) b_hi = buoyancy5(g, Tcur, rqcur, k, LV.rho(k), LV.rrho(k), LV.pi(k), LV.T_r(k));
+        if constexpr (BM == 4 && dryq) b_hi = buoyancy5_dry(g, Tcur, LV.rho(k), LV.rrho(k), LV.pi(k), LV.T_r(k));
+        else if constexpr (BM == 4) b_hi = buoyancy5(g, Tcur, rqcur, k, LV.rho(k), LV.rrho(k), LV.pi(k), LV.T_r(k));
         else if constexpr (BM == 0) b_hi = buoyancy3(g, Tcur, rqcur, k);
         else if constexpr (BM == 3) b_hi = bz_buoyancy(g, bT, bq, (long long)n, k);
         else if constexpr (BM == 2) { b_hi = Tcur - g.p_r[k]; r_hi = rqcur - g.rho[k]; }
@@ -940,15 +980,18 @@
             if constexpr (BM == 2) Gval = adv - (b_hi - b_lo) * g.rdzf[k] - g.g * ((r_hi + r_lo) / 2.0);
             else if constexpr (BM == 1) Gval = adv;
             else Gval = adv + 0.5 * (b_lo + b_hi);
-            if (store)
-                L.out[n] = (ST && E.mode == 0) ? Gval : bz_rk_apply_pre(E.mode, E.dt, E.alpha, E.oma, u0cur, E.u0_out, Gval, uold, n);
+            if (store) {
+                if constexpr (UB) lean_stp(out_k, o, bz_rk_apply_lev(E.mode, E.dt, E.alpha, E.oma, u0cur, u0o_k, Gval, uold, o));
+                else L.out[n] = (ST && E.mode == 0) ? Gval : bz_rk_apply_pre(E.mode, E.dt, E.alpha, E.oma, u0cur, E.u0_out, Gval, uold, n);
+            }
         }
         fz_lo = fz_hi;
         b_lo = b_hi;
         r_lo = r_hi;
 #pragma unroll
-        for (int s = 0; s < 3; ++s) { qu[s] = qu[s + 1]; qv[s] = qv[s + 1]; qt[s] = qt[s + 1]; qw[s] = qw[s + 1]; }
-        qu[3] = qun; qv[3] = qvn; qt[3] = qtn; qw[3] = qwnew;
+        for (int s = 0; s < 3; ++s) { qu[s] = qu[s + 1]; qv[s] = qv[s + 1]; qw[s] = qw[s + 1]; }
+        qu[3] = qun; qv[3] = qvn; qw[3] = qwnew;
+        if (!UB || top) { qt[0] = qt[1]; qt[1] = qt[2]; qt[2] = qt[3]; qt[3] = qtn; }
         raw0 = raw1; raw1 = raw2; raw2 = tcur_raw;
         tcur_raw = p_top; u0cur = p_u0;
         if (ST) tcur_v = p_topv;
@@ -956,5 +999,6 @@
         for (int s = 0; s < 5; ++s) wr[s] = wr[s + 1];
         wr[5] = wnew;
         buf ^= 1;
-    }
-}
+        if constexpr (UB) { rw_k += szl; ru_2 += szl; rv_2 += szl; th_k += szl; u0_1 += szl; out_k += szl; u0o_k += szl; }
+    }
+}
```

Result: no change. 4.232 billion (median of 6 runs) (+0.8%).
